# nkwangyh/CubemapSLAM

Hardware: AMD Instinct MI355X
Metric: frames/sec (extract+match+localBA) on Lafida cam0 (higher is better)
Workload: dtype u8 (extract/match), f64 (BA)

## Files before the change

### cubemapslam_amd/api.py

```python
import time
import ctypes as C
import os
import numpy as np

_HERE = os.path.dirname(os.path.abspath(__file__))
LIB_PATH = os.environ.get("CMS_HIP_LIB") or os.path.join(_HERE, "lib", "libcubemapslam_hip.so")


class CmsError(RuntimeError):
    pass


class Camera(C.Structure):
    _fields_ = [("c", C.c_double), ("d", C.c_double), ("e", C.c_double), ("u0", C.c_double), ("v0", C.c_double),
                ("invpol", C.c_double * 12), ("pol", C.c_double * 5), ("Iw", C.c_int), ("Ih", C.c_int),
                ("face", C.c_int), ("fov_deg", C.c_double)]


class OrbParams(C.Structure):
    _fields_ = [("nfeatures", C.c_int), ("scale_factor", C.c_float), ("nlevels", C.c_int),
                ("ini_th_fast", C.c_int), ("min_th_fast", C.c_int)]


class Geometry(C.Structure):
    _fields_ = [("W", C.c_int), ("F", C.c_int), ("nlevels", C.c_int), ("kp_cap", C.c_int), ("max_batch", C.c_int),
                ("level_w", C.c_int * 12), ("level_h", C.c_int * 12), ("level_quota", C.c_int * 12),
                ("level_cells", C.c_int * 12), ("scale", C.c_float * 12), ("inv_scale", C.c_float * 12),
                ("sigma2", C.c_float * 12), ("inv_sigma2", C.c_float * 12), ("pyramid_bytes_per_frame", C.c_size_t),
                ("candidate_entries_per_frame", C.c_size_t), ("fisheye_stride", C.c_int)]


class BaStats(C.Structure):
    _fields_ = [("iterations_done", C.c_int * 2), ("chi2_initial", C.c_double * 2), ("chi2_final", C.c_double * 2),
                ("lambda_final", C.c_double * 2), ("n_outliers_mid", C.c_int), ("n_outliers_final", C.c_int)]


KP_DTYPE = np.dtype([("x", "<f4"), ("y", "<f4"), ("size", "<f4"), ("angle", "<f4"), ("response", "<f4"),
                     ("octave", "<i4")])

_lib = None


def lib():
    global _lib
    if _lib is None:
        if not os.path.exists(LIB_PATH):
            raise CmsError("libcubemapslam_hip.so is missing -- build it with `python -m cubemapslam_amd.build` "
                           "(there is no CPU fallback)")
        L = C.CDLL(LIB_PATH)
        L.cms_last_error.restype = C.c_char_p
        for n in ("cms_ctx_stream", "cms_frames_input", "cms_ba_stream"):
            getattr(L, n).restype = C.c_void_p
            getattr(L, n).argtypes = [C.c_void_p]
        L.cms_ctx_create.argtypes = [C.c_void_p, C.c_int, C.c_void_p, C.c_void_p, C.c_int]
        L.cms_ctx_destroy.argtypes = [C.c_void_p]
        L.cms_ctx_destroy.restype = None
        L.cms_ctx_geometry.argtypes = [C.c_void_p, C.c_void_p]
        L.cms_remap.argtypes = [C.c_void_p, C.c_void_p, C.c_int, C.c_void_p, C.c_int]
        L.cms_set_mask.argtypes = [C.c_void_p, C.c_void_p, C.c_int]
        L.cms_extract.argtypes = [C.c_void_p, C.c_void_p, C.c_int, C.c_void_p, C.c_void_p, C.c_int, C.c_void_p]
        L.cms_remap_extract.argtypes = [C.c_void_p, C.c_void_p, C.c_int, C.c_void_p, C.c_void_p, C.c_int, C.c_void_p]
        L.cms_frames_upload.argtypes = [C.c_void_p, C.c_void_p, C.c_int, C.c_size_t, C.c_int]
        L.cms_frames_upload_async.argtypes = [C.c_void_p, C.c_void_p, C.c_int, C.c_size_t, C.c_int]
        L.cms_frames_upload_wait.argtypes = [C.c_void_p]
        L.cms_frames_upload_device.argtypes = [C.c_void_p, C.c_void_p, C.c_int]
        L.cms_frames_process_device.argtypes = [C.c_void_p, C.c_void_p, C.c_int]
        L.cms_host_alloc.argtypes = [C.c_void_p, C.c_size_t]
        L.cms_host_free.argtypes = [C.c_void_p]
        L.cms_host_free.restype = None
        L.cms_ba_profile_kernel.argtypes = [C.c_void_p, C.c_int]
        L.cms_ba_profile_get.argtypes = [C.c_void_p, C.c_void_p, C.c_void_p]
        L.cms_ba_debug_compose.argtypes = [C.c_int, C.c_void_p, C.c_int, C.c_int, C.c_void_p, C.c_void_p, C.c_int, C.c_void_p, C.c_void_p, C.c_void_p, C.c_void_p]
        L.cms_frames_process.argtypes = [C.c_void_p, C.c_int, C.c_int]
        L.cms_frames_sync.argtypes = [C.c_void_p]
        L.cms_frames_results.argtypes = [C.c_void_p, C.c_void_p, C.c_void_p, C.c_void_p]
        L.cms_frames_fetch.argtypes = [C.c_void_p, C.c_int, C.c_void_p, C.c_void_p, C.c_int, C.c_void_p]
        L.cms_debug_lut.argtypes = [C.c_void_p, C.c_void_p, C.c_void_p]
        L.cms_debug_cubemap.argtypes = [C.c_void_p, C.c_int, C.c_void_p, C.c_int]
        L.cms_debug_level.argtypes = [C.c_void_p, C.c_int, C.c_int, C.c_void_p, C.c_int]
        L.cms_debug_candidates.argtypes = [C.c_void_p, C.c_int, C.c_int, C.c_void_p, C.c_int, C.c_void_p]
        L.cms_debug_distributed.argtypes = [C.c_void_p, C.c_int, C.c_int, C.c_void_p, C.c_int, C.c_void_p]
        L.cms_profile_enable.argtypes = [C.c_void_p, C.c_int]
        L.cms_profile_get.argtypes = [C.c_void_p, C.c_void_p]
        L.cms_hamming_best2.argtypes = [C.c_void_p, C.c_void_p, C.c_int, C.c_void_p, C.c_int] + [C.c_void_p] * 9
        L.cms_hamming_best2_device.argtypes = [C.c_void_p, C.c_void_p, C.c_void_p, C.c_int] + [C.c_void_p] * 10
        L.cms_hamming_matrix.argtypes = [C.c_void_p, C.c_void_p, C.c_int, C.c_void_p, C.c_int, C.c_void_p]
        L.cms_ba_create.argtypes = [C.c_void_p, C.c_int, C.c_int, C.c_void_p, C.c_void_p, C.c_int, C.c_void_p, C.c_int,
                                    C.c_void_p, C.c_void_p, C.c_void_p, C.c_void_p, C.c_void_p, C.c_double, C.c_double,
                                    C.c_double, C.c_double]
        L.cms_ba_reset.argtypes = [C.c_void_p]
        L.cms_ba_optimize.argtypes = [C.c_void_p, C.c_int, C.c_int, C.c_void_p, C.c_void_p]
        L.cms_ba_read.argtypes = [C.c_void_p, C.c_void_p, C.c_void_p, C.c_void_p]
        L.cms_ba_destroy.argtypes = [C.c_void_p]
        L.cms_ba_destroy.restype = None
        L.cms_ba_run.argtypes = [C.c_int, C.c_int, C.c_void_p, C.c_void_p, C.c_int, C.c_void_p, C.c_int, C.c_void_p,
                                 C.c_void_p, C.c_void_p, C.c_void_p, C.c_void_p, C.c_double, C.c_double, C.c_double,
                                 C.c_double, C.c_int, C.c_int, C.c_void_p, C.c_void_p, C.c_void_p]
        L.cms_ba_linearize.argtypes = [C.c_int, C.c_int, C.c_void_p, C.c_void_p, C.c_int, C.c_void_p, C.c_int, C.c_void_p,
                                       C.c_void_p, C.c_void_p, C.c_void_p, C.c_void_p, C.c_double, C.c_double, C.c_double,
                                       C.c_double, C.c_int, C.c_double] + [C.c_void_p] * 7
        L.cms_area_set_keypoints.argtypes = [C.c_void_p, C.c_int, C.c_int, C.c_void_p]
        L.cms_area_grid.argtypes = [C.c_void_p, C.c_int]
        L.cms_features_in_area.argtypes = [C.c_void_p, C.c_int, C.c_int] + [C.c_void_p] * 7 + [C.c_int, C.c_void_p]
        L.cms_features_in_area_device.argtypes = [C.c_void_p, C.c_int, C.c_int] + [C.c_void_p] * 8 + [C.c_int, C.c_int, C.c_void_p]
        L.cms_features_in_area_batch_device.argtypes = [C.c_void_p, C.c_int] + [C.c_void_p] * 9 + [C.c_int, C.c_void_p]
        L.cms_area_set_descriptors.argtypes = [C.c_void_p, C.c_int, C.c_int, C.c_void_p]
        L.cms_search_local_points.argtypes = ([C.c_void_p, C.c_int, C.c_void_p, C.c_int] + [C.c_void_p] * 5 + [C.c_float] * 3 + [C.c_int, C.c_int] +
                                              [C.c_void_p] * 9)
        L.cms_search_by_projection.argtypes = ([C.c_void_p, C.c_int, C.c_void_p, C.c_int] + [C.c_void_p] * 5 + [C.c_float, C.c_int, C.c_int, C.c_int] +
                                               [C.c_void_p] * 3)
        L.cms_project_last_frame_device.argtypes = [C.c_void_p, C.c_int] + [C.c_void_p] * 5 + [C.c_float] + [C.c_void_p] * 5
        L.cms_rotation_filter_device.argtypes = [C.c_void_p, C.c_int] + [C.c_void_p] * 5 + [C.c_int]
        L.cms_is_in_frustum_device.argtypes = [C.c_void_p, C.c_int] + [C.c_void_p] * 6 + [C.c_float, C.c_float] + [C.c_void_p] * 8
        L.cms_search_local_points_device.argtypes = [C.c_void_p, C.c_int] + [C.c_void_p] * 5 + [C.c_float, C.c_int] + [C.c_void_p] * 3
        L.cms_create_new_map_points.argtypes = [C.c_void_p, C.c_int, C.c_void_p, C.c_void_p, C.c_void_p, C.c_int, C.c_int] + [C.c_void_p] * 5
        L.cms_kfstore_create.argtypes = [C.c_void_p, C.c_void_p, C.c_int, C.c_int, C.c_int]
        L.cms_kfstore_destroy.argtypes = [C.c_void_p]
        L.cms_kfstore_destroy.restype = None
        L.cms_kfstore_put.argtypes = [C.c_void_p, C.c_int, C.c_void_p]
        L.cms_kfstore_update.argtypes = [C.c_void_p, C.c_int] + [C.c_void_p] * 5
        L.cms_kfstore_fuse_search.argtypes = [C.c_void_p, C.c_int] + [C.c_void_p] * 8 + [C.c_float, C.c_void_p, C.c_void_p]
        L.cms_kfstore_fuse_search_sets.argtypes = [C.c_void_p, C.c_int] + [C.c_void_p] * 6 + [C.c_int] + [C.c_void_p] * 3 + [C.c_float, C.c_void_p, C.c_void_p]
        L.cms_kfstore_put_from_frame.argtypes = [C.c_void_p, C.c_int, C.c_void_p, C.c_int, C.c_int, C.c_void_p, C.c_void_p, C.c_void_p, C.c_float, C.c_void_p, C.c_int,
                                                 C.c_void_p, C.c_void_p, C.c_void_p]
        L.cms_kfstore_update_poses.argtypes = [C.c_void_p, C.c_int] + [C.c_void_p] * 4
        L.cms_kfstore_debug_fetch.argtypes = [C.c_void_p, C.c_int] + [C.c_void_p] * 12
        L.cms_ba_debug_fetch_plan.argtypes = [C.c_void_p] * 14
        L.cms_kfstore_create_new_map_points.argtypes = [C.c_void_p, C.c_int, C.c_void_p, C.c_void_p, C.c_void_p, C.c_int, C.c_int] + [C.c_void_p] * 5
        L.cms_distinctive_descriptors.argtypes = [C.c_void_p, C.c_int, C.c_void_p, C.c_void_p, C.c_void_p]
        L.cms_update_normal_and_depth.argtypes = [C.c_void_p, C.c_int] + [C.c_void_p] * 8
        L.cms_fuse_search.argtypes = [C.c_void_p, C.c_int, C.c_void_p, C.c_int] + [C.c_void_p] * 6 + [C.c_float, C.c_void_p, C.c_void_p]
        L.cms_pose_create.argtypes = [C.c_void_p, C.c_int, C.c_int, C.c_int]
        L.cms_pose_destroy.argtypes = [C.c_void_p]
        L.cms_pose_destroy.restype = None
        L.cms_pose_stream.argtypes = [C.c_void_p]
        L.cms_pose_stream.restype = C.c_void_p
        _edge = [C.c_void_p] * 5 + [C.c_double] * 4
        L.cms_pose_upload.argtypes = [C.c_void_p, C.c_int] + _edge + [C.c_void_p]
        L.cms_pose_launch.argtypes = [C.c_void_p]
        L.cms_pose_fetch.argtypes = [C.c_void_p, C.c_void_p, C.c_void_p, C.c_void_p, C.c_void_p]
        L.cms_pose_optimize_batch.argtypes = [C.c_void_p, C.c_int] + _edge + [C.c_void_p] * 4
        L.cms_pose_optimize.argtypes = [C.c_int, C.c_int] + [C.c_void_p] * 4 + [C.c_double] * 4 + [C.c_void_p] * 4
        _lib = L
    return _lib


def _p(a):
    if a is None:
        return None
    if isinstance(a, int):
        return C.c_void_p(a)
    return a.ctypes.data_as(C.c_void_p)


def _chk(rc, what):
    if rc < 0:
        raise CmsError("%s failed (%d): %s" % (what, rc, lib().cms_last_error().decode()))
    return rc


def make_camera(d):
    cam = Camera()
    for k in ("c", "d", "e", "u0", "v0", "Iw", "Ih", "face", "fov_deg"):
        setattr(cam, k, d[k])
    for i in range(12):
        cam.invpol[i] = d["invpol"][i] if i < len(d["invpol"]) else 0.0
    for i in range(5):
        cam.pol[i] = d["pol"][i] if i < len(d["pol"]) else 0.0
    return cam


RT_DTYPE = np.dtype([(n, "<u2") for n in ("tx", "ty", "x0", "y0", "nd", "rows", "flags", "pad")])
RT_LDS_MAX = 32768


def remap_lut_host(cam):
    cam = make_camera(cam) if isinstance(cam, dict) else cam
    W = 3 * cam.face
    out = np.zeros((W, (W + 3) // 4 * 4), np.uint32)
    f = lib().cms_remap_lut_host
    f.argtypes = [C.c_void_p, C.c_void_p, C.c_int]
    _chk(f(C.byref(cam), _p(out), out.shape[1]), "cms_remap_lut_host")
    return out[:, :W]


def remap_tiles_host(cam, lut, tile_w, tile_h, lds_budget=RT_LDS_MAX):
    cam = make_camera(cam) if isinstance(cam, dict) else cam
    lut = np.ascontiguousarray(lut, np.uint32)
    W = 3 * cam.face
    cap = ((W + tile_w - 1) // tile_w) * ((W + tile_h - 1) // tile_h)
    out = np.zeros(cap, RT_DTYPE)
    n_live, n_all, lds = C.c_int(), C.c_int(), C.c_int()
    f = lib().cms_remap_tiles_host
    f.argtypes = [C.c_void_p, C.c_void_p] + [C.c_int] * 4 + [C.c_void_p, C.c_int] + [C.c_void_p] * 3
    _chk(f(C.byref(cam), _p(lut), lut.strides[0] // 4, tile_w, tile_h, lds_budget, _p(out), cap, C.byref(n_live), C.byref(n_all), C.byref(lds)),
         "cms_remap_tiles_host")
    return out[:n_all.value].copy(), n_live.value, lds.value


class Context:

    def __init__(self, cam, nfeatures=2000, scale_factor=1.2, nlevels=8, ini_th=20, min_th=7, max_batch=1, device=0):
        self.cam = make_camera(cam) if isinstance(cam, dict) else cam
        self.orb = OrbParams(nfeatures, scale_factor, nlevels, ini_th, min_th)
        self.h = C.c_void_p()
        _chk(lib().cms_ctx_create(C.byref(self.h), device, C.byref(self.cam), C.byref(self.orb), max_batch), "cms_ctx_create")
        self.geom = Geometry()
        _chk(lib().cms_ctx_geometry(self.h, C.byref(self.geom)), "cms_ctx_geometry")
        self.W = self.geom.W
        self.max_batch = max_batch

    def close(self):
        if getattr(self, "h", None) and self.h.value:
            lib().cms_ctx_destroy(self.h)
            self.h = C.c_void_p()

    def __del__(self):
        try:
            self.close()
        except Exception:
            pass

    @property
    def stream(self):
        return lib().cms_ctx_stream(self.h)

    def set_mask(self, mask):
        mask = np.ascontiguousarray(mask, np.uint8)
        _chk(lib().cms_set_mask(self.h, _p(mask), mask.strides[0]), "cms_set_mask")

    def set_distance_bounds_mode(self, scaled):
        f = lib().cms_set_distance_bounds_mode
        f.argtypes = [C.c_void_p, C.c_int]
        _chk(f(self.h, int(scaled)), "cms_set_distance_bounds_mode")

    def set_gaussian_mode(self, column_mode):
        f = lib().cms_set_gaussian_mode
        f.argtypes = [C.c_void_p, C.c_int]
        _chk(f(self.h, int(column_mode)), "cms_set_gaussian_mode")

    def remap(self, fisheye, cubemap=None):
        fisheye = np.ascontiguousarray(fisheye, np.uint8)
        if cubemap is None:
            cubemap = np.zeros((self.W, self.W), np.uint8)
        _chk(lib().cms_remap(self.h, _p(fisheye), fisheye.strides[0], _p(cubemap), cubemap.strides[0]), "cms_remap")
        return cubemap

    def extract(self, cubemap, cap=None):
        cubemap = np.ascontiguousarray(cubemap, np.uint8)
        cap = cap or self.geom.kp_cap
        kps = np.zeros(cap, KP_DTYPE)
        desc = np.zeros((cap, 32), np.uint8)
        n = C.c_int()
        _chk(lib().cms_extract(self.h, _p(cubemap), cubemap.strides[0], _p(kps), _p(desc), cap, C.byref(n)), "cms_extract")
        return kps[:n.value].copy(), desc[:n.value].copy()

    def remap_extract(self, fisheye, cap=None):
        fisheye = np.ascontiguousarray(fisheye, np.uint8)
        cap = cap or self.geom.kp_cap
        kps = np.zeros(cap, KP_DTYPE)
        desc = np.zeros((cap, 32), np.uint8)
        n = C.c_int()
        _chk(lib().cms_remap_extract(self.h, _p(fisheye), fisheye.strides[0], _p(kps), _p(desc), cap, C.byref(n)), "cms_remap_extract")
        return kps[:n.value].copy(), desc[:n.value].copy()

    def remap_extract_rays(self, fisheye, cap=None):
        fisheye = np.ascontiguousarray(fisheye, np.uint8)
# ... 44 lines not shown
    def sync(self):
        _chk(lib().cms_frames_sync(self.h), "cms_frames_sync")

    def fetch(self, b):
        cap = self.geom.kp_cap
        kps = np.zeros(cap, KP_DTYPE)
        desc = np.zeros((cap, 32), np.uint8)
        n = C.c_int()
        _chk(lib().cms_frames_fetch(self.h, b, _p(kps), _p(desc), cap, C.byref(n)), "cms_frames_fetch")
        return kps[:n.value].copy(), desc[:n.value].copy()

    def results_ptrs(self):
        a, b, c = C.c_void_p(), C.c_void_p(), C.c_void_p()
        _chk(lib().cms_frames_results(self.h, C.byref(a), C.byref(b), C.byref(c)), "cms_frames_results")
        return a.value, b.value, c.value

    def input_ptr(self):
        return lib().cms_frames_input(self.h)

    def profile(self, on=True):
        lib().cms_profile_enable(self.h, 1 if on else 0)

    def profile_ms(self):
        ms = np.zeros(7, np.float32)
        _chk(lib().cms_profile_get(self.h, _p(ms)), "cms_profile_get")
        return dict(zip(("remap", "pyramid", "fast", "octree", "cull", "describe", "total"), ms.tolist()))

    def debug_lut(self):
        W = self.W
        out = np.zeros((W, (W + 3) // 4 * 4), np.uint32)
        s = C.c_int()
        _chk(lib().cms_debug_lut(self.h, _p(out), C.byref(s)), "cms_debug_lut")
        return out[:, :W]

    def debug_level(self, b, l):
        w, h = self.geom.level_w[l], self.geom.level_h[l]
        out = np.zeros((h, w), np.uint8)
        _chk(lib().cms_debug_level(self.h, b, l, _p(out), w), "cms_debug_level")
        return out

    def debug_candidates(self, b, l):
        cap = self.geom.level_w[l] * self.geom.level_h[l] // 4 + 4096
        out = np.zeros((cap, 3), np.int32)
        n = C.c_int()
        _chk(lib().cms_debug_candidates(self.h, b, l, _p(out), cap, C.byref(n)), "cms_debug_candidates")
        return out[:n.value].copy()

    def debug_distributed(self, b, l):
        cap = self.geom.level_quota[l] + 8
        out = np.zeros((cap, 3), np.int32)
        n = C.c_int()
        _chk(lib().cms_debug_distributed(self.h, b, l, _p(out), cap, C.byref(n)), "cms_debug_distributed")
        return out[:n.value].copy()

    def hamming_best2(self, qdesc, tdesc, cand_off, cand_idx, tlevel=None, texcl=None):
        qdesc = np.ascontiguousarray(qdesc, np.uint8); tdesc = np.ascontiguousarray(tdesc, np.uint8)
        cand_off = np.ascontiguousarray(cand_off, np.int32); cand_idx = np.ascontiguousarray(cand_idx, np.int32)
        tl = np.ascontiguousarray(tlevel, np.int32) if tlevel is not None else None
        tx = np.ascontiguousarray(texcl, np.uint8) if texcl is not None else None
        nq = len(qdesc)
        outs = [np.zeros(max(nq, 1), np.int32) for _ in range(5)]
        _chk(lib().cms_hamming_best2(self.h, _p(qdesc), nq, _p(tdesc), len(tdesc), _p(cand_off), _p(cand_idx), _p(tl), _p(tx),
                                     *[_p(o) for o in outs]), "cms_hamming_best2")
        keys = ("best_idx", "best_dist", "best_level", "second_dist", "second_level")
        return {k: o[:nq] for k, o in zip(keys, outs)}

    def area_set_keypoints(self, b, kps):
        kps = np.ascontiguousarray(kps, KP_DTYPE)
        _chk(lib().cms_area_set_keypoints(self.h, b, len(kps), _p(kps)), "cms_area_set_keypoints")

    def area_grid(self, B):
        _chk(lib().cms_area_grid(self.h, B), "cms_area_grid")

    def features_in_area(self, b, qx, qy, qr, qmin, qmax, cap=None):
        qx = np.ascontiguousarray(qx, np.float32); qy = np.ascontiguousarray(qy, np.float32); qr = np.ascontiguousarray(qr, np.float32)
        qmin = np.ascontiguousarray(qmin, np.int32); qmax = np.ascontiguousarray(qmax, np.int32)
        nq = len(qx)
        cap = cap or max(1, 64 * nq + 1024)
        off = np.zeros(nq + 1, np.int32); idx = np.zeros(cap, np.int32); tot = C.c_int(0)
        _chk(lib().cms_features_in_area(self.h, b, nq, _p(qx), _p(qy), _p(qr), _p(qmin), _p(qmax), _p(off), _p(idx), cap, C.byref(tot)),
             "cms_features_in_area")
        return off, idx[:tot.value]

    def features_in_area_device(self, b, nq, d_q5, d_cnt, d_off, d_idx, cap, idx_base, d_total):
        _chk(lib().cms_features_in_area_device(self.h, b, nq, *[C.c_void_p(int(a)) for a in d_q5], C.c_void_p(int(d_cnt)), C.c_void_p(int(d_off)),
                                               C.c_void_p(int(d_idx)), cap, idx_base, C.c_void_p(int(d_total))), "cms_features_in_area_device")

    def features_in_area_batch_device(self, nq, d_qframe, d_q5, d_cnt, d_off, d_idx, cap, d_total):
        _chk(lib().cms_features_in_area_batch_device(self.h, nq, C.c_void_p(int(d_qframe)), *[C.c_void_p(int(a)) for a in d_q5], C.c_void_p(int(d_cnt)),
                                                     C.c_void_p(int(d_off)), C.c_void_p(int(d_idx)), cap, C.c_void_p(int(d_total))),
             "cms_features_in_area_batch_device")

    def area_set_descriptors(self, b, desc):
        desc = np.ascontiguousarray(desc, np.uint8)
        _chk(lib().cms_area_set_descriptors(self.h, b, len(desc), _p(desc)), "cms_area_set_descriptors")

    def search_local_points(self, b, pose15, pos, normal, min_dist, max_dist, mp_desc, kp_mp, viewing_cos_limit=0.5, th=1.0, nnratio=0.8,
                            th_high=100):
        pose15 = np.ascontiguousarray(pose15, np.float32).reshape(15)
        pos = np.ascontiguousarray(pos, np.float32).reshape(-1, 3); normal = np.ascontiguousarray(normal, np.float32).reshape(-1, 3)
        n = len(pos)
        min_dist = np.ascontiguousarray(min_dist, np.float32); max_dist = np.ascontiguousarray(max_dist, np.float32)
        mp_desc = np.ascontiguousarray(mp_desc, np.uint8).reshape(n, 32)
        assert kp_mp.dtype == np.int32 and kp_mp.flags.c_contiguous
        vis = np.zeros(n, np.uint8); px = np.zeros(n, np.float32); py = np.zeros(n, np.float32); lvl = np.zeros(n, np.int32)
        vc = np.zeros(n, np.float32); match = np.full(n, -1, np.int32)
        nm = C.c_int(0); rounds = C.c_int(0)
        _chk(lib().cms_search_local_points(self.h, b, _p(pose15), n, _p(pos), _p(normal), _p(min_dist), _p(max_dist), _p(mp_desc),
                                           viewing_cos_limit, th, nnratio, th_high, len(kp_mp), _p(kp_mp), _p(vis), _p(px), _p(py), _p(lvl),
                                           _p(vc), _p(match), C.addressof(nm), C.addressof(rounds)), "cms_search_local_points")
        return dict(in_view=vis, proj_x=px, proj_y=py, level=lvl, view_cos=vc, match=match, n_matches=nm.value, rounds=rounds.value)

    def search_by_projection(self, b, pose12, valid, Xw, octave, angle, mp_desc, kp_mp, th=15.0, check_ori=True, th_high=100):
        a = [np.ascontiguousarray(pose12, np.float32), np.ascontiguousarray(valid, np.uint8), np.ascontiguousarray(Xw, np.float32),
             np.ascontiguousarray(octave, np.int32), np.ascontiguousarray(angle, np.float32), np.ascontiguousarray(mp_desc, np.uint8)]
        n = len(a[1])
        match = np.full(n, -1, np.int32); nm = C.c_int(0)
        assert kp_mp.dtype == np.int32
        _chk(lib().cms_search_by_projection(self.h, b, _p(a[0]), n, *[_p(v) for v in a[1:]], th, int(check_ori), th_high, len(kp_mp), _p(kp_mp), _p(match),
                                            C.addressof(nm)), "cms_search_by_projection")
        return match, nm.value

    def search_for_initialization(self, b2, k1, d1, prev_matched, window=100, nnratio=0.9, check_ori=True):
        k1 = np.ascontiguousarray(k1, KP_DTYPE); d1 = np.ascontiguousarray(d1, np.uint8)
        assert prev_matched.dtype == np.float32 and prev_matched.flags.c_contiguous and prev_matched.shape == (len(k1), 2)
        m12 = np.full(max(len(k1), 1), -1, np.int32); nm = C.c_int(0)
        f = lib().cms_search_for_initialization
        f.argtypes = [C.c_void_p, C.c_int, C.c_int, C.c_void_p, C.c_void_p, C.c_void_p, C.c_int, C.c_float, C.c_int, C.c_void_p, C.c_void_p]
        _chk(f(self.h, b2, len(k1), _p(k1), _p(d1), _p(prev_matched), int(window), float(nnratio), int(check_ori), _p(m12), C.addressof(nm)),
             "cms_search_for_initialization")
        return m12[:len(k1)], nm.value

    def project_last_frame_device(self, n, d_qframe, d_pose12, d_valid, d_Xw, d_oct, th, d_q5):
        v = lambda a: C.c_void_p(int(a)) if a else None
        _chk(lib().cms_project_last_frame_device(self.h, n, v(d_qframe), v(d_pose12), v(d_valid), v(d_Xw), v(d_oct), th, *[v(a) for a in d_q5]),
             "cms_project_last_frame_device")

    def rotation_filter_device(self, B, d_mp_off, d_last_angle, d_kp_mp, d_mp_match, d_n_matches, check_orientation=True):
        v = lambda a: C.c_void_p(int(a)) if a else None
        _chk(lib().cms_rotation_filter_device(self.h, B, v(d_mp_off), v(d_last_angle), v(d_kp_mp), v(d_mp_match), v(d_n_matches), int(check_orientation)),
             "cms_rotation_filter_device")

    def is_in_frustum_device(self, nmp, d_mp_frame, d_pose15, d_pos, d_normal, d_min, d_max, viewing_cos_limit, th, d_outs5, d_q3):
        v = lambda a: C.c_void_p(int(a)) if a else None
        _chk(lib().cms_is_in_frustum_device(self.h, nmp, v(d_mp_frame), v(d_pose15), v(d_pos), v(d_normal), v(d_min), v(d_max),
                                            viewing_cos_limit, th, *[v(a) for a in d_outs5], *[v(a) for a in d_q3]), "cms_is_in_frustum_device")

    def search_local_points_device(self, B, d_mp_off, d_mp_desc, d_cand_off, d_cand_idx, d_pair_dist, nnratio, th_high, d_kp_mp, d_mp_match,
                                   d_rounds=0):
        v = lambda a: C.c_void_p(int(a)) if a else None
        _chk(lib().cms_search_local_points_device(self.h, B, v(d_mp_off), v(d_mp_desc), v(d_cand_off), v(d_cand_idx), v(d_pair_dist), nnratio,
                                                  th_high, v(d_kp_mp), v(d_mp_match), v(d_rounds)), "cms_search_local_points_device")

    def hamming_best2_device(self, qdesc, q_row, nq, tdesc, cand_off, cand_idx, t_level, t_excl, outs):
        _chk(lib().cms_hamming_best2_device(self.h, _p(qdesc), _p(q_row), nq, _p(tdesc), _p(cand_off), _p(cand_idx), _p(t_level),
                                            _p(t_excl), *[_p(o) for o in outs]), "cms_hamming_best2_device")

    def hamming_matrix(self, a, b):
        a = np.ascontiguousarray(a, np.uint8); b = np.ascontiguousarray(b, np.uint8)
        out = np.zeros((len(a), len(b)), np.uint16)
        _chk(lib().cms_hamming_matrix(self.h, _p(a), len(a), _p(b), len(b), _p(out)), "cms_hamming_matrix")
        return out


class PinnedArray:

    def __init__(self, shape):
        n = int(np.prod(shape))
        self.p = C.c_void_p()
        _chk(lib().cms_host_alloc(C.byref(self.p), n), "cms_host_alloc")
        self.array = np.ctypeslib.as_array((C.c_uint8 * n).from_address(self.p.value)).reshape(shape)

    def close(self):
        if self.p:
            self.array = None
            lib().cms_host_free(self.p)
            self.p = None

    def __del__(self):
        try:
            self.close()
        except Exception:
            pass


class Keyframe(C.Structure):
    _fields_ = [("n", C.c_int), ("kps", C.c_void_p), ("desc", C.c_void_p), ("rays", C.c_void_p), ("mp", C.c_void_p),
                ("Rcw", C.c_float * 9), ("tcw", C.c_float * 3), ("Ow", C.c_float * 3),
                ("nnodes", C.c_int), ("node_id", C.c_void_p), ("node_off", C.c_void_p), ("node_feat", C.c_void_p), ("median_depth", C.c_float)]


def make_keyframe(kf):
    n = len(kf["x"])
    kps = np.zeros(n, KP_DTYPE); kps["x"] = kf["x"]; kps["y"] = kf["y"]; kps["octave"] = kf["octave"]; kps["angle"] = kf["angle"]
    keep = [kps, np.ascontiguousarray(kf["desc"], np.uint8), np.ascontiguousarray(kf["rays"], np.float32), np.ascontiguousarray(kf["mp"], np.int32),
            np.ascontiguousarray(kf["node_id"], np.int32), np.ascontiguousarray(kf["node_off"], np.int32), np.ascontiguousarray(kf["node_feat"], np.int32)]
    K = Keyframe()
    K.n = n; K.kps = keep[0].ctypes.data; K.desc = keep[1].ctypes.data; K.rays = keep[2].ctypes.data; K.mp = keep[3].ctypes.data
    K.Rcw[:] = [float(v) for v in np.asarray(kf["R"], np.float32).reshape(9)]
    K.tcw[:] = [float(v) for v in kf["t"]]; K.Ow[:] = [float(v) for v in kf["Ow"]]
    K.nnodes = len(keep[4]); K.node_id = keep[4].ctypes.data; K.node_off = keep[5].ctypes.data; K.node_feat = keep[6].ctypes.data
    K.median_depth = float(kf["median_depth"])
    return K, keep


def search_for_triangulation(ctx, K1, K2, E12=None, check_orientation=False):
    m = np.full(max(K1.n, 1), -1, np.int32)
    n = C.c_int()
    e = None if E12 is None else np.ascontiguousarray(E12, np.float32)
    lib().cms_search_for_triangulation.argtypes = [C.c_void_p, C.c_void_p, C.c_void_p, C.c_void_p, C.c_int, C.c_void_p, C.c_void_p]
    _chk(lib().cms_search_for_triangulation(ctx.h, C.byref(K1), C.byref(K2), _p(e) if e is not None else None, int(check_orientation), _p(m), C.byref(n)),
         "cms_search_for_triangulation")
    return m[:K1.n].copy(), n.value


def create_new_map_points(ctx, jobs, check_orientation=False, cap=None):
    nj = len(jobs)
    cur = (Keyframe * max(nj, 1))(*[j[0] for j in jobs])
    flat = [k for j in jobs for k in j[1]]
    neigh = (Keyframe * max(len(flat), 1))(*flat)
    off = np.concatenate([[0], np.cumsum([len(j[1]) for j in jobs])]).astype(np.int32)
    cap = cap if cap is not None else max([j[0].n for j in jobs] + [1])
    n_new = np.zeros(max(nj, 1), np.int32)
    on = np.zeros((max(nj, 1), cap), np.int32); o1 = np.zeros_like(on); o2 = np.zeros_like(on); ox = np.zeros((max(nj, 1), cap, 3), np.float32)
    _chk(lib().cms_create_new_map_points(ctx.h, nj, C.addressof(cur), _p(off), C.addressof(neigh), int(check_orientation), cap, _p(n_new), _p(on), _p(o1),
                                         _p(o2), _p(ox)), "cms_create_new_map_points")
    return [(on[j, :n_new[j]].copy(), o1[j, :n_new[j]].copy(), o2[j, :n_new[j]].copy(), ox[j, :n_new[j]].copy()) for j in range(nj)]


class BowJob(C.Structure):
    _fields_ = [("slot", C.c_int), ("b", C.c_int), ("n", C.c_int), ("nnodes", C.c_int), ("node_id", C.c_void_p), ("node_off", C.c_void_p),
                ("node_feat", C.c_void_p), ("kf_skip", C.c_void_p)]


def _bow_fv(fv):
    if isinstance(fv, dict):
        fv = (fv["node_id"], fv["node_off"], fv["node_feat"])
    nid, noff, nfeat = (np.ascontiguousarray(a, np.int32) for a in fv)
    if len(noff) == 0:
        noff = np.zeros(1, np.int32)
    return nid, noff, (nfeat if len(nfeat) else np.zeros(1, np.int32))


def search_by_bow(ctx, b, n, fv, K, skip=None, nnratio=0.7, check_orientation=True):
    nid, noff, nfeat = _bow_fv(fv)
    sk = None if skip is None else np.ascontiguousarray(skip, np.uint8)
    kf_idx = np.full(max(n, 1), -1, np.int32)
    nm = C.c_int()
    L = lib()
    L.cms_search_by_bow.argtypes = [C.c_void_p, C.c_int, C.c_int, C.c_int, C.c_void_p, C.c_void_p, C.c_void_p, C.c_void_p, C.c_void_p, C.c_float, C.c_int,
                                    C.c_void_p, C.c_void_p]
    _chk(L.cms_search_by_bow(ctx.h, b, n, len(nid), _p(nid), _p(noff), _p(nfeat), C.byref(K), _p(sk), float(nnratio), int(check_orientation), _p(kf_idx),
                             C.byref(nm)), "cms_search_by_bow")
    return kf_idx[:n].copy(), nm.value


class KeyframeStore:

    def __init__(self, ctx, max_keyframes, max_features=2048, max_nodes=2048):
        self.ctx = ctx
        self.h = C.c_void_p()
        _chk(lib().cms_kfstore_create(C.byref(self.h), ctx.h, max_keyframes, max_features, max_nodes), "cms_kfstore_create")

    def close(self):
        if self.h:
            lib().cms_kfstore_destroy(self.h); self.h = None

    def __del__(self):
        try:
            self.close()
        except Exception:
            pass

    def put(self, slot, K):
        _chk(lib().cms_kfstore_put(self.h, slot, C.byref(K)), "cms_kfstore_put")

    def update(self, slot, R=None, t=None, Ow=None, median_depth=None, mp=None):
        f = lambda a, dt: None if a is None else np.ascontiguousarray(a, dt)
        a = [f(R, np.float32), f(t, np.float32), f(Ow, np.float32), None if median_depth is None else np.array([median_depth], np.float32), f(mp, np.int32)]
        _chk(lib().cms_kfstore_update(self.h, slot, *[_p(v) for v in a]), "cms_kfstore_update")

    def put_from_frame(self, slot, src_ctx, b, n, kf):
        f32 = lambda a: np.ascontiguousarray(a, np.float32)
        i32 = lambda a: None if a is None else np.ascontiguousarray(a, np.int32)
        R, t, Ow = f32(np.asarray(kf["R"]).reshape(9)), f32(kf["t"]), f32(kf["Ow"])
        mp, nid, noff, nfeat = i32(kf.get("mp")), i32(kf["node_id"]), i32(kf["node_off"]), i32(kf["node_feat"])
        L = lib()
        _chk(L.cms_kfstore_put_from_frame(self.h, slot, src_ctx.h, b, n, _p(R), _p(t), _p(Ow), float(kf["median_depth"]), _p(mp), len(nid), _p(nid), _p(noff), _p(nfeat)),
             "cms_kfstore_put_from_frame")

    def put_from_frames(self, src_ctx, items):
        class KfFromFrame(C.Structure):
            _fields_ = [("slot", C.c_int), ("b", C.c_int), ("n", C.c_int), ("Rcw", C.c_void_p), ("tcw", C.c_void_p), ("Ow", C.c_void_p), ("median_depth", C.c_float),
                        ("mp", C.c_void_p), ("nnodes", C.c_int), ("node_id", C.c_void_p), ("node_off", C.c_void_p), ("node_feat", C.c_void_p)]
        arr = (KfFromFrame * len(items))()
        keep = []
        f32 = lambda a: np.ascontiguousarray(a, np.float32)
        i32 = lambda a: None if a is None else np.ascontiguousarray(a, np.int32)
        ptr = lambda a: None if a is None else a.ctypes.data
        for q, (slot, b, n, kf) in zip(arr, items):
            R, t, Ow = f32(np.asarray(kf["R"]).reshape(9)), f32(kf["t"]), f32(kf["Ow"])
            mp, nid, noff, nfeat = i32(kf.get("mp")), i32(kf["node_id"]), i32(kf["node_off"]), i32(kf["node_feat"])
            keep.append((R, t, Ow, mp, nid, noff, nfeat))
            q.slot = slot; q.b = b; q.n = n; q.Rcw = ptr(R); q.tcw = ptr(t); q.Ow = ptr(Ow); q.median_depth = float(kf["median_depth"]); q.mp = ptr(mp)
            q.nnodes = len(nid); q.node_id = ptr(nid); q.node_off = ptr(noff); q.node_feat = ptr(nfeat)
        L = lib()
# ... 405 lines not shown
```

### cubemapslam_amd/csrc/cms_api_frames.hip

```cpp
#include <chrono>
#include <thread>
#include <hip/hip_runtime.h>
#include <math.h>
#include <stdio.h>
#include <stdlib.h>
#include <string.h>
#include <algorithm>
#include <string>
#include <vector>
#include "../../include/cubemapslam_hip.h"
#include "cms_types.h"
#include "orb_pattern.inc"

static bool cms_cu_mask_from_env(uint32_t* words, int* n_words) {
  const char* v = getenv("CMS_CTX_CU_MASK");
  if (!v || !*v) return false;
  int n = 0;
  while (*v && n < 8) {
    char* end = nullptr;
    words[n++] = (uint32_t)strtoul(v, &end, 16);
    if (end == v) return false;
    v = *end == ',' ? end + 1 : end;
    if (*end && *end != ',') return false;
  }
  *n_words = n;
  return n > 0;
}

static thread_local std::string g_cms_err;
static int cms_fail(int code, const char* what, hipError_t e = hipSuccess) {
  char buf[512];
  if (e != hipSuccess) snprintf(buf, sizeof(buf), "%s: %s", what, hipGetErrorString(e));
  else snprintf(buf, sizeof(buf), "%s", what);
  g_cms_err = buf;
  return code;
}
#define HIPCHK(call)                                                        \
  do {                                                                      \
    hipError_t _e = (call);                                                 \
    if (_e != hipSuccess) return cms_fail(CMS_ERR_HIP, #call, _e);          \
  } while (0)

extern "C" const char* cms_last_error(void) { return g_cms_err.c_str(); }
extern "C" int cms_device_count(void) {
  int n = 0;
  if (hipGetDeviceCount(&n) != hipSuccess) return 0;
  return n;
}

struct cms_ctx {
  int device = 0;
  cms_camera cam;
  cms_orb_params orb;
  int max_batch = 0;
  CmsGeom g;
  float scale[CMS_MAX_LEVELS], inv_scale[CMS_MAX_LEVELS], sigma2[CMS_MAX_LEVELS], inv_sigma2[CMS_MAX_LEVELS];
  hipStream_t stream = nullptr;
  int fstride = 0;
  size_t fish_pitch = 0;
  int lut_stride = 0, mstride = 0;
  bool have_mask = false;
  int dirty_frames = 0;
  uint8_t* d_fish = nullptr; uint32_t* d_lut = nullptr; uint8_t* d_pyr = nullptr; uint8_t* d_mask = nullptr;
  cms_remap_tile* d_rtiles = nullptr; int rt_mode = 1, rt_tw = 64, rt_live = 0, rt_all = 0, rt_lds = 0;
  CmsResizeTab* d_tab = nullptr; float* d_pattern = nullptr;
  uint32_t* d_cand = nullptr; uint16_t* d_node = nullptr; int* d_cand_cnt = nullptr; int* d_overflow = nullptr;
  uint32_t* d_qt_out = nullptr; int* d_qt_cnt = nullptr;
  uint32_t* d_cell_cand = nullptr; int* d_cell_cnt = nullptr;
  int* d_cells_all = nullptr; int* d_cells_nz = nullptr; int n_cells_all = 0, n_cells_nz = 0;
  uint16_t* d_area_sorted = nullptr; int* d_area_cell_start = nullptr; int* d_area_nvalid = nullptr; int area_frames = 0;
  int* d_area_bsum = nullptr; int area_bsum_cap = 0;
  int* d_area_tmp = nullptr; size_t area_tmp_cap = 0;
  uint8_t* h_fish_stage = nullptr; int fish_stage_frames = 0;
  hipStream_t copy_stream = nullptr; hipEvent_t ev_upload_done = nullptr, ev_remap_done = nullptr;
  bool upload_pending = false, remap_recorded = false;
  int dist_bounds_scaled = 0;
  hipEvent_t ev_block = nullptr; int last_batch = 0;
  hipEvent_t ev_extracted = nullptr; bool extracted_recorded = false;
  uint8_t* h_stage = nullptr; size_t h_stage_bytes = 0;
  CmsKeyPoint* d_kps = nullptr; uint32_t* d_aux = nullptr; uint8_t* d_desc = nullptr; int* d_kp_cnt = nullptr;
  uint32_t* d_order = nullptr; uint32_t* d_aux_sorted = nullptr; int* d_walk_cnt = nullptr; float* d_rays = nullptr;
  void* d_match = nullptr; size_t match_bytes = 0;
  bool prof = false;
  bool desc_spatial = false;
  hipEvent_t ev[8] = {nullptr, nullptr, nullptr, nullptr, nullptr, nullptr, nullptr, nullptr};
  size_t fast_lds = 0, qt_lds = 0;
};

static inline double cms_horner12(const double* c, double x) {
  double r = 0.0;
  for (int i = 11; i >= 0; --i) r = r * x + c[i];
  return r;
}
static void cms_cubemap_to_fisheye(const cms_camera& cam, double up, double vp, double* uf, double* vf) {
  const int F = cam.face;
  const double half = F / 2.0;
  float i = (float)up, j = (float)vp;
  *uf = -1; *vf = -1;
  const float fi = i / (float)F, fj = j / (float)F;
  int face = CMS_FACE_UNKNOWN;
  if (fi >= 0 && fi < 1 && fj >= 1 && fj < 2) face = CMS_FACE_LEFT;
  else if (fi >= 1 && fi < 2 && fj >= 0 && fj < 1) face = CMS_FACE_UPPER;
  else if (fi >= 1 && fi < 2 && fj >= 1 && fj < 2) face = CMS_FACE_FRONT;
  else if (fi >= 1 && fi < 2 && fj >= 2 && fj < 3) face = CMS_FACE_LOWER;
  else if (fi >= 2 && fi < 3 && fj >= 1 && fj < 2) face = CMS_FACE_RIGHT;
  if (face == CMS_FACE_UNKNOWN) return;
  i = i - (float)((int)(i / (float)F) * F);
  j = j - (float)((int)(j / (float)F) * F);
  const double lx = ((double)i - half) * 1.0 / half, ly = ((double)j - half) * 1.0 / half, lz = 1.0;
  double x, y, z;
  switch (face) {
    case CMS_FACE_FRONT: x = lx; y = ly; z = lz; break;
    case CMS_FACE_LEFT: x = -lz; y = ly; z = lx; break;
    case CMS_FACE_RIGHT: x = lz; y = ly; z = -lx; break;
    case CMS_FACE_LOWER: x = lx; y = lz; z = -ly; break;
    default: x = lx; y = -lz; z = ly; break;
  }
  double norm = sqrt(x * x + y * y);
  if (norm == 0.0) norm = 1e-14;
  const double theta = atan(-z / norm);
  const double rho = cms_horner12(cam.invpol, theta);
  const double uu = x / norm * rho, vv = y / norm * rho;
  *uf = uu * cam.c + vv * cam.d + cam.u0;
  *vf = uu * cam.e + vv + cam.v0;
  if (*uf < 0 || *uf >= cam.Iw || *vf < 0 || *vf >= cam.Ih) { *uf = -1; *vf = -1; }
}
static void cms_build_lut(const cms_camera& cam, int lut_stride, std::vector<uint32_t>& lut) {
  const int W = 3 * cam.face;
  lut.assign((size_t)W * lut_stride, 0u);
  for (int y = 0; y < W; ++y)
    for (int x = 0; x < W; ++x) {
      double u, v;
      cms_cubemap_to_fisheye(cam, (double)x, (double)y, &u, &v);
      if (u < 0 || v < 0 || u >= cam.Iw || v >= cam.Ih) continue;
      const float mu = (float)u, mv = (float)v;
      const int sx = (int)lrint((double)(mu * 32.f)), sy = (int)lrint((double)(mv * 32.f));
      const uint32_t X = (uint32_t)(sx >> 5), Y = (uint32_t)(sy >> 5), ax = (uint32_t)(sx & 31), ay = (uint32_t)(sy & 31);
      lut[(size_t)y * lut_stride + x] = X | (Y << 11) | (ax << 22) | (ay << 27);
    }
}

extern "C" int cms_remap_lut_host(const cms_camera* cam, uint32_t* lut, int lut_stride) {
  if (!cam || !lut || cam->face < 1 || lut_stride < 3 * cam->face) return cms_fail(CMS_ERR_ARG, "cms_remap_lut_host: bad argument");
  std::vector<uint32_t> v;
  cms_build_lut(*cam, lut_stride, v);
  memcpy(lut, v.data(), v.size() * 4);
  return CMS_OK;
}
extern "C" int cms_remap_tiles_host(const cms_camera* cam, const uint32_t* lut, int lut_stride, int tile_w, int tile_h, int lds_budget,
                                    cms_remap_tile* out, int cap, int* n_live, int* n_all, int* lds_bytes) {
  if (!cam || !lut || !out || !n_live || !n_all || !lds_bytes || cam->face < 1 || lut_stride < 3 * cam->face || !cms_rt_shape_ok(tile_w, tile_h) || lds_budget < 0)
    return cms_fail(CMS_ERR_ARG, "cms_remap_tiles_host: bad argument");
  std::vector<cms_remap_tile> v;
  cms_rt_build(cam->face, lut, lut_stride, tile_w, tile_h, lds_budget, v, n_live, lds_bytes);
  *n_all = (int)v.size();
  if ((int)v.size() > cap) return cms_fail(CMS_ERR_OVERFLOW, "cms_remap_tiles_host: caller capacity too small");
  memcpy(out, v.data(), v.size() * sizeof(cms_remap_tile));
  return CMS_OK;
}

static inline short cms_sat_short(float v) {
  const long iv = lrint((double)v);
  return (short)(iv < -32768 ? -32768 : iv > 32767 ? 32767 : iv);
}
static void cms_resize_table(int sn, int dn, bool clamp_frac, CmsResizeTab* out) {
  const double inv_scale = (double)dn / sn, scale = 1. / inv_scale;
  for (int d = 0; d < dn; ++d) {
    float f = (float)((d + 0.5) * scale - 0.5);
    int s = (int)floorf(f);
    f -= s;
    if (clamp_frac) {
      if (s < 0) { f = 0; s = 0; }
      if (s >= sn - 1) { f = 0; s = sn - 1; }
    }
    out[d].s = (short)s;
    out[d].a0 = cms_sat_short((1.f - f) * 2048);
    out[d].a1 = cms_sat_short(f * 2048);
    out[d].pad = 0;
  }
}

static size_t align_up(size_t v, size_t a) { return (v + a - 1) / a * a; }

static void cms_ctx_free(cms_ctx* c) {
  if (!c) return;
  hipSetDevice(c->device);
  void* ptrs[] = {c->d_fish, c->d_lut, c->d_pyr, c->d_mask, c->d_tab, c->d_pattern, c->d_cand, c->d_node, c->d_cand_cnt,
                  c->d_overflow, c->d_qt_out, c->d_qt_cnt, c->d_kps, c->d_aux, c->d_order, c->d_aux_sorted, c->d_desc, c->d_kp_cnt, c->d_match, c->d_cell_cand,
                  c->d_cell_cnt, c->d_cells_all, c->d_cells_nz, c->d_area_sorted, c->d_area_cell_start, c->d_area_nvalid, c->d_area_bsum, c->d_area_tmp, c->d_walk_cnt, c->d_rays, c->d_rtiles};
  for (void* p : ptrs) if (p) hipFree(p);
  if (c->h_fish_stage) (void)hipHostFree(c->h_fish_stage);
  if (c->h_stage) (void)hipHostFree(c->h_stage);
  for (int i = 0; i < 8; ++i) if (c->ev[i]) hipEventDestroy(c->ev[i]);
  if (c->ev_extracted) hipEventDestroy(c->ev_extracted);
  if (c->ev_block) hipEventDestroy(c->ev_block);
  if (c->ev_upload_done) hipEventDestroy(c->ev_upload_done);
  if (c->ev_remap_done) hipEventDestroy(c->ev_remap_done);
  if (c->copy_stream) hipStreamDestroy(c->copy_stream);
  if (c->stream) hipStreamDestroy(c->stream);
  delete c;
}

extern "C" int cms_ctx_create(cms_ctx** out, int device, const cms_camera* cam, const cms_orb_params* orb, int max_batch) {
  if (!out || !cam || !orb || max_batch < 1) return cms_fail(CMS_ERR_ARG, "cms_ctx_create: bad argument");
  *out = nullptr;
  if (orb->nlevels < 1 || orb->nlevels > CMS_MAX_LEVELS) return cms_fail(CMS_ERR_UNSUPPORTED, "nlevels must be 1..12");
  if (cam->face < 32 || 3 * cam->face > 4095) return cms_fail(CMS_ERR_UNSUPPORTED, "face size must satisfy 32 <= F and 3F <= 4095");
  if (cam->Iw < 2 || cam->Ih < 2 || cam->Iw > 2047 || cam->Ih > 2047) return cms_fail(CMS_ERR_UNSUPPORTED, "fisheye size must be <= 2047");
  int ndev = 0;
  if (hipGetDeviceCount(&ndev) != hipSuccess || ndev == 0) return cms_fail(CMS_ERR_NO_DEVICE, "no HIP device: the product path has no CPU fallback");
  if (device < 0 || device >= ndev) return cms_fail(CMS_ERR_ARG, "device index out of range");
  HIPCHK(hipSetDevice(device));
  cms_ctx* c = new cms_ctx;
  c->device = device; c->cam = *cam; c->orb = *orb; c->max_batch = max_batch;
  CmsGeom& g = c->g;
  memset(&g, 0, sizeof(g));
  const int L = orb->nlevels, F = cam->face, W = 3 * F;
  g.nlevels = L; g.W = W; g.F = F; g.ini_th = orb->ini_th_fast; g.min_th = orb->min_th_fast;
  const double scaleFactor = orb->scale_factor;
  c->scale[0] = 1.0f; c->sigma2[0] = 1.0f;
  for (int i = 1; i < L; ++i) { c->scale[i] = (float)(c->scale[i - 1] * scaleFactor); c->sigma2[i] = c->scale[i] * c->scale[i]; }
  for (int i = 0; i < L; ++i) { c->inv_scale[i] = 1.0f / c->scale[i]; c->inv_sigma2[i] = 1.0f / c->sigma2[i]; }
  {
    const float factor = (float)(1.0f / scaleFactor);
    float nDesired = orb->nfeatures * (1 - factor) / (1 - (float)pow((double)factor, (double)L));
    int sum = 0;
    for (int l = 0; l < L - 1; ++l) { g.lv[l].quota = (int)lrint((double)nDesired); sum += g.lv[l].quota; nDesired *= factor; }
    g.lv[L - 1].quota = orb->nfeatures - sum > 0 ? orb->nfeatures - sum : 0;
  }
  size_t off = 0, cand_off = 0, tab_off = 0;
  int cell0 = 0, kp_off = 0, maxq = 0, wCellMax = 0, hCellMax = 0;
  for (int l = 0; l < L; ++l) {
    CmsLevel& lv = g.lv[l];
    lv.w = (int)lrint((double)((float)W * c->inv_scale[l]));
    lv.h = lv.w;
    if (lv.w < 2 * CMS_MINB + 30) { delete c; return cms_fail(CMS_ERR_UNSUPPORTED, "pyramid level too small for the FAST cell grid"); }
    lv.stride = (int)align_up((size_t)lv.w + 8, 128);
    lv.off = off;
    off += align_up((size_t)lv.stride * (lv.h + 1), 256);
    const float width = (float)(lv.w - 2 * CMS_MINB), height = (float)(lv.h - 2 * CMS_MINB);
    lv.nCols = (int)(width / 30.f); lv.nRows = (int)(height / 30.f);
    lv.wCell = (int)ceilf(width / lv.nCols); lv.hCell = (int)ceilf(height / lv.nRows);
    lv.cell0 = cell0; cell0 += lv.nCols * lv.nRows;
    lv.cand_cap = (lv.w * lv.h) / 4 + 4096;
    lv.cand_off = cand_off; cand_off += align_up((size_t)lv.cand_cap, 64);
    lv.kp_off = kp_off; kp_off += lv.quota + 3;
    lv.scale = c->scale[l];
    lv.patch_size = (float)(int)(31 * c->scale[l]);
    lv.tab_off = tab_off; tab_off += (size_t)lv.w + lv.h;
    if (lv.quota > maxq) maxq = lv.quota;
    if (lv.wCell > wCellMax) wCellMax = lv.wCell;
    if (lv.hCell > hCellMax) hCellMax = lv.hCell;
    if (lv.nCols > 255 || lv.nRows > 255) { delete c; return cms_fail(CMS_ERR_UNSUPPORTED, "more than 255 FAST cells per row"); }
  }
  g.total_cells = cell0; g.kp_cap = kp_off; g.pyr_bytes = off; g.cand_total = cand_off;
  g.qt_maxn = 8;
  while (g.qt_maxn < maxq + 3) g.qt_maxn <<= 1;
  if (g.qt_maxn > 2048) { delete c; return cms_fail(CMS_ERR_UNSUPPORTED, "per-level feature quota above 2045 is not supported"); }
  g.tile_h = hCellMax + 6;
  g.tile_stride = (int)align_up((size_t)wCellMax + 6 + 3, 4) + 4;
  g.sc_h = hCellMax + 2;
  g.sc_stride = (int)align_up((size_t)wCellMax + 2, 4);
  g.list_cap = wCellMax * hCellMax;
  g.cell_cap = (int)align_up((size_t)((wCellMax + 1) / 2) * ((hCellMax + 1) / 2), 8);
  g.dbg_stop = getenv("CMS_DBG_FAST_STOP") ? atoi(getenv("CMS_DBG_FAST_STOP")) : 0;
  c->desc_spatial = getenv("CMS_DESC_SPATIAL_ORDER") != nullptr && g.kp_cap <= CMS_ORDER_MAX && max_batch <= 65535;
  g.gauss_column_mode = 0;
  if (wCellMax > 60 || hCellMax > 60) { delete c; return cms_fail(CMS_ERR_UNSUPPORTED, "FAST cell larger than 60 pixels"); }
  if (orb->scale_factor < 1.01f || orb->scale_factor > 1.9f) { delete c; return cms_fail(CMS_ERR_UNSUPPORTED, "scaleFactor must be in [1.01, 1.9]"); }
  g.fast_cell_lds = (int)align_up((size_t)g.tile_h * g.tile_stride + (size_t)g.sc_h * g.sc_stride + 2 * (size_t)g.list_cap + 16, 16);
  c->fast_lds = CMS_FAST_WPB * (size_t)g.fast_cell_lds;
  c->qt_lds = 64 * (size_t)g.qt_maxn + 4 * 512 + 64;

  c->fstride = (int)align_up((size_t)cam->Iw, 64);
  c->fish_pitch = (size_t)c->fstride * cam->Ih;
  c->lut_stride = (int)align_up((size_t)W, 4);
  c->mstride = (int)align_up((size_t)W, 64);
  const size_t B = (size_t)max_batch;
#define ALLOC(ptr, bytes) do { hipError_t _e = hipMalloc((void**)&(ptr), (bytes)); if (_e != hipSuccess) { cms_ctx_free(c); return cms_fail(CMS_ERR_HIP, "hipMalloc " #ptr, _e); } } while (0)
  hipError_t e;
  {
    const char* pr = getenv("CMS_FRAME_STREAM_PRIORITY");
    int lo = 0, hi = 0;
    uint32_t cu_mask[8]; int cu_words = 0;
    if (cms_cu_mask_from_env(cu_mask, &cu_words))
      e = hipExtStreamCreateWithCUMask(&c->stream, (uint32_t)cu_words, cu_mask);
    else
    if (pr && hipDeviceGetStreamPriorityRange(&lo, &hi) == hipSuccess && lo != hi)
      e = hipStreamCreateWithPriority(&c->stream, hipStreamNonBlocking, pr[0] == 'h' ? hi : lo);
    else
      e = hipStreamCreateWithFlags(&c->stream, hipStreamNonBlocking);
  }
  if (e != hipSuccess) { cms_ctx_free(c); return cms_fail(CMS_ERR_HIP, "hipStreamCreate", e); }
  for (int i = 0; i < 8; ++i) hipEventCreate(&c->ev[i]);
  ALLOC(c->d_fish, B * c->fish_pitch + 256);
  ALLOC(c->d_lut, (size_t)W * c->lut_stride * 4);
  ALLOC(c->d_pyr, B * g.pyr_bytes + 256);
  ALLOC(c->d_mask, (size_t)W * c->mstride);
  ALLOC(c->d_tab, tab_off * sizeof(CmsResizeTab));
  ALLOC(c->d_pattern, 1024 * sizeof(float));
  ALLOC(c->d_cand, B * g.cand_total * 4);
  ALLOC(c->d_node, B * g.cand_total * 2);
  ALLOC(c->d_cand_cnt, B * L * sizeof(int));
  ALLOC(c->d_overflow, sizeof(int));
  ALLOC(c->d_cell_cand, B * g.total_cells * g.cell_cap * 4);
  ALLOC(c->d_cell_cnt, B * g.total_cells * sizeof(int));
  ALLOC(c->d_qt_out, B * g.kp_cap * 4);
  ALLOC(c->d_qt_cnt, B * L * sizeof(int));
  ALLOC(c->d_kps, B * g.kp_cap * sizeof(CmsKeyPoint));
  ALLOC(c->d_aux, B * g.kp_cap * 4);
  ALLOC(c->d_order, B * g.kp_cap * 4);
  ALLOC(c->d_walk_cnt, 16);
  ALLOC(c->d_rays, B * g.kp_cap * 12);
  ALLOC(c->d_aux_sorted, B * g.kp_cap * 4);
  ALLOC(c->d_desc, B * g.kp_cap * 32);
  ALLOC(c->d_kp_cnt, B * sizeof(int));
#undef ALLOC
  hipMemset(c->d_pyr, 0, B * g.pyr_bytes + 256);
  hipMemset(c->d_fish, 0, B * c->fish_pitch + 256);
  hipMemset(c->d_mask, 255, (size_t)W * c->mstride);
  hipMemset(c->d_overflow, 0, sizeof(int));
  hipMemset(c->d_kp_cnt, 0, B * sizeof(int));
  {
    std::vector<uint32_t> lut;
    cms_build_lut(*cam, c->lut_stride, lut);
    hipMemcpy(c->d_lut, lut.data(), lut.size() * 4, hipMemcpyHostToDevice);
    {
      const char* m = getenv("CMS_REMAP_TILES"); const char* tw = getenv("CMS_REMAP_TILE_W");
      c->rt_mode = m && *m ? atoi(m) : 1;
      c->rt_tw = tw && *tw ? atoi(tw) : 64;
      if (c->rt_mode < 0 || c->rt_mode > 2 || !cms_rt_shape_ok(c->rt_tw, CMS_RT_PIXELS / std::max(c->rt_tw, 1))) {
        cms_ctx_free(c); return cms_fail(CMS_ERR_ARG, "CMS_REMAP_TILES must be 0, 1 or 2 and CMS_REMAP_TILE_W 32, 64 or 128");
      }
      std::vector<cms_remap_tile> tiles;
      cms_rt_build(F, lut.data(), c->lut_stride, c->rt_tw, CMS_RT_PIXELS / c->rt_tw, c->rt_mode == 1 ? CMS_RT_LDS_MAX : 0, tiles, &c->rt_live, &c->rt_lds);
      c->rt_all = (int)tiles.size();
      if (hipMalloc((void**)&c->d_rtiles, tiles.size() * sizeof(cms_remap_tile)) != hipSuccess) { cms_ctx_free(c); return cms_fail(CMS_ERR_HIP, "hipMalloc tile table"); }
      hipMemcpy(c->d_rtiles, tiles.data(), tiles.size() * sizeof(cms_remap_tile), hipMemcpyHostToDevice);
    }
    std::vector<CmsResizeTab> tab(tab_off);
    for (int l = 1; l < L; ++l) {
      cms_resize_table(g.lv[l - 1].w, g.lv[l].w, true, &tab[g.lv[l].tab_off]);
      cms_resize_table(g.lv[l - 1].h, g.lv[l].h, false, &tab[g.lv[l].tab_off + g.lv[l].w]);
    }
    g.lv[0].zlo = F; g.lv[0].zhi = F;
    for (int l = 1; l < L; ++l) {
      const CmsResizeTab* tx = &tab[g.lv[l].tab_off];
      const int sw = g.lv[l - 1].w, dw = g.lv[l].w;
      int lo = 0, hi = 0;
      while (lo < dw && std::min((int)tx[lo].s + 1, sw - 1) < g.lv[l - 1].zlo) ++lo;
      while (hi < dw && (int)tx[dw - 1 - hi].s >= sw - g.lv[l - 1].zhi) ++hi;
      g.lv[l].zlo = lo; g.lv[l].zhi = hi;
    }
    hipMemcpy(c->d_tab, tab.data(), tab.size() * sizeof(CmsResizeTab), hipMemcpyHostToDevice);
    std::vector<int> all, nz;
    for (int l = 0; l < L; ++l) {
      if (g.lv[l].nRows > 255 || g.lv[l].nCols > 255) { cms_ctx_free(c); return cms_fail(CMS_ERR_UNSUPPORTED, "cms_ctx_create: more than 255 FAST cells per row"); }
      const CmsLevel& lv = g.lv[l];
      const int maxBX = lv.w - CMS_MINB, maxBY = lv.h - CMS_MINB;
      for (int ci = 0; ci < lv.nRows; ++ci)
        for (int cj = 0; cj < lv.nCols; ++cj) {
          const int iniY = CMS_MINB + ci * lv.hCell, iniX = CMS_MINB + cj * lv.wCell;
          if (iniY >= maxBY - 3 || iniX >= maxBX - 6) continue;
          const int maxY = std::min(iniY + lv.hCell + 6, maxBY), maxX = std::min(iniX + lv.wCell + 6, maxBX);
          if (maxX - iniX - 6 <= 0 || maxY - iniY - 6 <= 0) continue;
          const int id = l | (ci << 4) | (cj << 12);
          all.push_back(id);
          const bool zero = (maxX <= lv.zlo || iniX >= lv.w - lv.zhi) && (maxY <= lv.zlo || iniY >= lv.h - lv.zhi);
          if (!zero) nz.push_back(id);
        }
    }
    auto xcd_stripe = [](std::vector<int>& v) {
      if (getenv("CMS_FAST_NO_XCD_STRIPE")) return;
      const size_t n = v.size(), per = (n + 7) / 8;
      std::vector<int> out;
      out.reserve(n);
      for (size_t j = 0; j < per; ++j)
        for (size_t x = 0; x < 8; ++x) if (x * per + j < n) out.push_back(v[x * per + j]);
      v.swap(out);
    };
    xcd_stripe(all); xcd_stripe(nz);
    c->n_cells_all = (int)all.size(); c->n_cells_nz = (int)nz.size();
    if (hipMalloc((void**)&c->d_cells_all, std::max<size_t>(all.size(), 1) * 4) != hipSuccess ||
        hipMalloc((void**)&c->d_cells_nz, std::max<size_t>(nz.size(), 1) * 4) != hipSuccess) {
      cms_ctx_free(c); return cms_fail(CMS_ERR_HIP, "hipMalloc cell lists");
    }
    hipMemcpy(c->d_cells_all, all.data(), all.size() * 4, hipMemcpyHostToDevice);
    hipMemcpy(c->d_cells_nz, nz.data(), nz.size() * 4, hipMemcpyHostToDevice);
    float patf[1024];
    for (int i = 0; i < 1024; ++i) patf[i] = (float)kOrbPattern[i];
    hipMemcpy(c->d_pattern, patf, sizeof(patf), hipMemcpyHostToDevice);
  }
  e = hipFuncSetAttribute((const void*)k_quadtree, hipFuncAttributeMaxDynamicSharedMemorySize, (int)c->qt_lds);
  if (e != hipSuccess) { cms_ctx_free(c); return cms_fail(CMS_ERR_HIP, "hipFuncSetAttribute(k_quadtree)", e); }
  e = hipDeviceSynchronize();
  if (e != hipSuccess) { cms_ctx_free(c); return cms_fail(CMS_ERR_HIP, "ctx init", e); }
  *out = c;
  return CMS_OK;
}

extern "C" void cms_ctx_destroy(cms_ctx* ctx) { cms_ctx_free(ctx); }
extern "C" void* cms_ctx_stream(cms_ctx* ctx) { return ctx ? (void*)ctx->stream : nullptr; }

extern "C" int cms_ctx_geometry(const cms_ctx* c, cms_geometry* o) {
  if (!c || !o) return cms_fail(CMS_ERR_ARG, "cms_ctx_geometry: null");
  memset(o, 0, sizeof(*o));
  o->W = c->g.W; o->F = c->g.F; o->nlevels = c->g.nlevels; o->kp_cap = c->g.kp_cap; o->max_batch = c->max_batch;
  for (int l = 0; l < c->g.nlevels; ++l) {
    o->level_w[l] = c->g.lv[l].w; o->level_h[l] = c->g.lv[l].h; o->level_quota[l] = c->g.lv[l].quota;
    o->level_cells[l] = c->g.lv[l].nCols * c->g.lv[l].nRows;
    o->scale[l] = c->scale[l]; o->inv_scale[l] = c->inv_scale[l]; o->sigma2[l] = c->sigma2[l]; o->inv_sigma2[l] = c->inv_sigma2[l];
  }
  o->pyramid_bytes_per_frame = c->g.pyr_bytes; o->candidate_entries_per_frame = c->g.cand_total;
  o->fisheye_stride = c->fstride;
  return CMS_OK;
}

extern "C" void* cms_frames_input(cms_ctx* c) { return c ? (void*)c->d_fish : nullptr; }

static int cms_frames_upload_impl(cms_ctx* c, const uint8_t* fisheye, int fstride, size_t frame_pitch, int B, bool wait) {
  if (!c || !fisheye || B < 1 || B > c->max_batch || fstride < c->cam.Iw) return cms_fail(CMS_ERR_ARG, "cms_frames_upload: bad argument");
  HIPCHK(hipSetDevice(c->device));
  const size_t per_frame = c->fish_pitch;
  if (!c->h_fish_stage || c->fish_stage_frames < B) {
    if (c->h_fish_stage) (void)hipHostFree(c->h_fish_stage);
    c->h_fish_stage = nullptr; c->fish_stage_frames = 0;
    if (hipHostMalloc((void**)&c->h_fish_stage, per_frame * (size_t)B) == hipSuccess) c->fish_stage_frames = B;
  }
  if (c->h_fish_stage) {
    for (int b = 0; b < B; ++b)
      for (int r = 0; r < c->cam.Ih; ++r)
        memcpy(c->h_fish_stage + (size_t)b * per_frame + (size_t)r * c->fstride, fisheye + (size_t)b * frame_pitch + (size_t)r * fstride, (size_t)c->cam.Iw);
    HIPCHK(hipMemcpyAsync(c->d_fish, c->h_fish_stage, per_frame * (size_t)B, hipMemcpyHostToDevice, c->stream));
  } else {
    for (int b = 0; b < B; ++b)
      HIPCHK(hipMemcpy2DAsync(c->d_fish + (size_t)b * c->fish_pitch, c->fstride, fisheye + (size_t)b * frame_pitch, fstride,
                              c->cam.Iw, c->cam.Ih, hipMemcpyHostToDevice, c->stream));
  }
  if (wait || !c->h_fish_stage) HIPCHK(hipStreamSynchronize(c->stream));
  return CMS_OK;
}
extern "C" int cms_frames_upload(cms_ctx* c, const uint8_t* fisheye, int fstride, size_t frame_pitch, int B) {
  return cms_frames_upload_impl(c, fisheye, fstride, frame_pitch, B, true);
}

extern "C" int cms_frames_upload_async(cms_ctx* c, const uint8_t* fisheye, int fstride, size_t frame_pitch, int B) {
  if (!c || !fisheye || B < 1 || B > c->max_batch || fstride < c->cam.Iw) return cms_fail(CMS_ERR_ARG, "cms_frames_upload_async: bad argument");
  HIPCHK(hipSetDevice(c->device));
  if (!c->copy_stream) {
    HIPCHK(hipStreamCreateWithFlags(&c->copy_stream, hipStreamNonBlocking));
    HIPCHK(hipEventCreateWithFlags(&c->ev_upload_done, hipEventDisableTiming));
    HIPCHK(hipEventCreateWithFlags(&c->ev_remap_done, hipEventDisableTiming));
    HIPCHK(hipEventRecord(c->ev_remap_done, c->stream));
    c->remap_recorded = true;
  }
  if (c->remap_recorded) HIPCHK(hipStreamWaitEvent(c->copy_stream, c->ev_remap_done, 0));
  if (fstride == c->fstride && (frame_pitch == c->fish_pitch || B == 1)) {
    HIPCHK(hipMemcpyAsync(c->d_fish, fisheye, c->fish_pitch * (size_t)B, hipMemcpyHostToDevice, c->copy_stream));
  } else {
    for (int b = 0; b < B; ++b)
      HIPCHK(hipMemcpy2DAsync(c->d_fish + (size_t)b * c->fish_pitch, c->fstride, fisheye + (size_t)b * frame_pitch, fstride,
                              c->cam.Iw, c->cam.Ih, hipMemcpyHostToDevice, c->copy_stream));
  }
  HIPCHK(hipEventRecord(c->ev_upload_done, c->copy_stream));
  c->upload_pending = true;
  return CMS_OK;
}
extern "C" int cms_frames_upload_device(cms_ctx* c, const void* d_src, int B) {
  if (!c || !d_src || B < 1 || B > c->max_batch) return cms_fail(CMS_ERR_ARG, "cms_frames_upload_device: bad argument");
  HIPCHK(hipSetDevice(c->device));
  HIPCHK(hipMemcpyAsync(c->d_fish, d_src, c->fish_pitch * (size_t)B, hipMemcpyDeviceToDevice, c->stream));
  return CMS_OK;
}
extern "C" int cms_stream_copy_device(cms_ctx* c, void* d_dst, const void* d_src, size_t bytes) {
  if (!c || (bytes > 0 && (!d_dst || !d_src))) return cms_fail(CMS_ERR_ARG, "cms_stream_copy_device: bad argument");
  if (bytes == 0) return CMS_OK;
  HIPCHK(hipSetDevice(c->device));
  HIPCHK(hipMemcpyAsync(d_dst, d_src, bytes, hipMemcpyDeviceToDevice, c->stream));
  return CMS_OK;
}
// ... 422 lines not shown
```

### cubemapslam_amd/csrc/cms_api_track.hip

```cpp
#include <mutex>
#include <cmath>
#include <vector>

extern "C" int cms_area_set_descriptors(cms_ctx* c, int b, int n, const uint8_t* desc) {
  if (!c || b < 0 || b >= c->max_batch || n < 0 || n > c->g.kp_cap || (n > 0 && !desc)) return cms_fail(CMS_ERR_ARG, "cms_area_set_descriptors: bad argument");
  HIPCHK(hipSetDevice(c->device));
  if (n > 0) HIPCHK(hipMemcpyAsync(c->d_desc + (size_t)b * c->g.kp_cap * 32, desc, (size_t)n * 32, hipMemcpyHostToDevice, c->stream));
  HIPCHK(hipStreamSynchronize(c->stream));
  return CMS_OK;
}

extern "C" int cms_set_distance_bounds_mode(cms_ctx* c, int scaled) {
  if (!c || scaled < 0 || scaled > 1) return cms_fail(CMS_ERR_ARG, "cms_set_distance_bounds_mode: mode must be 0 or 1");
  c->dist_bounds_scaled = scaled;
  return CMS_OK;
}

extern "C" int cms_is_in_frustum_device(cms_ctx* c, int nmp, const void* d_mp_frame, const void* d_pose15, const void* d_pos, const void* d_normal,
                                        const void* d_min_dist, const void* d_max_dist, float viewing_cos_limit, float th, void* d_in_view,
                                        void* d_proj_x, void* d_proj_y, void* d_level, void* d_view_cos, void* d_qr, void* d_qmin, void* d_qmax) {
  if (!c || nmp < 0 || (nmp > 0 && (!d_pose15 || !d_pos || !d_normal || !d_min_dist || !d_max_dist || !d_in_view || !d_proj_x || !d_proj_y ||
                                    !d_level || !d_view_cos)) || (d_qr && (!d_qmin || !d_qmax)))
    return cms_fail(CMS_ERR_ARG, "cms_is_in_frustum_device: bad argument");
  if (nmp == 0) return CMS_OK;
  if (c->g.nlevels > 16) return cms_fail(CMS_ERR_UNSUPPORTED, "cms_is_in_frustum_device: more than 16 pyramid levels");
  HIPCHK(hipSetDevice(c->device));
  CmsFrustumArgs a;
  a.pose15 = (const float*)d_pose15; a.mp_frame = (const int*)d_mp_frame; a.n = nmp;
  a.P = (const float*)d_pos; a.normal = (const float*)d_normal; a.min_dist = (const float*)d_min_dist; a.max_dist = (const float*)d_max_dist;
  a.viewing_cos_limit = viewing_cos_limit; a.th = th; a.bounds_scaled = c->dist_bounds_scaled;
  a.log_scale = std::log(c->g.nlevels > 1 ? c->scale[1] : 1.2f);
  a.nlevels = c->g.nlevels; a.F = c->g.F;
  for (int l = 0; l < 16; ++l) a.sf[l] = l < c->g.nlevels ? c->scale[l] : 0.0f;
  a.in_view = (uint8_t*)d_in_view; a.proj_x = (float*)d_proj_x; a.proj_y = (float*)d_proj_y; a.level = (int*)d_level; a.view_cos = (float*)d_view_cos;
  a.qr = (float*)d_qr; a.qmin = (int*)d_qmin; a.qmax = (int*)d_qmax;
  hipLaunchKernelGGL(k_in_frustum, dim3((nmp + 255) / 256), dim3(256), 0, c->stream, a);
  HIPCHK(hipGetLastError());
  return CMS_OK;
}

extern "C" int cms_search_local_points_device(cms_ctx* c, int B, const void* d_mp_off, const void* d_mp_desc, const void* d_cand_off,
                                              const void* d_cand_idx, void* d_pair_dist, float nnratio, int th_high, void* d_kp_mp,
                                              void* d_mp_match, void* d_rounds) {
  if (!c || B < 1 || B > c->area_frames || !d_mp_off || !d_mp_desc || !d_cand_off || !d_cand_idx || !d_pair_dist || !d_kp_mp || !d_mp_match)
    return cms_fail(CMS_ERR_ARG, "cms_search_local_points_device: bad argument (cms_area_grid first)");
  if (c->g.kp_cap > CMS_TRACK_KPMAX) return cms_fail(CMS_ERR_UNSUPPORTED, "cms_search_local_points_device: more than 4096 key points per frame");
  HIPCHK(hipSetDevice(c->device));
  CmsSearchLocalArgs a;
  a.mp_off = (const int*)d_mp_off; a.mp_desc = (const uint4*)d_mp_desc; a.cand_off = (const int*)d_cand_off; a.cand_idx = (const int*)d_cand_idx;
  a.t_desc = (const uint4*)c->d_desc; a.kp = (const CmsKeyPoint*)c->d_kps; a.kp_cap = c->g.kp_cap;
  a.pair_dist = (uint16_t*)d_pair_dist; a.kp_mp = (int*)d_kp_mp; a.mp_match = (int*)d_mp_match; a.rounds = (int*)d_rounds;
  a.nnratio = nnratio; a.th_high = th_high; a.frame0 = 0; a.total = nullptr; a.cap = 0;
  hipLaunchKernelGGL(k_search_local, dim3(B), dim3(1024), 0, c->stream, a);
  HIPCHK(hipGetLastError());
  return CMS_OK;
}

extern "C" int cms_search_local_points(cms_ctx* c, int b, const float* pose15, int nmp, const float* pos, const float* normal,
                                       const float* min_dist, const float* max_dist, const uint8_t* mp_desc, float viewing_cos_limit, float th,
                                       float nnratio, int th_high, int nkp, int* kp_mp, uint8_t* in_view, float* proj_x, float* proj_y,
                                       int* level, float* view_cos, int* mp_match, int* n_matches, int* rounds) {
  if (!c || !pose15 || nmp < 0 || nkp < 0 || nkp > (c ? c->g.kp_cap : 0) || (nmp > 0 && (!pos || !normal || !min_dist || !max_dist || !mp_desc || !mp_match)) ||
      (nkp > 0 && !kp_mp))
    return cms_fail(CMS_ERR_ARG, "cms_search_local_points: bad argument");
  if (b < 0 || b >= c->area_frames) return cms_fail(CMS_ERR_ARG, "cms_search_local_points: no grid for this frame (cms_area_grid first)");
  if (c->g.kp_cap > CMS_TRACK_KPMAX) return cms_fail(CMS_ERR_UNSUPPORTED, "cms_search_local_points: more than 4096 key points per frame");
  if (n_matches) *n_matches = 0;
  if (rounds) *rounds = 0;
  if (nmp == 0) return CMS_OK;
  HIPCHK(hipSetDevice(c->device));
  hipStream_t s = c->stream;
  const size_t n4 = (size_t)nmp * 4, kp4 = (size_t)c->g.kp_cap * 4;
  auto al = [](size_t v) { return (v + 255) & ~(size_t)255; };
  size_t o = 0;
  auto take = [&](size_t bytes) { const size_t at = o; o += al(bytes); return at; };
  const size_t o_pose = take(64), o_pos = take(3 * n4), o_nrm = take(3 * n4), o_min = take(n4), o_max = take(n4), o_desc = take((size_t)nmp * 32),
               o_qf = take(n4), o_mpoff = take(16), o_kpmp = take(kp4);
  const size_t in_bytes = o;
  const size_t o_vis = take(nmp), o_px = take(n4), o_py = take(n4), o_lvl = take(n4), o_vc = take(n4), o_match = take(n4), o_tot = take(16), o_rounds = take(16);
  const size_t out_begin = o_kpmp, out_bytes = o - o_kpmp;
  const size_t o_qr = take(n4), o_qmin = take(n4), o_qmax = take(n4), o_cnt = take(n4), o_off = take(n4 + 4);
  const size_t fixed = o;
  int cap = 64 * nmp + 1024;
  for (int attempt = 0; attempt < 2; ++attempt) {
    const size_t o_idx = fixed, o_pd = fixed + al((size_t)cap * 4);
    int rc = cms_scratch(c, o_pd + al((size_t)cap * 2));
    if (rc) return rc;
    rc = cms_hstage(c, std::max(in_bytes, out_begin + out_bytes));
    if (rc) return rc;
    uint8_t* p = (uint8_t*)c->d_match;
    uint8_t* h = c->h_stage;
    memcpy(h + o_pose, pose15, 60);
    memcpy(h + o_pos, pos, 3 * n4); memcpy(h + o_nrm, normal, 3 * n4); memcpy(h + o_min, min_dist, n4); memcpy(h + o_max, max_dist, n4);
    memcpy(h + o_desc, mp_desc, (size_t)nmp * 32);
    { int* qf = reinterpret_cast<int*>(h + o_qf); for (int i = 0; i < nmp; ++i) qf[i] = b; }
    { int* mo = reinterpret_cast<int*>(h + o_mpoff); mo[0] = 0; mo[1] = nmp; }
    { int* km = reinterpret_cast<int*>(h + o_kpmp); for (int k = 0; k < c->g.kp_cap; ++k) km[k] = k < nkp ? kp_mp[k] : -1; }
    HIPCHK(hipMemcpyAsync(p, h, in_bytes, hipMemcpyHostToDevice, s));
    rc = cms_is_in_frustum_device(c, nmp, nullptr, p + o_pose, p + o_pos, p + o_nrm, p + o_min, p + o_max, viewing_cos_limit, th, p + o_vis,
                                  p + o_px, p + o_py, p + o_lvl, p + o_vc, p + o_qr, p + o_qmin, p + o_qmax);
    if (rc) return rc;
    rc = cms_features_in_area_batch_device(c, nmp, p + o_qf, p + o_px, p + o_py, p + o_qr, p + o_qmin, p + o_qmax, p + o_cnt, p + o_off, p + o_idx,
                                           cap, p + o_tot);
    if (rc) return rc;
    CmsSearchLocalArgs a;
    a.mp_off = (const int*)(p + o_mpoff); a.mp_desc = (const uint4*)(p + o_desc); a.cand_off = (const int*)(p + o_off); a.cand_idx = (const int*)(p + o_idx);
    a.t_desc = (const uint4*)c->d_desc; a.kp = (const CmsKeyPoint*)c->d_kps; a.kp_cap = c->g.kp_cap;
    a.pair_dist = (uint16_t*)(p + o_pd);
    a.kp_mp = (int*)(p + o_kpmp) - (size_t)b * c->g.kp_cap;
    a.mp_match = (int*)(p + o_match); a.rounds = (int*)(p + o_rounds);
    a.nnratio = nnratio; a.th_high = th_high; a.frame0 = b; a.total = (const int*)(p + o_tot); a.cap = cap;
    hipLaunchKernelGGL(k_search_local, dim3(1), dim3(1024), 0, s, a);
    HIPCHK(hipGetLastError());
    HIPCHK(hipMemcpyAsync(h + out_begin, p + out_begin, out_bytes, hipMemcpyDeviceToHost, s));
    HIPCHK(hipStreamSynchronize(s));
    const int tot = *reinterpret_cast<const int*>(h + o_tot);
    if (tot > cap) { cap = tot + 64; continue; }
    const int* match = reinterpret_cast<const int*>(h + o_match);
    if (nkp > 0) memcpy(kp_mp, h + o_kpmp, (size_t)nkp * 4);
    if (in_view) memcpy(in_view, h + o_vis, nmp);
    if (proj_x) memcpy(proj_x, h + o_px, n4);
    if (proj_y) memcpy(proj_y, h + o_py, n4);
    if (level) memcpy(level, h + o_lvl, n4);
    if (view_cos) memcpy(view_cos, h + o_vc, n4);
    int nm = 0;
    for (int i = 0; i < nmp; ++i) {
      const int m = match[i];
      mp_match[i] = m >= 0 ? m - b * c->g.kp_cap : -1;
      nm += m >= 0;
    }
    if (n_matches) *n_matches = nm;
    if (rounds) *rounds = *reinterpret_cast<const int*>(h + o_rounds);
    return CMS_OK;
  }
  return cms_fail(CMS_ERR_OVERFLOW, "cms_search_local_points: candidate lists kept growing");
}

extern "C" int cms_project_last_frame_device(cms_ctx* c, int n, const void* d_qframe, const void* d_pose12, const void* d_valid, const void* d_Xw,
                                             const void* d_oct, float th, void* d_qx, void* d_qy, void* d_qr, void* d_qmin, void* d_qmax) {
  if (!c || n < 0 || (n > 0 && (!d_pose12 || !d_valid || !d_Xw || !d_oct || !d_qx || !d_qy || !d_qr || !d_qmin || !d_qmax)))
    return cms_fail(CMS_ERR_ARG, "cms_project_last_frame_device: bad argument");
  if (n == 0) return CMS_OK;
  HIPCHK(hipSetDevice(c->device));
  CmsProjectLastArgs a;
  a.pose12 = (const float*)d_pose12; a.q_frame = (const int*)d_qframe; a.n = n; a.valid = (const uint8_t*)d_valid; a.Xw = (const float*)d_Xw;
  a.oct = (const int*)d_oct; a.th = th; a.F = c->g.F;
  {
    const float fov = (float)c->cam.fov_deg;
    const float pif = 3.1415926535897932384626f;
    a.cos_fov = std::cos(fov / 2 * (pif / 180));
  }
  for (int l = 0; l < 16; ++l) a.sf[l] = l < c->g.nlevels ? c->scale[l] : 0.0f;
  a.qx = (float*)d_qx; a.qy = (float*)d_qy; a.qr = (float*)d_qr; a.qmin = (int*)d_qmin; a.qmax = (int*)d_qmax;
  hipLaunchKernelGGL(k_project_last, dim3((n + 255) / 256), dim3(256), 0, c->stream, a);
  HIPCHK(hipGetLastError());
  return CMS_OK;
}
extern "C" int cms_rotation_filter_device(cms_ctx* c, int B, const void* d_mp_off, const void* d_last_angle, void* d_kp_mp, void* d_mp_match,
                                          void* d_n_matches, int check_orientation) {
  if (!c || B < 1 || !d_mp_off || !d_last_angle || !d_kp_mp || !d_mp_match) return cms_fail(CMS_ERR_ARG, "cms_rotation_filter_device: bad argument");
  HIPCHK(hipSetDevice(c->device));
  CmsRotFilterArgs a;
  a.mp_off = (const int*)d_mp_off; a.last_angle = (const float*)d_last_angle; a.kp = (const CmsKeyPoint*)c->d_kps; a.kp_mp = (int*)d_kp_mp;
  a.mp_match = (int*)d_mp_match; a.n_matches = (int*)d_n_matches; a.check_orientation = check_orientation; a.total = nullptr; a.cap = 0;
  hipLaunchKernelGGL(k_rot_filter, dim3(B), dim3(1024), 0, c->stream, a);
  HIPCHK(hipGetLastError());
  return CMS_OK;
}

extern "C" int cms_search_by_projection(cms_ctx* c, int b, const float* pose12, int nlast, const uint8_t* valid, const float* Xw, const int* octave,
                                        const float* angle, const uint8_t* mp_desc, float th, int check_orientation, int th_high, int nkp, int* kp_mp,
                                        int* match, int* n_matches) {
  if (!c || !pose12 || nlast < 0 || nkp < 0 || nkp > (c ? c->g.kp_cap : 0) || (nlast > 0 && (!valid || !Xw || !octave || !angle || !mp_desc || !match)) ||
      (nkp > 0 && !kp_mp))
    return cms_fail(CMS_ERR_ARG, "cms_search_by_projection: bad argument");
  if (b < 0 || b >= c->area_frames) return cms_fail(CMS_ERR_ARG, "cms_search_by_projection: no grid for this frame (cms_area_grid first)");
  if (c->g.kp_cap > CMS_TRACK_KPMAX) return cms_fail(CMS_ERR_UNSUPPORTED, "cms_search_by_projection: more than 4096 key points per frame");
  if (n_matches) *n_matches = 0;
  if (nlast == 0) return CMS_OK;
  for (int i = 0; i < nlast; ++i)
    if (valid[i] && (octave[i] < 0 || octave[i] >= c->g.nlevels)) return cms_fail(CMS_ERR_ARG, "cms_search_by_projection: octave out of range");
  HIPCHK(hipSetDevice(c->device));
  hipStream_t s = c->stream;
  const size_t n4 = (size_t)nlast * 4, kp4 = (size_t)c->g.kp_cap * 4;
  auto al = [](size_t v) { return (v + 255) & ~(size_t)255; };
  size_t o = 0;
  auto take = [&](size_t bytes) { const size_t at = o; o += al(bytes); return at; };
  const size_t o_pose = take(64), o_valid = take(nlast), o_xw = take(3 * n4), o_oct = take(n4), o_ang = take(n4), o_desc = take((size_t)nlast * 32),
               o_qf = take(n4), o_mpoff = take(16), o_kpmp = take(kp4);
  const size_t in_bytes = o;
  const size_t o_match = take(n4), o_nm = take(16), o_tot = take(16);
  const size_t out_begin = o_kpmp, out_bytes = o - o_kpmp;
  const size_t o_qx = take(n4), o_qy = take(n4), o_qr = take(n4), o_qmin = take(n4), o_qmax = take(n4), o_cnt = take(n4), o_off = take(n4 + 4);
  const size_t fixed = o;
  int cap = 64 * nlast + 1024;
  for (int attempt = 0; attempt < 2; ++attempt) {
    const size_t o_idx = fixed, o_pd = fixed + al((size_t)cap * 4);
    int rc = cms_scratch(c, o_pd + al((size_t)cap * 2));
    if (rc) return rc;
    rc = cms_hstage(c, std::max(in_bytes, out_begin + out_bytes));
    if (rc) return rc;
    uint8_t* p = (uint8_t*)c->d_match;
    uint8_t* h = c->h_stage;
    memcpy(h + o_pose, pose12, 48);
    memcpy(h + o_valid, valid, nlast); memcpy(h + o_xw, Xw, 3 * n4); memcpy(h + o_oct, octave, n4); memcpy(h + o_ang, angle, n4);
    memcpy(h + o_desc, mp_desc, (size_t)nlast * 32);
    { int* qf = reinterpret_cast<int*>(h + o_qf); for (int i = 0; i < nlast; ++i) qf[i] = b; }
    { int* mo = reinterpret_cast<int*>(h + o_mpoff); mo[0] = 0; mo[1] = nlast; }
    { int* km = reinterpret_cast<int*>(h + o_kpmp); for (int k = 0; k < c->g.kp_cap; ++k) km[k] = k < nkp ? kp_mp[k] : -1; }
    HIPCHK(hipMemcpyAsync(p, h, in_bytes, hipMemcpyHostToDevice, s));
    rc = cms_project_last_frame_device(c, nlast, nullptr, p + o_pose, p + o_valid, p + o_xw, p + o_oct, th, p + o_qx, p + o_qy, p + o_qr, p + o_qmin, p + o_qmax);
    if (rc) return rc;
    rc = cms_features_in_area_batch_device(c, nlast, p + o_qf, p + o_qx, p + o_qy, p + o_qr, p + o_qmin, p + o_qmax, p + o_cnt, p + o_off, p + o_idx, cap, p + o_tot);
    if (rc) return rc;
    CmsSearchLocalArgs a;
    a.mp_off = (const int*)(p + o_mpoff); a.mp_desc = (const uint4*)(p + o_desc); a.cand_off = (const int*)(p + o_off); a.cand_idx = (const int*)(p + o_idx);
    a.t_desc = (const uint4*)c->d_desc; a.kp = (const CmsKeyPoint*)c->d_kps; a.kp_cap = c->g.kp_cap;
    a.pair_dist = (uint16_t*)(p + o_pd); a.kp_mp = (int*)(p + o_kpmp) - (size_t)b * c->g.kp_cap; a.mp_match = (int*)(p + o_match); a.rounds = nullptr;
    a.nnratio = -1.0f; a.th_high = th_high; a.frame0 = b; a.total = (const int*)(p + o_tot); a.cap = cap;
    hipLaunchKernelGGL(k_search_local, dim3(1), dim3(1024), 0, s, a);
    CmsRotFilterArgs r;
    r.mp_off = (const int*)(p + o_mpoff); r.last_angle = (const float*)(p + o_ang); r.kp = (const CmsKeyPoint*)c->d_kps; r.kp_mp = a.kp_mp;
    r.mp_match = (int*)(p + o_match); r.n_matches = (int*)(p + o_nm); r.check_orientation = check_orientation; r.total = a.total; r.cap = cap;
    hipLaunchKernelGGL(k_rot_filter, dim3(1), dim3(1024), 0, s, r);
    HIPCHK(hipGetLastError());
    HIPCHK(hipMemcpyAsync(h + out_begin, p + out_begin, out_bytes, hipMemcpyDeviceToHost, s));
    HIPCHK(hipStreamSynchronize(s));
    const int tot = *reinterpret_cast<const int*>(h + o_tot);
    if (tot > cap) { cap = tot + 64; continue; }
    const int* m = reinterpret_cast<const int*>(h + o_match);
    if (nkp > 0) memcpy(kp_mp, h + o_kpmp, (size_t)nkp * 4);
    for (int i = 0; i < nlast; ++i) match[i] = m[i] >= 0 ? m[i] - b * c->g.kp_cap : -1;
    if (n_matches) *n_matches = *reinterpret_cast<const int*>(h + o_nm);
    return CMS_OK;
  }
  return cms_fail(CMS_ERR_OVERFLOW, "cms_search_by_projection: candidate lists kept growing");
}

extern "C" int cms_search_for_initialization(cms_ctx* c, int b2, int n1, const cms_keypoint* kps1, const uint8_t* desc1, float* prev_matched,
                                             int window_size, float nnratio, int check_orientation, int* matches12, int* n_matches) {
  if (!c || n1 < 0 || (n1 > 0 && (!kps1 || !desc1 || !prev_matched || !matches12)) || window_size < 0)
    return cms_fail(CMS_ERR_ARG, "cms_search_for_initialization: bad argument");
  if (b2 < 0 || b2 >= c->area_frames) return cms_fail(CMS_ERR_ARG, "cms_search_for_initialization: no grid for this frame (cms_area_grid first)");
  if (n_matches) *n_matches = 0;
  if (n1 == 0) return CMS_OK;
  HIPCHK(hipSetDevice(c->device));
  {
    static std::mutex mu;
    static bool done[64] = {false};
    std::lock_guard<std::mutex> lk(mu);
    if (c->device >= 0 && c->device < 64 && !done[c->device]) {
      HIPCHK(hipFuncSetAttribute((const void*)k_init_greedy, hipFuncAttributeMaxDynamicSharedMemorySize, 160 * 1024 - 1024));
      done[c->device] = true;
    }
  }
  const size_t lds = (size_t)c->g.kp_cap * 8;
  if (lds > 160 * 1024 - 1024) return cms_fail(CMS_ERR_UNSUPPORTED, "cms_search_for_initialization: too many key points per frame for the LDS tables");
  hipStream_t s = c->stream;
  std::vector<int> qi;
  for (int i = 0; i < n1; ++i) if (kps1[i].octave <= 0) qi.push_back(i);
  const int nq = (int)qi.size();
  for (int i = 0; i < n1; ++i) matches12[i] = -1;
  if (nq == 0) return CMS_OK;
  const size_t q4 = (size_t)nq * 4, n4 = (size_t)n1 * 4;
  auto al = [](size_t v) { return (v + 255) & ~(size_t)255; };
  size_t o = 0;
  auto take = [&](size_t bytes) { const size_t at = o; o += al(bytes); return at; };
  const size_t o_qi = take(q4), o_qx = take(q4), o_qy = take(q4), o_qr = take(q4), o_qmin = take(q4), o_qmax = take(q4), o_qf = take(q4),
               o_desc = take((size_t)n1 * 32), o_ang = take(n4), o_prev = take(2 * n4);
  const size_t in_bytes = o;
  const size_t o_m12 = take(n4), o_nm = take(16), o_tot = take(16);
  const size_t out_begin = o_prev, out_bytes = o - o_prev;
  const size_t o_bin = take(n1), o_cnt = take(q4), o_off = take(q4 + 4);
  const size_t fixed = o;
  int cap = 128 * nq + 4096;
  for (int attempt = 0; attempt < 2; ++attempt) {
    const size_t o_idx = fixed, o_pd = fixed + al((size_t)cap * 4);
    int rc = cms_scratch(c, o_pd + al((size_t)cap * 2));
    if (rc) return rc;
    rc = cms_hstage(c, std::max(in_bytes, out_begin + out_bytes));
    if (rc) return rc;
    uint8_t* p = (uint8_t*)c->d_match;
    uint8_t* h = c->h_stage;
    {
      int* hq = reinterpret_cast<int*>(h + o_qi); float* hx = reinterpret_cast<float*>(h + o_qx); float* hy = reinterpret_cast<float*>(h + o_qy);
      float* hr = reinterpret_cast<float*>(h + o_qr); int* hmin = reinterpret_cast<int*>(h + o_qmin); int* hmax = reinterpret_cast<int*>(h + o_qmax);
      int* hf = reinterpret_cast<int*>(h + o_qf);
      for (int q = 0; q < nq; ++q) {
        hq[q] = qi[q]; hx[q] = prev_matched[2 * qi[q]]; hy[q] = prev_matched[2 * qi[q] + 1]; hr[q] = (float)window_size; hmin[q] = 0; hmax[q] = 0; hf[q] = b2;
      }
      float* ha = reinterpret_cast<float*>(h + o_ang);
      for (int i = 0; i < n1; ++i) ha[i] = kps1[i].angle;
      memcpy(h + o_desc, desc1, (size_t)n1 * 32);
      memcpy(h + o_prev, prev_matched, 2 * n4);
    }
    HIPCHK(hipMemcpyAsync(p, h, in_bytes, hipMemcpyHostToDevice, s));
    rc = cms_features_in_area_batch_device(c, nq, p + o_qf, p + o_qx, p + o_qy, p + o_qr, p + o_qmin, p + o_qmax, p + o_cnt, p + o_off, p + o_idx, cap, p + o_tot);
    if (rc) return rc;
    CmsInitArgs a;
    a.nq = nq; a.q_i1 = (const int*)(p + o_qi); a.cand_off = (const int*)(p + o_off); a.cand_idx = (const int*)(p + o_idx);
    a.desc1 = (const uint4*)(p + o_desc); a.t_desc = (const uint4*)c->d_desc; a.kp2 = (const CmsKeyPoint*)c->d_kps; a.row0 = b2 * c->g.kp_cap; a.kp_cap = c->g.kp_cap;
    a.angle1 = (const float*)(p + o_ang); a.pair_dist = (uint16_t*)(p + o_pd);
    a.n1 = n1; a.matches12 = (int*)(p + o_m12); a.prev_matched = (float*)(p + o_prev); a.n_matches = (int*)(p + o_nm); a.bin_of = (int8_t*)(p + o_bin);
    a.nnratio = nnratio; a.check_orientation = check_orientation; a.total = (const int*)(p + o_tot); a.cap = cap;
    hipLaunchKernelGGL(k_init_dist, dim3(nq), dim3(64), 0, s, a);
    hipLaunchKernelGGL(k_init_greedy, dim3(1), dim3(64), lds, s, a);
    HIPCHK(hipGetLastError());
    HIPCHK(hipMemcpyAsync(h + out_begin, p + out_begin, out_bytes, hipMemcpyDeviceToHost, s));
    HIPCHK(hipStreamSynchronize(s));
    const int tot = *reinterpret_cast<const int*>(h + o_tot);
    if (tot > cap) { cap = tot + 64; continue; }
    memcpy(matches12, h + o_m12, n4);
    memcpy(prev_matched, h + o_prev, 2 * n4);
    if (n_matches) *n_matches = *reinterpret_cast<const int*>(h + o_nm);
    return CMS_OK;
  }
  return cms_fail(CMS_ERR_OVERFLOW, "cms_search_for_initialization: candidate lists kept growing");
}
```

### cubemapslam_amd/csrc/cms_area_kernels.hip

```cpp
#include <hip/hip_runtime.h>
#include <stdint.h>
#include "cms_types.h"
#include "cms_area_table.h"

#define CMS_AREA_CELLS (5 * CMS_AREA_G * CMS_AREA_G)
#define CMS_AREA_MAXKP 16383

extern "C" __global__ void __launch_bounds__(1024)
k_area_grid(const CmsKeyPoint* __restrict__ kps, const int* __restrict__ kp_cnt, int kp_cap, int F, float inv,
            uint16_t* __restrict__ sorted_idx, int* __restrict__ cell_start, int* __restrict__ n_valid_out) {
  extern __shared__ uint32_t area_lds[];
  uint32_t* keys = area_lds;
  uint32_t* sorted = area_lds + (kp_cap + 1);
  __shared__ int s_nvalid;
  const int b = blockIdx.x, tid = threadIdx.x, T = blockDim.x;
  const int n = min(kp_cnt[b], min(kp_cap, CMS_AREA_MAXKP));
  const CmsKeyPoint* kp = kps + (size_t)b * kp_cap;
  if (tid == 0) s_nvalid = 0;
  __syncthreads();
  for (int i = tid; i < n; i += T) {
    const float x = kp[i].x, y = kp[i].y;
    const double fi = (double)(x / (float)F), fj = (double)(y / (float)F);
    int f = -1;
    if (fi >= 0 && fi < 1 && fj >= 1 && fj < 2) f = 1;
    else if (fi >= 1 && fi < 2 && fj >= 0 && fj < 1) f = 3;
    else if (fi >= 1 && fi < 2 && fj >= 1 && fj < 2) f = 0;
    else if (fi >= 1 && fi < 2 && fj >= 2 && fj < 3) f = 4;
    else if (fi >= 2 && fi < 3 && fj >= 1 && fj < 2) f = 2;
    uint32_t key = 0xFFFFC000u | (uint32_t)i;
    if (f >= 0) {
      const int px = (int)(x * inv) % CMS_AREA_G, py = (int)(y * inv) % CMS_AREA_G;
      key = ((uint32_t)((f * CMS_AREA_G + px) * CMS_AREA_G + py) << 14) | (uint32_t)i;
      atomicAdd(&s_nvalid, 1);
    }
    keys[i] = key;
  }
  __syncthreads();
  for (int i = tid; i < n; i += T) {
    const uint32_t k = keys[i];
    int r = 0;
    for (int q = 0; q < n; ++q) r += keys[q] < k ? 1 : 0;
    sorted[r] = k;
  }
  __syncthreads();
  const int nv = s_nvalid;
  uint16_t* si = sorted_idx + (size_t)b * kp_cap;
  int* cs = cell_start + (size_t)b * (CMS_AREA_CELLS + 1);
  for (int s = tid; s < nv; s += T) {
    const int c = (int)(sorted[s] >> 14), prev = s ? (int)(sorted[s - 1] >> 14) : -1;
    si[s] = (uint16_t)(sorted[s] & 0x3FFFu);
    for (int cc = prev + 1; cc <= c; ++cc) cs[cc] = s;
  }
  const int last = nv ? (int)(sorted[nv - 1] >> 14) : -1;
  for (int cc = last + 1 + tid; cc <= CMS_AREA_CELLS; cc += T) cs[cc] = nv;
  if (tid == 0) n_valid_out[b] = nv;
}

struct CmsAreaArgs {
  const CmsKeyPoint* kp;
  const uint16_t* sorted_idx;
  const int* cell_start;
  const float* qx; const float* qy; const float* qr; const int* qmin; const int* qmax;
  const int* q_frame;
  int kp_cap;
  int nq, F; float inv;
  int* cnt;
  const int* off;
  int* idx; int cap; int idx_base;
  int* tmp;
};
#define CMS_AREA_TMP 8

#define CMS_AREA_QL 8
extern "C" __global__ void __launch_bounds__(256) k_area_query(CmsAreaArgs a, int pass) {
  const int gl = threadIdx.x & (CMS_AREA_QL - 1);
  const int q = (blockIdx.x * blockDim.x + threadIdx.x) / CMS_AREA_QL;
  const int qq = q < a.nq ? q : 0;
  const float x = a.qx[qq], y = a.qy[qq], r = a.qr[qq];
  const bool live = q < a.nq && !(r < 0.0f);
  const int minLevel = a.qmin[qq], maxLevel = a.qmax[qq];
  const bool check = (minLevel > 0) || (maxLevel >= 0);
  CmsAreaRectI rc[3];
  const int base = (pass && live) ? a.off[qq] : 0;
  bool copied = false;
  if (pass && a.tmp && live) {
    const int c = a.cnt[qq];
    if (c <= CMS_AREA_TMP) {
      if (gl < c && base + gl < a.cap) a.idx[base + gl] = a.tmp[(size_t)qq * CMS_AREA_TMP + gl];
      copied = true;
    }
  }
  const int nr = (live && !copied) ? cms_area_rects(x, y, r, a.F, a.inv, rc) : 0;
  int n = 0;
  int* tmpq = (!pass && a.tmp) ? a.tmp + (size_t)qq * CMS_AREA_TMP : nullptr;
  const int fr = a.q_frame ? a.q_frame[qq] : 0;
  const CmsKeyPoint* kp = a.kp + (size_t)fr * a.kp_cap;
  const uint16_t* sorted_idx = a.sorted_idx + (size_t)fr * a.kp_cap;
  const int* cell_start = a.cell_start + (size_t)fr * (CMS_AREA_CELLS + 1);
  const int idx_base = a.idx_base + (a.q_frame ? fr * a.kp_cap : 0);
  for (int k = 0; k < 3; ++k) {
    const bool has = k < nr;
    const int x0 = has ? max(0, rc[k].x0) : 0, x1 = has ? min(CMS_AREA_G - 1, rc[k].x1) : -1;
    const int y0 = has ? max(0, rc[k].y0) : 0, y1 = has ? min(CMS_AREA_G - 1, rc[k].y1) : -1;
    const int face = has ? rc[k].face : 0;
    const int ncol = (x1 >= x0 && y1 >= y0) ? x1 - x0 + 1 : 0;
    int maxcol = ncol;
    for (int o = 32; o > 0; o >>= 1) maxcol = max(maxcol, __shfl_xor(maxcol, o));
    for (int cb = 0; cb < maxcol; cb += CMS_AREA_QL) {
      const int ix = x0 + cb + gl;
      const bool col = cb + gl < ncol;
      int s0 = 0, s1 = 0;
      if (col) {
        const int c0 = (face * CMS_AREA_G + ix) * CMS_AREA_G + y0;
        s0 = cell_start[c0]; s1 = cell_start[c0 + (y1 - y0) + 1];
      }
      int h0 = 0, h1 = 0, h2 = 0, h3 = 0;
      int nh = 0;
      for (int s = s0; s < s1; ++s) {
        const int j = sorted_idx[s];
        const CmsKeyPoint p = kp[j];
        if (check) {
          if (p.octave < minLevel) continue;
          if (maxLevel >= 0 && p.octave > maxLevel) continue;
        }
        if (fabsf(p.x - x) < r && fabsf(p.y - y) < r) {
          if (nh == 0) h0 = j; else if (nh == 1) h1 = j; else if (nh == 2) h2 = j; else if (nh == 3) h3 = j;
          ++nh;
        }
      }
      int incl = nh;
#pragma unroll
      for (int o = 1; o < CMS_AREA_QL; o <<= 1) { const int t = __shfl_up(incl, o, CMS_AREA_QL); if (gl >= o) incl += t; }
      const int tot = __shfl(incl, CMS_AREA_QL - 1, CMS_AREA_QL);
      if (tmpq && nh > 0) {
        int w = n + incl - nh;
        if (w < CMS_AREA_TMP) {
          if (nh <= 4) {
            tmpq[w] = idx_base + h0;
            if (nh > 1 && w + 1 < CMS_AREA_TMP) tmpq[w + 1] = idx_base + h1;
            if (nh > 2 && w + 2 < CMS_AREA_TMP) tmpq[w + 2] = idx_base + h2;
            if (nh > 3 && w + 3 < CMS_AREA_TMP) tmpq[w + 3] = idx_base + h3;
          } else {
            for (int s = s0; s < s1 && w < CMS_AREA_TMP; ++s) {
              const int j = sorted_idx[s];
              const CmsKeyPoint p = kp[j];
              if (check && (p.octave < minLevel || (maxLevel >= 0 && p.octave > maxLevel))) continue;
              if (fabsf(p.x - x) < r && fabsf(p.y - y) < r) { tmpq[w] = idx_base + j; ++w; }
            }
          }
        }
      }
      if (pass && nh > 0) {
        int w = base + n + incl - nh;
        if (nh <= 4) {
          if (w < a.cap) a.idx[w] = idx_base + h0;
          if (nh > 1 && w + 1 < a.cap) a.idx[w + 1] = idx_base + h1;
          if (nh > 2 && w + 2 < a.cap) a.idx[w + 2] = idx_base + h2;
          if (nh > 3 && w + 3 < a.cap) a.idx[w + 3] = idx_base + h3;
        } else {
          for (int s = s0; s < s1; ++s) {
            const int j = sorted_idx[s];
            const CmsKeyPoint p = kp[j];
            if (check && (p.octave < minLevel || (maxLevel >= 0 && p.octave > maxLevel))) continue;
            if (fabsf(p.x - x) < r && fabsf(p.y - y) < r) { if (w < a.cap) a.idx[w] = idx_base + j; ++w; }
          }
        }
      }
      n += tot;
    }
  }
  if (!pass && q < a.nq && gl == 0) a.cnt[q] = n;
}

extern "C" __global__ void __launch_bounds__(1024) k_area_blocksum(const int* __restrict__ cnt, int nq, int* __restrict__ bsum) {
  __shared__ int part[16];
  const int i = blockIdx.x * 1024 + threadIdx.x, lane = threadIdx.x & 63, wv = threadIdx.x >> 6;
  int v = i < nq ? cnt[i] : 0;
  for (int o = 32; o > 0; o >>= 1) v += __shfl_xor(v, o);
  if (lane == 0) part[wv] = v;
  __syncthreads();
  if (threadIdx.x == 0) { int t = 0; for (int w = 0; w < 16; ++w) t += part[w]; bsum[blockIdx.x] = t; }
}
extern "C" __global__ void __launch_bounds__(1024) k_area_scan(const int* __restrict__ cnt, int nq, const int* __restrict__ bsum,
                                                                int* __restrict__ off, int* __restrict__ total) {
  __shared__ int part[16];
  __shared__ int s_before;
  const int tid = threadIdx.x, lane = tid & 63, wv = tid >> 6;
  int before = 0;
  for (int b = tid; b < (int)blockIdx.x; b += 1024) before += bsum[b];
  for (int o = 32; o > 0; o >>= 1) before += __shfl_xor(before, o);
  if (lane == 0) part[wv] = before;
  __syncthreads();
  if (tid == 0) { int t = 0; for (int w = 0; w < 16; ++w) t += part[w]; s_before = t; }
  __syncthreads();
  const int i = blockIdx.x * 1024 + tid;
  const int v = i < nq ? cnt[i] : 0;
  int incl = v;
#pragma unroll
  for (int o = 1; o < 64; o <<= 1) { const int t = __shfl_up(incl, o); if (lane >= o) incl += t; }
  __syncthreads();
  if (lane == 63) part[wv] = incl;
  __syncthreads();
  int wbase = 0;
  for (int w = 0; w < wv; ++w) wbase += part[w];
  const int mine = s_before + wbase + incl;
  if (i < nq) off[i + 1] = mine;
  if (i == 0) off[0] = 0;
  if (i == nq - 1 && total) *total = mine;
}
```

### cubemapslam_amd/csrc/cms_area_table.h

```cpp
#ifndef CMS_AREA_TABLE_H
#define CMS_AREA_TABLE_H
#include <stdint.h>

#define CMS_AREA_G 50
#ifdef CMS_AREA_HOST_EMU
#include <math.h>
#define AREA_TAB static const
#define AREA_FN inline
#else
#define AREA_TAB static const __device__
#define AREA_FN __device__ __forceinline__
#endif

enum { AV_A, AV_B, AV_C, AV_D,
       AV_BO, AV_DO,
       AV_AU, AV_CU,
       AV_AN, AV_CN,
       AV_COUNT };
#define AE_Z 0
#define AE_G1 1
#define AE_GG 2
#define AE_V(v) (3 + (v))
#define AE_M(v) (3 + AV_COUNT + (v))

struct CmsAreaRect { int8_t face, x0, x1, y0, y1; };
struct CmsAreaCase { int8_t n; CmsAreaRect r[3]; };

#define AF 0
#define AL 1
#define AR 2
#define AU 3
#define AW 4
#define vA AE_V(AV_A)
#define vB AE_V(AV_B)
#define vC AE_V(AV_C)
#define vD AE_V(AV_D)
#define vBO AE_V(AV_BO)
#define vDO AE_V(AV_DO)
#define vAU AE_V(AV_AU)
#define vCU AE_V(AV_CU)
#define vAN AE_V(AV_AN)
#define vCN AE_V(AV_CN)
#define mA AE_M(AV_A)
#define mB AE_M(AV_B)
#define mC AE_M(AV_C)
#define mD AE_M(AV_D)
#define mBO AE_M(AV_BO)
#define mDO AE_M(AV_DO)
#define mAU AE_M(AV_AU)
#define mCU AE_M(AV_CU)
#define mAN AE_M(AV_AN)
#define mCN AE_M(AV_CN)
#define Z_ AE_Z
#define G1 AE_G1
#define GG AE_GG
#define NONE {0, 0, 0, 0, 0}

AREA_TAB CmsAreaCase kAreaXin[5][2] = {
   {{2, {{AF, vA, vB, vC, G1}, {AW, vA, vB, Z_, vDO}, NONE}}, {2, {{AU, vA, vB, vCU, G1}, {AF, vA, vB, Z_, vD}, NONE}}},
   {{2, {{AL, vA, vB, vC, G1}, {AW, Z_, vDO, mB, mA}, NONE}}, {2, {{AU, Z_, vCN, vA, vB}, {AL, vA, vB, Z_, vD}, NONE}}},
   {{2, {{AR, vA, vB, vC, G1}, {AW, mDO, G1, vA, vB}, NONE}}, {2, {{AU, vCU, G1, mB, mA}, {AR, vA, vB, Z_, vD}, NONE}}},
   {{2, {{AU, vA, vB, vC, G1}, {AF, vA, vB, Z_, vDO}, NONE}}, {1, {{AW, vA, vB, Z_, vD}, NONE, NONE}}},
   {{1, {{AW, vA, vB, vC, G1}, NONE, NONE}},                   {2, {{AF, vA, vB, vCU, G1}, {AW, vA, vB, Z_, vD}, NONE}}},
};
AREA_TAB CmsAreaCase kAreaYin[5][2] = {
   {{2, {{AF, vA, G1, vC, vD}, {AR, Z_, vBO, vC, vD}, NONE}}, {2, {{AL, vAU, G1, vC, vD}, {AF, Z_, vB, vC, vD}, NONE}}},
   {{2, {{AF, Z_, vBO, vC, vD}, {AL, vA, G1, vC, vD}, NONE}}, {1, {{AL, Z_, vB, vC, vD}, NONE, NONE}}},
   {{1, {{AR, vA, G1, vC, vD}, NONE, NONE}},                   {2, {{AF, vAU, G1, vC, vD}, {AR, Z_, vB, vC, vD}, NONE}}},
   {{2, {{AU, vA, G1, vC, vD}, {AR, mD, mC, Z_, vBO}, NONE}}, {2, {{AL, vC, vD, Z_, vAN}, {AU, Z_, vB, vC, vD}, NONE}}},
   {{2, {{AW, vA, G1, vC, vD}, {AR, vC, vD, mBO, GG}, NONE}}, {2, {{AL, mD, mC, vAU, G1}, {AW, Z_, vB, vC, vD}, NONE}}},
};
AREA_TAB CmsAreaCase kAreaCorner[5][4] = {
   {{3, {{AF, vA, G1, vC, G1}, {AR, Z_, vBO, vC, G1}, {AW, vA, G1, Z_, vDO}}},
               {3, {{AF, Z_, vB, vC, G1}, {AL, vAU, G1, vC, G1}, {AW, Z_, vB, Z_, vDO}}},
               {3, {{AF, vA, G1, Z_, vD}, {AR, Z_, vBO, Z_, vD}, {AU, vA, G1, mCU, G1}}},
               {3, {{AF, Z_, vB, Z_, vD}, {AL, mAU, G1, Z_, vD}, {AU, Z_, vB, mCU, G1}}}},
   {{3, {{AL, vA, G1, vC, G1}, {AF, Z_, vBO, vC, G1}, {AW, Z_, vDO, Z_, mA}}},
               {2, {{AL, Z_, vB, vC, G1}, {AW, Z_, vDO, mB, G1}, NONE}},
               {3, {{AL, vA, G1, Z_, vD}, {AF, Z_, vBO, Z_, vD}, {AU, Z_, vCN, vA, G1}}},
               {2, {{AL, Z_, vB, Z_, vD}, {AU, Z_, vCN, Z_, vD}, NONE}}},
   {{2, {{AR, vA, G1, vC, G1}, {AW, mDO, G1, vA, G1}, NONE}},
               {3, {{AR, Z_, vB, vC, G1}, {AF, mAN, G1, vC, G1}, {AW, mDO, G1, Z_, vB}}},
               {2, {{AR, vA, G1, Z_, vD}, {AU, mCN, G1, Z_, mA}, NONE}},
               {3, {{AR, Z_, vB, Z_, vD}, {AF, mAN, G1, Z_, vD}, {AU, mCN, G1, mB, G1}}}},
   {{3, {{AU, vA, G1, vC, G1}, {AR, Z_, mC, Z_, vBO}, {AF, vA, G1, Z_, vDO}}},
               {3, {{AU, Z_, vB, vC, G1}, {AL, vC, G1, Z_, vAN}, {AF, Z_, vB, Z_, vDO}}},
               {2, {{AU, vA, G1, Z_, vD}, {AR, mD, G1, Z_, vD}, NONE}},
               {2, {{AU, Z_, vB, Z_, vD}, {AL, Z_, vD, Z_, vAN}, NONE}}},
   {{2, {{AW, vA, G1, vC, G1}, {AR, vA, G1, mBO, G1}, NONE}},
               {2, {{AW, Z_, vB, vC, G1}, {AL, Z_, mC, mAU, G1}, NONE}},
               {3, {{AW, vA, G1, Z_, vD}, {AR, Z_, vD, mBO, GG}, {AF, vA, G1, mCN, G1}}},
               {3, {{AW, Z_, vB, Z_, vD}, {AL, mAN, G1, mAN, GG}, {AF, Z_, vB, mCN, G1}}}},
};
#undef AF
#undef AL
#undef AR
#undef AU
#undef AW
#undef NONE

struct CmsAreaRectI { int face, x0, x1, y0, y1; };

AREA_FN int cms_area_rects(float x, float y, float r, int F, float inv, CmsAreaRectI out[3]) {
  int face = -1;
  {
    const float i = x / (float)F, j = y / (float)F;
    if (i >= 0 && i < 1 && j >= 1 && j < 2) face = 1;
    else if (i >= 1 && i < 2 && j >= 0 && j < 1) face = 3;
    else if (i >= 1 && i < 2 && j >= 1 && j < 2) face = 0;
    else if (i >= 1 && i < 2 && j >= 2 && j < 3) face = 4;
    else if (i >= 2 && i < 3 && j >= 1 && j < 2) face = 2;
  }
  if (face < 0) return 0;
  const int cornerX = (int)x / F * F, cornerY = (int)y / F * F;
  const float xin = x - (float)cornerX, yin = y - (float)cornerY;
  const float xs = xin - r, xe = xin + r, ys = yin - r, ye = yin + r;
  const bool xu = xs < 0, xo = xe > (float)(F - 1), yu = ys < 0, yo = ye > (float)(F - 1);
  const bool xinf = !xo && !xu, yinf = !yo && !yu;
  const float Ff = (float)F;
  int v[AV_COUNT];
  v[AV_A] = (int)floorf(xs * inv); v[AV_B] = (int)floorf(xe * inv); v[AV_C] = (int)floorf(ys * inv); v[AV_D] = (int)floorf(ye * inv);
  v[AV_BO] = (int)floorf((xe - Ff) * inv); v[AV_DO] = (int)floorf((ye - Ff) * inv);
  v[AV_AU] = (int)floorf((xs + Ff) * inv); v[AV_CU] = (int)floorf((ys + Ff) * inv);
  v[AV_AN] = (int)floorf((-xs) * inv); v[AV_CN] = (int)floorf((-ys) * inv);
  const CmsAreaCase* cs;
  CmsAreaCase inside;
  if (xinf && yinf) {
    inside.n = 1;
    inside.r[0].face = (int8_t)face; inside.r[0].x0 = vA; inside.r[0].x1 = vB; inside.r[0].y0 = vC; inside.r[0].y1 = vD;
    cs = &inside;
  } else if (xinf) {
    cs = &kAreaXin[face][yo ? 0 : 1];
  } else if (yinf) {
    cs = &kAreaYin[face][xo ? 0 : 1];
  } else {
    int k;
    if (xo && yo) k = 0; else if (xu && yo) k = 1; else if (xo && yu) k = 2; else k = 3;
    cs = &kAreaCorner[face][k];
  }
  auto ev = [&](int e) -> int {
    if (e == AE_Z) return 0;
    if (e == AE_G1) return CMS_AREA_G - 1;
    if (e == AE_GG) return CMS_AREA_G;
    if (e < 3 + AV_COUNT) return v[e - 3];
    return CMS_AREA_G - v[e - 3 - AV_COUNT] - 1;
  };
  for (int k = 0; k < cs->n; ++k) {
    out[k].face = cs->r[k].face; out[k].x0 = ev(cs->r[k].x0); out[k].x1 = ev(cs->r[k].x1); out[k].y0 = ev(cs->r[k].y0); out[k].y1 = ev(cs->r[k].y1);
  }
  return cs->n;
}
#undef vA
#undef vB
#undef vC
#undef vD
#undef vBO
#undef vDO
#undef vAU
#undef vCU
#undef vAN
#undef vCN
#undef mA
#undef mB
#undef mC
#undef mD
#undef mBO
#undef mDO
#undef mAU
#undef mCU
#undef mAN
#undef mCN
#undef Z_
#undef G1
#undef GG
#endif
```

### cubemapslam_amd/csrc/cms_track_kernels.hip

```cpp
#include <hip/hip_runtime.h>
#include <stdint.h>

struct CmsFrustumArgs {
  const float* pose15;
  const int* mp_frame;
  int n;
  const float* P; const float* normal; const float* min_dist; const float* max_dist;
  float viewing_cos_limit, log_scale, th;
  int nlevels, F;
  int bounds_scaled;
  float sf[16];
  uint8_t* in_view; float* proj_x; float* proj_y; int* level; float* view_cos;
  float* qr; int* qmin; int* qmax;
};

__device__ __forceinline__ void track_distance_bounds(int scaled, float min_in, float max_in, float& minDistance, float& maxDistance, float& raw_max) {
  if (scaled) {
    maxDistance = max_in; minDistance = min_in;
    float r = (float)((double)max_in / (double)1.2f);
    const float lo = __uint_as_float(__float_as_uint(r) - 1u), hi = __uint_as_float(__float_as_uint(r) + 1u);
    if (r > 0.0f && __fmul_rn(1.2f, lo) == max_in) r = lo;
    else if (__fmul_rn(1.2f, r) != max_in && __fmul_rn(1.2f, hi) == max_in) r = hi;
    raw_max = r;
  } else {
    raw_max = max_in; maxDistance = __fmul_rn(1.2f, max_in); minDistance = __fmul_rn(0.8f, min_in);
  }
}

__host__ __device__ __forceinline__ int track_rays_to_cubemap(int F, float x, float y, float z, float& up, float& vp) {
  const double f = F / 2.0;
  float lx, ly, lz, ox, oy;
  int face;
  if (z > 0 && x / z <= 1 && x / z >= -1 && y / z <= 1 && y / z >= -1) { face = 0; lx = x; ly = y; lz = z; ox = (float)F; oy = (float)F; }
  else if (x > 0 && y / x <= 1 && y / x >= -1 && z / x <= 1 && z / x >= -1) { face = 2; lx = -z; ly = y; lz = x; ox = (float)(2 * F); oy = (float)F; }
  else if (x < 0 && y / (-x) <= 1 && y / (-x) >= -1 && z / (-x) <= 1 && z / (-x) >= -1) { face = 1; lx = z; ly = y; lz = -x; ox = 0.0f; oy = (float)F; }
  else if (y > 0 && x / y <= 1 && x / y >= -1 && z / y <= 1 && z / y >= -1) { face = 4; lx = x; ly = -z; lz = y; ox = (float)F; oy = (float)(2 * F); }
  else if (y < 0 && x / (-y) <= 1 && x / (-y) >= -1 && z / (-y) <= 1 && z / (-y) >= -1) { face = 3; lx = x; ly = z; lz = -y; ox = (float)F; oy = 0.0f; }
  else { up = -1.0f; vp = -1.0f; return -1; }
  up = (float)((double)lx * f / (double)lz + f);
  vp = (float)((double)ly * f / (double)lz + f);
  if (up < 0 || up >= F || vp < 0 || vp >= F) return -1;
  if (ox != 0.0f) up += ox;
  if (oy != 0.0f) vp += oy;
  return face;
}

extern "C" __global__ void __launch_bounds__(256) k_in_frustum(CmsFrustumArgs a) {
  const int i = blockIdx.x * blockDim.x + threadIdx.x;
  if (i >= a.n) return;
  const float* ps = a.pose15 + 15 * (size_t)(a.mp_frame ? a.mp_frame[i] : 0);
  uint8_t vis = 0; float u = -1.0f, v = -1.0f, vc = 0.0f; int lvl = -1;
  const float px = a.P[3 * (size_t)i], py = a.P[3 * (size_t)i + 1], pz = a.P[3 * (size_t)i + 2];
  float Pc[3];
#pragma unroll
  for (int r = 0; r < 3; ++r) {
    float t = __fmul_rn(ps[3 * r], px);
    t = __fadd_rn(t, __fmul_rn(ps[3 * r + 1], py));
    t = __fadd_rn(t, __fmul_rn(ps[3 * r + 2], pz));
    Pc[r] = (float)((double)t * 1.0 + (double)ps[9 + r] * 1.0);
  }
  const float mnMax = (float)(3 * a.F);
  do {
    const int face = track_rays_to_cubemap(a.F, Pc[0], Pc[1], Pc[2], u, v);
    if (face < 0) break;
    if (u < 0.0f || u > mnMax || v < 0.0f || v > mnMax) break;
    float maxd, maxDistance, minDistance;
    track_distance_bounds(a.bounds_scaled, a.min_dist[i], a.max_dist[i], minDistance, maxDistance, maxd);
    const float PO[3] = {__fsub_rn(px, ps[12]), __fsub_rn(py, ps[13]), __fsub_rn(pz, ps[14])};
    double s = 0;
#pragma unroll
    for (int k = 0; k < 3; ++k) s = __dadd_rn(s, __dmul_rn((double)PO[k], (double)PO[k]));
    const float dist = (float)sqrt(s);
    if (dist < minDistance || dist > maxDistance) break;
    double d = 0;
#pragma unroll
    for (int k = 0; k < 3; ++k) d = __dadd_rn(d, __dmul_rn((double)PO[k], (double)a.normal[3 * (size_t)i + k]));
    vc = (float)(d / (double)dist);
    if (vc < a.viewing_cos_limit) break;
    const float ratio = maxd / dist;
    const float lg = (float)log((double)ratio);
    int ns = (int)ceilf(lg / a.log_scale);
    if (ns < 0) ns = 0; else if (ns >= a.nlevels) ns = a.nlevels - 1;
    lvl = ns; vis = 1;
  } while (false);
  if (!vis) { u = -1.0f; v = -1.0f; vc = 0.0f; }
  a.in_view[i] = vis; a.proj_x[i] = u; a.proj_y[i] = v; a.level[i] = lvl; a.view_cos[i] = vc;
  if (a.qr) {
    float r = (double)vc > 0.998 ? 2.5f : 4.0f;
    if (a.th != 1.0f) r = __fmul_rn(r, a.th);
    a.qr[i] = vis ? __fmul_rn(r, a.sf[lvl]) : -1.0f;
    a.qmin[i] = lvl - 1; a.qmax[i] = lvl;
  }
}

struct CmsSearchLocalArgs {
  const int* mp_off;
  const uint4* mp_desc;
  const int* cand_off; const int* cand_idx;
  const uint4* t_desc; const CmsKeyPoint* kp; int kp_cap;
  uint16_t* pair_dist;
  int* kp_mp;
  int* mp_match;
  int* rounds;
  float nnratio; int th_high;
  int frame0;
  const int* total; int cap;
};

__device__ __forceinline__ int track_hamming256(const uint4& a0, const uint4& a1, const uint4& b0, const uint4& b1) {
  return __popc(a0.x ^ b0.x) + __popc(a0.y ^ b0.y) + __popc(a0.z ^ b0.z) + __popc(a0.w ^ b0.w) +
         __popc(a1.x ^ b1.x) + __popc(a1.y ^ b1.y) + __popc(a1.z ^ b1.z) + __popc(a1.w ^ b1.w);
}

#define CMS_TRACK_KPMAX 4096
extern "C" __global__ void __launch_bounds__(1024) k_search_local(CmsSearchLocalArgs a) {
  __shared__ int min_open[CMS_TRACK_KPMAX];
  const int f = blockIdx.x, tid = threadIdx.x, nt = blockDim.x;
  if (a.total && *a.total > a.cap) return;
  const int m0 = a.mp_off[f], m1 = a.mp_off[f + 1];
  const int row0 = (f + a.frame0) * a.kp_cap;
  {
    const int sub = tid & 3;
    for (int i = m0 + (tid >> 2); i < m1; i += nt >> 2) {
      const int c0 = a.cand_off[i], c1 = a.cand_off[i + 1];
      if (c0 == c1) continue;
      const uint4 q0 = a.mp_desc[2 * (size_t)i], q1 = a.mp_desc[2 * (size_t)i + 1];
      for (int c = c0 + sub; c < c1; c += 4) {
        const size_t row = (size_t)a.cand_idx[c];
        a.pair_dist[c] = (uint16_t)track_hamming256(q0, q1, a.t_desc[2 * row], a.t_desc[2 * row + 1]);
      }
    }
  }
  for (int i = m0 + tid; i < m1; i += nt) a.mp_match[i] = a.cand_off[i] == a.cand_off[i + 1] ? -1 : -2;
  __syncthreads();
  int round = 0;
  for (;;) {
    for (int k = tid; k < a.kp_cap; k += nt) min_open[k] = 0x7FFFFFFF;
    __syncthreads();
    for (int i = m0 + tid; i < m1; i += nt) {
      if (a.mp_match[i] != -2) continue;
      for (int c = a.cand_off[i]; c < a.cand_off[i + 1]; ++c) {
        const int row = a.cand_idx[c];
        if (a.kp_mp[row] < 0) atomicMin(&min_open[row - row0], i);
      }
    }
    __syncthreads();
    int open = 0;
    for (int i = m0 + tid; i < m1; i += nt) {
      if (a.mp_match[i] != -2) continue;
      bool ok = true;
      for (int c = a.cand_off[i]; c < a.cand_off[i + 1] && ok; ++c) {
        const int row = a.cand_idx[c];
        ok = a.kp_mp[row] >= 0 || min_open[row - row0] == i;
      }
      if (ok) a.mp_match[i] = -3; else ++open;
    }
    __syncthreads();
    for (int i = m0 + tid; i < m1; i += nt) {
      if (a.mp_match[i] != -3) continue;
      int bestDist = 256, bestLevel = -1, bestDist2 = 256, bestLevel2 = -1, bestRow = -1;
      for (int c = a.cand_off[i]; c < a.cand_off[i + 1]; ++c) {
        const int row = a.cand_idx[c];
        if (a.kp_mp[row] >= 0) continue;
        const int dist = a.pair_dist[c];
        if (dist < bestDist) { bestDist2 = bestDist; bestDist = dist; bestLevel2 = bestLevel; bestLevel = a.kp[row].octave; bestRow = row; }
        else if (dist < bestDist2) { bestLevel2 = a.kp[row].octave; bestDist2 = dist; }
      }
      int m = -1;
      const bool ratio_ok = a.nnratio < 0.0f || !(bestLevel == bestLevel2 && (float)bestDist > __fmul_rn(a.nnratio, (float)bestDist2));
      if (bestDist <= a.th_high && ratio_ok) m = bestRow;
      if (m >= 0) a.kp_mp[m] = i;
      a.mp_match[i] = m;
    }
    ++round;
    if (__syncthreads_count(open > 0) == 0) break;
  }
  if (a.rounds && tid == 0) a.rounds[f] = round;
}


struct CmsProjectLastArgs {
  const float* pose12;
  const int* q_frame;
  int n; const uint8_t* valid; const float* Xw; const int* oct;
  float th, cos_fov; int F; float sf[16];
  float* qx; float* qy; float* qr; int* qmin; int* qmax;
};
extern "C" __global__ void __launch_bounds__(256) k_project_last(CmsProjectLastArgs a) {
  const int i = blockIdx.x * blockDim.x + threadIdx.x;
  if (i >= a.n) return;
  float u = -1.0f, v = -1.0f, r = -1.0f;
  const int o = a.oct[i];
  if (a.valid[i]) {
    const float* ps = a.pose12 + 12 * (size_t)(a.q_frame ? a.q_frame[i] : 0);
    const float p0 = a.Xw[3 * (size_t)i], p1 = a.Xw[3 * (size_t)i + 1], p2 = a.Xw[3 * (size_t)i + 2];
    float xc[3];
#pragma unroll
    for (int k = 0; k < 3; ++k) {
      float t = __fmul_rn(ps[3 * k], p0);
      t = __fadd_rn(t, __fmul_rn(ps[3 * k + 1], p1));
      t = __fadd_rn(t, __fmul_rn(ps[3 * k + 2], p2));
      xc[k] = (float)((double)t * 1.0 + (double)ps[9 + k] * 1.0);
    }
    if (!(xc[2] < a.cos_fov) && track_rays_to_cubemap(a.F, xc[0], xc[1], xc[2], u, v) >= 0) r = __fmul_rn(a.th, a.sf[o & 15]);
  }
  a.qx[i] = u; a.qy[i] = v; a.qr[i] = r; a.qmin[i] = o - 1; a.qmax[i] = o + 1;
}

__device__ __forceinline__ int track_rot_bin(float angle_ref, float angle_cur) {
  float rot = __fsub_rn(angle_ref, angle_cur);
  if (rot < 0.0f) rot = __fadd_rn(rot, 360.0f);
  int bin = (int)roundf(__fmul_rn(rot, 1.0f / 12));
  return bin == 30 ? 0 : bin;
}
__device__ __forceinline__ void track_three_maxima(const int* hist, int* keep) {
  int max1 = 0, max2 = 0, max3 = 0, i1 = -1, i2 = -1, i3 = -1;
  for (int b = 0; b < 30; ++b) {
    const int s = hist[b];
    if (s > max1) { max3 = max2; max2 = max1; max1 = s; i3 = i2; i2 = i1; i1 = b; }
    else if (s > max2) { max3 = max2; max2 = s; i3 = i2; i2 = b; }
    else if (s > max3) { max3 = s; i3 = b; }
  }
  if ((float)max2 < __fmul_rn(0.1f, (float)max1)) { i2 = -1; i3 = -1; } else if ((float)max3 < __fmul_rn(0.1f, (float)max1)) i3 = -1;
  keep[0] = i1; keep[1] = i2; keep[2] = i3;
}

struct CmsRotFilterArgs {
  const int* mp_off; const float* last_angle; const CmsKeyPoint* kp; int* kp_mp; int* mp_match; int* n_matches; int check_orientation;
  const int* total; int cap;
};
extern "C" __global__ void __launch_bounds__(1024) k_rot_filter(CmsRotFilterArgs a) {
  __shared__ int hist[32];
  __shared__ int keep[3];
  __shared__ int s_n;
  const int f = blockIdx.x, tid = threadIdx.x, nt = blockDim.x;
  if (a.total && *a.total > a.cap) return;
  const int m0 = a.mp_off[f], m1 = a.mp_off[f + 1];
  if (tid < 32) hist[tid] = 0;
  if (tid == 0) s_n = 0;
  __syncthreads();
  auto bin_of = [&](int i, int row) { return track_rot_bin(a.last_angle[i], a.kp[row].angle); };
  for (int i = m0 + tid; i < m1; i += nt) {
    const int row = a.mp_match[i];
    if (row >= 0 && a.check_orientation) atomicAdd(&hist[bin_of(i, row)], 1);
  }
  __syncthreads();
  if (tid == 0) track_three_maxima(hist, keep);
  __syncthreads();
  int mine = 0;
  for (int i = m0 + tid; i < m1; i += nt) {
    const int row = a.mp_match[i];
    if (row < 0) continue;
    if (a.check_orientation) {
      const int b = bin_of(i, row);
      if (b != keep[0] && b != keep[1] && b != keep[2]) { a.kp_mp[row] = -1; a.mp_match[i] = -1; continue; }
    }
    ++mine;
  }
  atomicAdd(&s_n, mine);
  __syncthreads();
  if (tid == 0 && a.n_matches) a.n_matches[f] = s_n;
}

struct CmsInitArgs {
  int nq; const int* q_i1;
  const int* cand_off; const int* cand_idx;
  const uint4* desc1; const uint4* t_desc; const CmsKeyPoint* kp2; int row0, kp_cap;
  const float* angle1; uint16_t* pair_dist;
  int n1; int* matches12; float* prev_matched; int* n_matches; int8_t* bin_of;
  float nnratio; int check_orientation;
  const int* total; int cap;
};
extern "C" __global__ void __launch_bounds__(64) k_init_dist(CmsInitArgs a) {
  if (*a.total > a.cap) return;
  const int q = blockIdx.x, i1 = a.q_i1[q];
  const uint4 q0 = a.desc1[2 * (size_t)i1], q1 = a.desc1[2 * (size_t)i1 + 1];
  for (int c = a.cand_off[q] + threadIdx.x; c < a.cand_off[q + 1]; c += 64) {
    const size_t row = (size_t)a.cand_idx[c];
    a.pair_dist[c] = (uint16_t)track_hamming256(q0, q1, a.t_desc[2 * row], a.t_desc[2 * row + 1]);
  }
}
extern "C" __global__ void __launch_bounds__(64) k_init_greedy(CmsInitArgs a) {
  extern __shared__ int init_lds[];
  __shared__ int hist[32];
  int* md = init_lds;
  int* m21 = init_lds + a.kp_cap;
  const int lane = threadIdx.x;
  for (int k = lane; k < a.kp_cap; k += 64) { md[k] = 0x7FFFFFFF; m21[k] = -1; }
  if (lane < 32) hist[lane] = 0;
  for (int i = lane; i < a.n1; i += 64) { a.matches12[i] = -1; a.bin_of[i] = -1; }
  __syncthreads();
  if (*a.total > a.cap) return;
  int nmatches = 0;
  for (int q = 0; q < a.nq; ++q) {
    const int i1 = a.q_i1[q], c0 = a.cand_off[q], c1 = a.cand_off[q + 1];
    if (c0 == c1) continue;
    unsigned k1 = 0xFFFFFFFFu, k2 = 0xFFFFFFFFu;
    for (int c = c0 + lane; c < c1; c += 64) {
      const int i2 = a.cand_idx[c] - a.row0;
      const unsigned dist = a.pair_dist[c];
      if (md[i2] <= (int)dist) continue;
      const unsigned key = (dist << 16) | (unsigned)(c - c0);
      if (key < k1) { k2 = k1; k1 = key; } else if (key < k2) k2 = key;
    }
    for (int o = 32; o > 0; o >>= 1) {
      const unsigned o1 = __shfl_xor(k1, o), o2 = __shfl_xor(k2, o);
      const unsigned lo = min(k1, o1), hi = max(k1, o1);
      k2 = min(hi, min(k2, o2)); k1 = lo;
    }
    if (k1 == 0xFFFFFFFFu) continue;
    const int bestDist = (int)(k1 >> 16);
    const int bestDist2 = k2 == 0xFFFFFFFFu ? 0x7FFFFFFF : (int)(k2 >> 16);
    if (bestDist <= 50 && (float)bestDist < __fmul_rn((float)bestDist2, a.nnratio)) {
      const int row = a.cand_idx[c0 + (int)(k1 & 0xFFFFu)], i2 = row - a.row0;
      const int old = m21[i2];
      __syncthreads();
      if (lane == 0) {
        if (old >= 0) a.matches12[old] = -1;
        a.matches12[i1] = i2; m21[i2] = i1; md[i2] = bestDist;
        if (a.check_orientation) {
          float rot = __fsub_rn(a.angle1[i1], a.kp2[row].angle);
          if (rot < 0.0f) rot = __fadd_rn(rot, 360.0f);
          int bin = (int)roundf(__fmul_rn(rot, 1.0f / 12));
          if (bin == 30) bin = 0;
          ++hist[bin];
          a.bin_of[i1] = (int8_t)bin;
        }
      }
      nmatches += old >= 0 ? 0 : 1;
      __syncthreads();
// ... 29 lines not shown
```

### cubemapslam_amd/host/batch_driver.cpp

```cpp
#include <atomic>
#include <chrono>
#include <condition_variable>
#include <cstring>
#include <deque>
#include <functional>
#include <future>
#include <memory>
#include <mutex>
#include <stdexcept>
#include <string>
#include <thread>
#include <pthread.h>
#include <vector>

#include "cubemapslam_hip.h"

#define CBD_MAX_GROUPS 8

extern "C" {
typedef struct cbd_frame_set {
  const void* d_frames;
  int nq; const void* d_mm_frame; const void* d_mm_pose; const void* d_mm_valid; const void* d_mm_xw; const void* d_mm_oct; void* d_mm_q[5];
  void* d_cnt; void* d_off; void* d_idx; int cand_cap; void* d_tot;
  const void* d_mm_mpoff; const void* d_mm_desc; void* d_mm_pd; void* d_mm_match; const void* d_mm_ang; void* d_mm_n;
// ... 42 lines not shown
    cv_.notify_one();
    th_.join();
  }
  template <class F> auto submit(F f) -> std::future<decltype(f())> {
    auto task = std::make_shared<std::packaged_task<decltype(f())()>>(std::move(f));
    auto fut = task->get_future();
    { std::lock_guard<std::mutex> lk(mu_); q_.push_back([task]() { (*task)(); }); }
    cv_.notify_one();
    return fut;
  }
 private:
  void run() {
    for (;;) {
      std::function<void()> job;
      {
        std::unique_lock<std::mutex> lk(mu_);
        cv_.wait(lk, [this]() { return stop_ || !q_.empty(); });
        if (q_.empty()) return;
        job = std::move(q_.front()); q_.pop_front();
      }
      job();
    }
  }
  std::mutex mu_; std::condition_variable cv_; std::deque<std::function<void()>> q_; bool stop_ = false;
  std::thread th_;
};

double now_ms() { return std::chrono::duration<double, std::milli>(std::chrono::steady_clock::now().time_since_epoch()).count(); }
struct Fail : std::runtime_error { using std::runtime_error::runtime_error; };
void chk(int rc, const char* what) { if (rc < 0) throw Fail(std::string(what) + ": " + cms_last_error()); }

typedef std::vector<cms_ba*> Windows;
struct BaJobResult { std::future<void> finish; double ms = 0; long n_new = 0; };
}

struct cbd {
  cbd_plan p;
  std::vector<std::unique_ptr<Worker>> mapping, ba, builder, finisher;
  std::mutex stats_mu; cbd_stats st;
  std::mutex store_mu[CBD_MAX_GROUPS];
  std::mutex wb_mu; int wb_pending[CBD_MAX_GROUPS];
  std::deque<std::pair<int, std::vector<std::future<Windows>>>> queue;
  std::vector<std::future<BaJobResult>> inflight;
  std::vector<std::future<void>> reads;
  std::vector<double> poses7; std::vector<uint8_t> pose_out; std::vector<int> pose_inl; std::vector<cms_pose_stats> pose_st;
  std::vector<std::vector<double>> rd_poses, rd_pts; std::vector<std::vector<uint8_t>> rd_flags;
  std::string err;
};

namespace {
Windows build_group(cbd* d, int set, int g) {
  const cbd_group& G = d->p.groups[g];
  const double t0 = now_ms();
  Windows w((size_t)G.nwin, nullptr);
  chk(cms_ba_create_many(w.data(), G.nwin, d->p.device, G.windows[set], d->p.create_threads), "cms_ba_create_many");
  for (cms_ba* b : w) chk(cms_ba_set_stream(b, G.ba_stream), "cms_ba_set_stream");
  std::lock_guard<std::mutex> lk(d->stats_mu);
  d->st.create_ms_sum += now_ms() - t0; d->st.create_windows += G.nwin;
  return w;
}
void submit_windows(cbd* d, int set) {
  std::vector<std::future<Windows>> futs;
  for (int g = 0; g < d->p.ngroups; ++g) futs.push_back(d->builder[(size_t)g]->submit([d, set, g]() { return build_group(d, set, g); }));
  d->queue.emplace_back(set, std::move(futs));
}
void apply_write_backs(cbd* d, int g) {
  const cbd_group& G = d->p.groups[g];
  for (;;) {
    { std::lock_guard<std::mutex> lk(d->wb_mu); if (d->wb_pending[g] <= 0) return; --d->wb_pending[g]; }
    const double t0 = now_ms();
    chk(cms_kfstore_update_poses(G.store, G.n_upd, G.upd_slots, G.upd_R, G.upd_t, G.upd_Ow), "cms_kfstore_update_poses");
    std::lock_guard<std::mutex> lk(d->stats_mu);
    d->st.upd_ms_sum += now_ms() - t0; ++d->st.upd_calls;
  }
}
long mapping_job(cbd* d, int g) {
  const cbd_group& G = d->p.groups[g];
  long n_new = 0;
  {
    std::lock_guard<std::mutex> lock(d->store_mu[g]);
    if (d->p.mapping_full) apply_write_backs(d, g);
    const double t0 = now_ms();
    chk(cms_kfstore_create_new_map_points(G.store, G.njobs, G.cur_slot, G.neigh_off, G.neigh_slot, 0, G.cap, G.n_new, G.o_neigh, G.o_idx1, G.o_idx2, G.o_x3d),
        "cms_kfstore_create_new_map_points");
    for (int j = 0; j < G.njobs; ++j) n_new += G.n_new[j];
    std::lock_guard<std::mutex> lk(d->stats_mu);
    d->st.tri_ms_sum += now_ms() - t0; ++d->st.tri_calls;
  }
  if (d->p.mapping_full) {
    const double t0 = now_ms();
    {
      std::lock_guard<std::mutex> lock(d->store_mu[g]);
      chk(cms_kfstore_fuse_search_sets(G.store, G.nsets, G.set_off, G.pos, G.normal, G.min_d, G.max_d, G.desc, G.nfjobs, G.job_slot, G.job_set, G.skip, G.th,
                                       G.best_idx, G.best_dist), "cms_kfstore_fuse_search_sets");
    }
    std::lock_guard<std::mutex> lk(d->stats_mu);
    d->st.fuse_ms_sum += now_ms() - t0; ++d->st.fuse_calls;
  }
  return n_new;
}
void finish_job(cbd* d, int g, Windows w) {
  const int n = (int)w.size();
  std::vector<double*> pp((size_t)n), pq((size_t)n); std::vector<uint8_t*> pf((size_t)n);
  const cbd_group& G = d->p.groups[g];
  size_t op = 0, oq = 0, of = 0;
  for (int i = 0; i < n; ++i) {
    const cms_ba_window& W0 = G.windows[0][i]; const cms_ba_window& W1 = G.windows[1][i];
    const size_t K = (size_t)std::max(W0.K, W1.K), P = (size_t)std::max(W0.P, W1.P), E = (size_t)std::max(W0.E, W1.E);
    pp[(size_t)i] = d->rd_poses[(size_t)g].data() + op; pq[(size_t)i] = d->rd_pts[(size_t)g].data() + oq; pf[(size_t)i] = d->rd_flags[(size_t)g].data() + of;
    op += 7 * K; oq += 3 * P; of += E;
  }
  chk(cms_ba_read_many(w.data(), n, pp.data(), pq.data(), pf.data()), "cms_ba_read_many");
  if (d->p.mapping_full) { std::lock_guard<std::mutex> lk(d->wb_mu); ++d->wb_pending[g]; }
  for (cms_ba* b : w) cms_ba_destroy(b);
}
BaJobResult ba_job(cbd* d, int g, std::shared_ptr<std::future<Windows>> wf, std::shared_ptr<std::future<long>> tri) {
  BaJobResult r;
  const double t0 = now_ms();
  Windows w = wf->get();
  const double t1 = now_ms();
  chk(cms_ba_profile_kernel(w[0], 3), "cms_ba_profile_kernel");
  r.n_new = tri->get();
  const double t2 = now_ms();
  std::vector<cms_ba_stats> stats(w.size());
  chk(cms_ba_optimize_many(w.data(), (int)w.size(), 5, 10, nullptr, stats.data()), "cms_ba_optimize_many");
  const double t3 = now_ms();
  double ms = 0; long nl = 0;
  chk(cms_ba_profile_get(w[0], &ms, &nl), "cms_ba_profile_get");
  r.finish = d->finisher[(size_t)g]->submit([d, g, w]() { finish_job(d, g, w); });
  r.ms = now_ms() - t0;
  std::lock_guard<std::mutex> lk(d->stats_mu);
  d->st.schur_ms += ms; d->st.schur_launches += nl;
  d->st.wait_windows_ms += t1 - t0; d->st.wait_tri_ms += t2 - t1; d->st.optimize_ms += t3 - t2;
  d->st.ba_ms_sum += r.ms; ++d->st.ba_jobs;
  return r;
}
void collect(cbd* d, std::vector<std::future<BaJobResult>>& ths) {
  std::vector<BaJobResult> res;
  for (auto& f : ths) res.push_back(f.get());
  if (res.empty()) return;
  for (auto& f : d->reads) f.get();
  d->reads.clear();
  long n_new = 0;
  for (auto& r : res) { d->reads.push_back(std::move(r.finish)); n_new += r.n_new; }
  std::lock_guard<std::mutex> lk(d->stats_mu);
  d->st.new_map_points_last_step = n_new;
}
void tracking(cbd* d, const cbd_frame_set& S) {
  cms_ctx* c = d->p.ctx; const int B = d->p.B;
  chk(cms_area_grid(c, B), "cms_area_grid");
  chk(cms_stream_copy_device(c, S.d_kpmp, S.d_kpmp0, S.kpmp_bytes), "cms_stream_copy_device");
  chk(cms_project_last_frame_device(c, S.nq, S.d_mm_frame, S.d_mm_pose, S.d_mm_valid, S.d_mm_xw, S.d_mm_oct, 15.0f, S.d_mm_q[0], S.d_mm_q[1], S.d_mm_q[2],
                                    S.d_mm_q[3], S.d_mm_q[4]), "cms_project_last_frame_device");
  chk(cms_features_in_area_batch_device(c, S.nq, S.d_mm_frame, S.d_mm_q[0], S.d_mm_q[1], S.d_mm_q[2], S.d_mm_q[3], S.d_mm_q[4], S.d_cnt, S.d_off, S.d_idx,
                                        S.cand_cap, S.d_tot), "cms_features_in_area_batch_device");
  chk(cms_search_local_points_device(c, B, S.d_mm_mpoff, S.d_mm_desc, S.d_off, S.d_idx, S.d_mm_pd, -1.0f, 100, S.d_kpmp, S.d_mm_match, nullptr),
      "cms_search_local_points_device");
  chk(cms_rotation_filter_device(c, B, S.d_mm_mpoff, S.d_mm_ang, S.d_kpmp, S.d_mm_match, S.d_mm_n, 1), "cms_rotation_filter_device");
  chk(cms_is_in_frustum_device(c, S.n_mp, S.d_lm_frame, S.d_lm_pose, S.d_lm_in[0], S.d_lm_in[1], S.d_lm_in[2], S.d_lm_in[3], 0.5f, 1.0f, S.d_lm_vis, S.d_lm_f[0],
                               S.d_lm_f[1], S.d_lm_i[0], S.d_lm_f[2], S.d_lm_f[3], S.d_lm_i[1], S.d_lm_i[2]), "cms_is_in_frustum_device");
  chk(cms_features_in_area_batch_device(c, S.n_mp, S.d_lm_frame, S.d_lm_f[0], S.d_lm_f[1], S.d_lm_f[3], S.d_lm_i[1], S.d_lm_i[2], S.d_lm_i[3], S.d_lm_off,
                                        S.d_lm_idx, S.lm_cap, S.d_lm_tot), "cms_features_in_area_batch_device");
  chk(cms_search_local_points_device(c, B, S.d_lm_mpoff, S.d_lm_desc, S.d_lm_off, S.d_lm_idx, S.d_lm_pd, 0.8f, 100, S.d_kpmp, S.d_lm_i[4], nullptr),
      "cms_search_local_points_device");
}
void one_step(cbd* d, int i) {
  const cbd_plan& p = d->p;
  const cbd_frame_set& S = p.sets[i & 1];
  chk(cms_pose_launch(p.po), "cms_pose_launch");
  chk(cms_frames_process_device(p.ctx, S.d_frames, p.B), "cms_frames_process_device");
  auto cur = std::move(d->queue.front()); d->queue.pop_front();
  submit_windows(d, d->queue.empty() ? (cur.first ^ 1) : (d->queue.back().first ^ 1));
  std::vector<std::future<BaJobResult>> ths;
  for (int g = 0; g < p.ngroups; ++g) {
    auto tri = std::make_shared<std::future<long>>(d->mapping[(size_t)g]->submit([d, g]() { return mapping_job(d, g); }));
    auto wf = std::make_shared<std::future<Windows>>(std::move(cur.second[(size_t)g]));
    ths.push_back(d->ba[(size_t)g]->submit([d, g, wf, tri]() { return ba_job(d, g, wf, tri); }));
  }
  tracking(d, S);
  if (p.mapping_full) {
    const double t0 = now_ms();
    for (int g = 0; g < p.ngroups; ++g) chk(cms_kfstore_put_from_frames(p.groups[g].store, p.ctx, S.put_n[g], S.put_items[g]), "cms_kfstore_put_from_frames");
    std::lock_guard<std::mutex> lk(d->stats_mu);
    d->st.put_ms_sum += now_ms() - t0; ++d->st.put_calls;
  }
  chk(cms_frames_sync(p.ctx), "cms_frames_sync");
  chk(cms_pose_fetch(p.po, d->poses7.data(), d->pose_out.data(), d->pose_inl.data(), d->pose_st.data()), "cms_pose_fetch");
  if (p.step_done) p.step_done(p.user, i, d->poses7.data(), p.B);
  float ms7[7];
  if (cms_profile_get(p.ctx, ms7) == CMS_OK) for (int k = 0; k < 7; ++k) d->st.stage_ms[k] += ms7[k];
  std::vector<std::future<BaJobResult>> prev = std::move(d->inflight);
  d->inflight = std::move(ths);
  collect(d, prev);
  ++d->st.steps;
}
}

extern "C" {
static thread_local std::string g_cbd_err;
const char* cbd_last_error() { return g_cbd_err.c_str(); }
#define CBD_TRY(...) try { __VA_ARGS__ } catch (const std::exception& e) { g_cbd_err = e.what(); return -1; }

cbd* cbd_create(const cbd_plan* plan, int max_pose_edges) {
  if (!plan || plan->ngroups < 1 || plan->ngroups > CBD_MAX_GROUPS || plan->B < 1) { g_cbd_err = "cbd_create: bad plan"; return nullptr; }
  cbd* d = new cbd;
  d->p = *plan;
  std::memset(&d->st, 0, sizeof(d->st));
  for (int g = 0; g < plan->ngroups; ++g) {
    const std::string gs = std::to_string(g);
    d->mapping.emplace_back(new Worker("cbd-map" + gs)); d->ba.emplace_back(new Worker("cbd-ba" + gs)); d->builder.emplace_back(new Worker("cbd-build" + gs));
    d->finisher.emplace_back(new Worker("cbd-finish" + gs));
    d->wb_pending[g] = 0;
    size_t np = 0, nq = 0, nf = 0;
    for (int i = 0; i < plan->groups[g].nwin; ++i) {
      const cms_ba_window& W0 = plan->groups[g].windows[0][i]; const cms_ba_window& W1 = plan->groups[g].windows[1][i];
      np += 7 * (size_t)std::max(W0.K, W1.K); nq += 3 * (size_t)std::max(W0.P, W1.P); nf += (size_t)std::max(W0.E, W1.E);
    }
    d->rd_poses.emplace_back(np); d->rd_pts.emplace_back(nq); d->rd_flags.emplace_back(nf);
  }
  d->poses7.assign(7 * (size_t)plan->B, 0.0); d->pose_out.assign((size_t)std::max(max_pose_edges, 1), 0); d->pose_inl.assign((size_t)plan->B, 0);
  d->pose_st.resize((size_t)plan->B);
  return d;
}
int cbd_begin(cbd* d) { CBD_TRY(for (int a = 0; a < std::max(1, d->p.ahead); ++a) submit_windows(d, a & 1); return 0;) }
int cbd_steps(cbd* d, int first, int n) { CBD_TRY(for (int i = 0; i < n; ++i) one_step(d, first + i); return 0;) }
int cbd_collect_inflight(cbd* d) { CBD_TRY(std::vector<std::future<BaJobResult>> prev = std::move(d->inflight); d->inflight.clear(); collect(d, prev); return 0;) }
int cbd_finish(cbd* d) {
  CBD_TRY(
    for (auto& f : d->reads) f.get();
    d->reads.clear();
    if (d->p.mapping_full)
      for (int g = 0; g < d->p.ngroups; ++g) { std::lock_guard<std::mutex> lock(d->store_mu[g]); apply_write_backs(d, g); }
    return 0;)
}
int cbd_drain(cbd* d) {
  CBD_TRY(
    while (!d->queue.empty()) {
      for (auto& f : d->queue.front().second) { Windows w = f.get(); for (cms_ba* b : w) cms_ba_destroy(b); }
      d->queue.pop_front();
    }
    return 0;)
}
void cbd_sizes(int* out4) { out4[0] = (int)sizeof(cbd_frame_set); out4[1] = (int)sizeof(cbd_group); out4[2] = (int)sizeof(cbd_plan); out4[3] = (int)sizeof(cbd_stats); }
void cbd_stats_get(cbd* d, cbd_stats* out, int reset) {
  std::lock_guard<std::mutex> lk(d->stats_mu);
  if (out) *out = d->st;
  if (reset) std::memset(&d->st, 0, sizeof(d->st));
}
void cbd_destroy(cbd* d) {
  if (!d) return;
  try { cbd_collect_inflight(d); cbd_finish(d); cbd_drain(d); } catch (...) {}
  delete d;
}
}
```

### include/cubemapslam_hip.h

```cpp
#ifndef CUBEMAPSLAM_HIP_H
#define CUBEMAPSLAM_HIP_H
#include <stddef.h>
#include <stdint.h>
#ifdef __cplusplus
extern "C" {
#endif

#define CMS_OK 0
#define CMS_ERR_ARG (-1)
#define CMS_ERR_HIP (-2)
#define CMS_ERR_UNSUPPORTED (-3)
#define CMS_ERR_OVERFLOW (-4)
#define CMS_ERR_NO_DEVICE (-5)

enum { CMS_FACE_UNKNOWN = -1, CMS_FACE_FRONT = 0, CMS_FACE_LEFT = 1, CMS_FACE_RIGHT = 2, CMS_FACE_UPPER = 3, CMS_FACE_LOWER = 4 };

typedef struct {
  double c, d, e, u0, v0;
  double invpol[12];
  double pol[5];
  int Iw, Ih;
  int face;
  double fov_deg;
} cms_camera;

typedef struct { int nfeatures; float scale_factor; int nlevels; int ini_th_fast; int min_th_fast; } cms_orb_params;

typedef struct { float x, y, size, angle, response; int octave; } cms_keypoint;

typedef struct {
  int W, F, nlevels, kp_cap, max_batch;
  int level_w[12], level_h[12], level_quota[12], level_cells[12];
  float scale[12], inv_scale[12], sigma2[12], inv_sigma2[12];
  size_t pyramid_bytes_per_frame, candidate_entries_per_frame;
  int fisheye_stride;
} cms_geometry;

typedef struct cms_ctx cms_ctx;

const char* cms_last_error(void);
int cms_device_count(void);

int cms_ctx_create(cms_ctx** out, int device, const cms_camera* cam, const cms_orb_params* orb, int max_batch);
void cms_ctx_destroy(cms_ctx* ctx);
int cms_ctx_geometry(const cms_ctx* ctx, cms_geometry* out);
void* cms_ctx_stream(cms_ctx* ctx);

int cms_remap(cms_ctx* ctx, const uint8_t* fisheye, int fstride, uint8_t* cubemap, int cstride);
int cms_set_mask(cms_ctx* ctx, const uint8_t* mask, int mstride);
int cms_set_gaussian_mode(cms_ctx* ctx, int column_mode);
int cms_extract(cms_ctx* ctx, const uint8_t* cubemap, int cstride, cms_keypoint* kps, uint8_t* desc, int cap, int* n);
int cms_remap_extract(cms_ctx* ctx, const uint8_t* fisheye, int fstride, cms_keypoint* kps, uint8_t* desc, int cap, int* n);
int cms_remap_extract_rays(cms_ctx* ctx, const uint8_t* fisheye, int fstride, cms_keypoint* kps, uint8_t* desc, float* rays, int cap, int* n);
int cms_frames_rays(cms_ctx* ctx, void** d_rays);
int cms_frames_fetch_rays(cms_ctx* ctx, int b, float* rays, int cap, int* n);

void* cms_frames_input(cms_ctx* ctx);
int cms_frames_upload(cms_ctx* ctx, const uint8_t* fisheye, int fstride, size_t frame_pitch, int B);
int cms_frames_upload_async(cms_ctx* ctx, const uint8_t* fisheye, int fstride, size_t frame_pitch, int B);
int cms_frames_upload_wait(cms_ctx* ctx);
int cms_stream_wait_extracted(cms_ctx* ctx, void* hip_stream);
int cms_frames_upload_device(cms_ctx* ctx, const void* d_src, int B);
int cms_stream_copy_device(cms_ctx* ctx, void* d_dst, const void* d_src, size_t bytes);
int cms_host_alloc(void** out, size_t bytes);
void cms_host_free(void* p);
int cms_frames_process(cms_ctx* ctx, int B, int from_fisheye);
int cms_frames_process_device(cms_ctx* ctx, const void* d_src, int B);
int cms_frames_sync(cms_ctx* ctx);
int cms_frames_results(cms_ctx* ctx, void** d_kps, void** d_desc, void** d_counts);
int cms_frames_fetch(cms_ctx* ctx, int b, cms_keypoint* kps, uint8_t* desc, int cap, int* n);

typedef struct { uint16_t tx, ty, x0, y0, nd, rows, flags, pad; } cms_remap_tile;
int cms_remap_lut_host(const cms_camera* cam, uint32_t* lut, int lut_stride);
int cms_remap_tiles_host(const cms_camera* cam, const uint32_t* lut, int lut_stride, int tile_w, int tile_h, int lds_budget,
                         cms_remap_tile* out, int cap, int* n_live, int* n_all, int* lds_bytes);

int cms_debug_lut(cms_ctx* ctx, uint32_t* out, int* stride);
int cms_debug_cubemap(cms_ctx* ctx, int b, uint8_t* dst, int dstride);
int cms_debug_level(cms_ctx* ctx, int b, int level, uint8_t* dst, int dstride);
int cms_debug_candidates(cms_ctx* ctx, int b, int level, int* xys, int cap, int* n);
int cms_debug_distributed(cms_ctx* ctx, int b, int level, int* xys, int cap, int* n);

int cms_profile_enable(cms_ctx* ctx, int on);
int cms_profile_get(cms_ctx* ctx, float* ms7);

int cms_hamming_best2(cms_ctx* ctx, const uint8_t* qdesc, int nq, const uint8_t* tdesc, int nt, const int* cand_off,
                      const int* cand_idx, const int* t_level, const uint8_t* t_excluded, int* best_idx, int* best_dist,
                      int* best_level, int* second_dist, int* second_level);
int cms_hamming_best2_device(cms_ctx* ctx, const void* qdesc, const void* q_row, int nq, const void* tdesc, const void* cand_off,
                             const void* cand_idx, const void* t_level, const void* t_excluded, void* best_idx,
                             void* best_dist, void* best_level, void* second_dist, void* second_level);
int cms_hamming_matrix(cms_ctx* ctx, const uint8_t* a, int na, const uint8_t* b, int nb, uint16_t* out);

typedef struct cms_ba cms_ba;
typedef struct {
  int iterations_done[2];
  double chi2_initial[2], chi2_final[2], lambda_final[2];
  int n_outliers_mid, n_outliers_final;
} cms_ba_stats;
int cms_ba_create(cms_ba** out, int device, int K, const double* poses, const uint8_t* fixed, int P, const double* points,
                  int E, const int* e_pose, const int* e_point, const double* e_obs, const double* e_invsig2,
                  const int8_t* e_face, double fx, double fy, double cx, double cy);
typedef struct cms_ba_window {
  int K; const double* poses; const uint8_t* fixed; int P; const double* points; int E; const int* e_pose; const int* e_point;
  const double* e_obs; const double* e_invsig2; const int8_t* e_face; double fx, fy, cx, cy;
  int flags;
} cms_ba_window;
#define CMS_BA_INPUTS_PINNED 1
#define CMS_BA_PLAN_ON_DEVICE 2
int cms_ba_create_many(cms_ba** out, int n, int device, const cms_ba_window* windows, int threads);
int cms_ba_read_many(cms_ba** bas, int n, double** poses, double** points, uint8_t** outlier_flags);
int cms_ba_reset(cms_ba* ba);
int cms_ba_optimize(cms_ba* ba, int its_robust, int its_final, const volatile uint8_t* stop, cms_ba_stats* stats);
int cms_ba_optimize_many(cms_ba** bas, int n, int its_robust, int its_final, const volatile uint8_t* stop, cms_ba_stats* stats);
int cms_ba_read(cms_ba* ba, double* poses, double* points, uint8_t* outlier_flags);
void* cms_ba_stream(cms_ba* ba);
int cms_ba_set_stream(cms_ba* ba, void* hip_stream);
int cms_ba_debug_clocks(cms_ba* ba, long long* out16);
int cms_ba_profile_kernel(cms_ba* ba, int kernel_id);
int cms_ba_profile_get(cms_ba* ba, double* total_ms, long* launches);
int cms_ba_debug_compose(int K, const uint8_t* fixed, int P, int E, const int* e_pose, const int* e_point, int lookahead,
                         int* pinv, int* chunk_pt0, int* n_chunks, uint8_t* rank);
int cms_ba_debug_plan(int K, const uint8_t* fixed, int P, int E, const int* e_pose, const int* e_point, int* pinv, int* perm, uint32_t* info,
                      int* chunk_pt0, int* rm_chunk, uint32_t* run_lane, int* counts, uint32_t* run_mf, uint32_t* run_fl);
int cms_ba_debug_fetch_plan(cms_ba* ba, int* pinv, int* perm, uint32_t* info, int* pt_off, int* e_pose, int* e_point, int8_t* e_face, int* chunk_e0,
                            int* rm_chunk, uint32_t* rm_cost, uint32_t* run_mf, uint32_t* run_fl, int* counts);
int cms_ba_debug_plan_fast(int K, const uint8_t* fixed, int P, int E, const int* e_pose, const int* e_point, int* pinv, int* perm, uint32_t* info,
                           int* chunk_pt0, int* rm_chunk, int* counts, uint32_t* run_mf, uint32_t* run_fl);
int cms_ba_debug_run_fg(int K, const uint8_t* fixed, int P, int E, const int* e_pose, const int* e_point, int fast, uint32_t* run_fg, int* rm_cut, int* counts);
int cms_ba_debug_match(int which, int n, const int* slots, int np, int* choice_out);
void cms_ba_destroy(cms_ba* ba);
int cms_ba_pool_trim(int device, size_t* released);
int cms_ba_set_deterministic(int on);
int cms_ba_get_deterministic(void);
int cms_ba_run(int device, int K, double* poses, const uint8_t* fixed, int P, double* points, int E, const int* e_pose,
               const int* e_point, const double* e_obs, const double* e_invsig2, const int8_t* e_face, double fx, double fy,
               double cx, double cy, int its_robust, int its_final, const volatile uint8_t* stop, uint8_t* outlier_flags,
               cms_ba_stats* stats);
int cms_ba_linearize(int device, int K, const double* poses, const uint8_t* fixed, int P, const double* points, int E,
                     const int* e_pose, const int* e_point, const double* e_obs, const double* e_invsig2,
                     const int8_t* e_face, double fx, double fy, double cx, double cy, int robust, double huber_delta,
                     double* err, double* Hpp, double* bp, double* Hll, double* bl, double* Hpl, double* robust_chi2_sum);

int cms_area_set_keypoints(cms_ctx* ctx, int b, int n, const cms_keypoint* kps);
int cms_area_grid(cms_ctx* ctx, int B);
int cms_features_in_area(cms_ctx* ctx, int b, int nq, const float* qx, const float* qy, const float* qr, const int* min_level,
                         const int* max_level, int* cand_off, int* cand_idx, int cap, int* total);
int cms_features_in_area_device(cms_ctx* ctx, int b, int nq, const void* d_qx, const void* d_qy, const void* d_qr, const void* d_min_level,
                                const void* d_max_level, void* d_cnt_scratch, void* d_cand_off, void* d_cand_idx, int cap, int idx_base,
                                void* d_total);
int cms_features_in_area_batch_device(cms_ctx* ctx, int nq, const void* d_qframe, const void* d_qx, const void* d_qy, const void* d_qr,
                                      const void* d_min_level, const void* d_max_level, void* d_cnt_scratch, void* d_cand_off,
                                      void* d_cand_idx, int cap, void* d_total);

int cms_area_set_descriptors(cms_ctx* ctx, int b, int n, const uint8_t* desc);
int cms_set_distance_bounds_mode(cms_ctx* ctx, int scaled);
int cms_search_by_projection(cms_ctx* ctx, int b, const float* pose12, int nlast, const uint8_t* valid, const float* Xw, const int* octave,
                             const float* angle, const uint8_t* mp_desc, float th, int check_orientation, int th_high, int nkp, int* kp_mp,
                             int* match, int* n_matches);
int cms_search_for_initialization(cms_ctx* ctx, int b2, int n1, const cms_keypoint* kps1, const uint8_t* desc1, float* prev_matched,
                                  int window_size, float nnratio, int check_orientation, int* matches12, int* n_matches);
int cms_project_last_frame_device(cms_ctx* ctx, int n, const void* d_qframe, const void* d_pose12, const void* d_valid, const void* d_Xw,
                                  const void* d_oct, float th, void* d_qx, void* d_qy, void* d_qr, void* d_qmin, void* d_qmax);
int cms_rotation_filter_device(cms_ctx* ctx, int B, const void* d_mp_off, const void* d_last_angle, void* d_kp_mp, void* d_mp_match,
                               void* d_n_matches, int check_orientation);
int cms_search_local_points(cms_ctx* ctx, int b, const float* pose15, int nmp, const float* pos, const float* normal,
                            const float* min_dist, const float* max_dist, const uint8_t* mp_desc, float viewing_cos_limit, float th,
                            float nnratio, int th_high, int nkp, int* kp_mp, uint8_t* in_view, float* proj_x, float* proj_y, int* level,
                            float* view_cos, int* mp_match, int* n_matches, int* rounds);
int cms_is_in_frustum_device(cms_ctx* ctx, int nmp, const void* d_mp_frame, const void* d_pose15, const void* d_pos, const void* d_normal,
                             const void* d_min_dist, const void* d_max_dist, float viewing_cos_limit, float th, void* d_in_view,
                             void* d_proj_x, void* d_proj_y, void* d_level, void* d_view_cos, void* d_qr, void* d_qmin, void* d_qmax);
int cms_search_local_points_device(cms_ctx* ctx, int B, const void* d_mp_off, const void* d_mp_desc, const void* d_cand_off,
                                   const void* d_cand_idx, void* d_pair_dist, float nnratio, int th_high, void* d_kp_mp, void* d_mp_match,
                                   void* d_rounds);

typedef struct {
  int n; const cms_keypoint* kps; const uint8_t* desc; const float* rays; const int* mp;
  float Rcw[9], tcw[3], Ow[3];
  int nnodes; const int* node_id; const int* node_off; const int* node_feat;
  float median_depth;
} cms_keyframe;
int cms_create_new_map_points(cms_ctx* ctx, int njobs, const cms_keyframe* cur, const int* neigh_off, const cms_keyframe* neigh,
                              int check_orientation, int cap_per_job, int* n_new, int* out_neigh, int* out_idx1, int* out_idx2,
                              float* out_x3d);
int cms_search_for_triangulation(cms_ctx* ctx, const cms_keyframe* kf1, const cms_keyframe* kf2, const float* E12, int check_orientation,
                                 int* matches12, int* n_matches);
typedef struct cms_kfstore cms_kfstore;
int cms_kfstore_create(cms_kfstore** out, cms_ctx* ctx, int max_keyframes, int max_features, int max_nodes);
void cms_kfstore_destroy(cms_kfstore* st);
int cms_kfstore_put(cms_kfstore* st, int slot, const cms_keyframe* kf);
int cms_kfstore_update(cms_kfstore* st, int slot, const float* Rcw, const float* tcw, const float* Ow, const float* median_depth, const int* mp);
int cms_kfstore_put_from_frame(cms_kfstore* st, int slot, cms_ctx* src, int b, int n, const float* Rcw, const float* tcw, const float* Ow, float median_depth,
                               const int* mp, int nnodes, const int* node_id, const int* node_off, const int* node_feat);
typedef struct {
  int slot, b, n;
  const float* Rcw; const float* tcw; const float* Ow; float median_depth;
  const int* mp; int nnodes; const int* node_id; const int* node_off; const int* node_feat;
} cms_kf_from_frame;
int cms_kfstore_put_from_frames(cms_kfstore* st, cms_ctx* src, int n_items, const cms_kf_from_frame* items);
int cms_kfstore_update_poses(cms_kfstore* st, int n, const int* slots, const float* Rcw, const float* tcw, const float* Ow);
int cms_kfstore_debug_fetch(cms_kfstore* st, int slot, cms_keypoint* kps, uint8_t* desc, float* rays, int* mp, int* feat_node, uint16_t* sorted,
                            int* node_id, int* node_off, int* node_feat, int* cell_start, uint32_t* header, int* misc);
int cms_kfstore_fuse_search(cms_kfstore* st, int njobs, const int* job_slot, const int* mp_off, const uint8_t* skip, const float* pos,
                            const float* normal, const float* min_dist, const float* max_dist, const uint8_t* mp_desc, float th, int* best_idx,
                            int* best_dist);
int cms_kfstore_fuse_search_sets(cms_kfstore* st, int nsets, const int* set_off, const float* pos, const float* normal, const float* min_dist,
                                 const float* max_dist, const uint8_t* mp_desc, int njobs, const int* job_slot, const int* job_set, const uint8_t* skip,
                                 float th, int* best_idx, int* best_dist);
int cms_kfstore_create_new_map_points(cms_kfstore* st, int njobs, const int* cur_slot, const int* neigh_off, const int* neigh_slot,
                                      int check_orientation, int cap_per_job, int* n_new, int* out_neigh, int* out_idx1, int* out_idx2,
                                      float* out_x3d);
int cms_distinctive_descriptors(cms_ctx* ctx, int npts, const int* obs_off, const uint8_t* desc, int* best_idx);
int cms_update_normal_and_depth(cms_ctx* ctx, int npts, const int* obs_off, const float* pos, const float* obs_Ow, const float* ref_Ow,
                                const int* ref_level, float* normal, float* min_dist, float* max_dist);
int cms_fuse_search(cms_ctx* ctx, int b, const float* pose15, int nmp, const uint8_t* skip, const float* pos, const float* normal,
                    const float* min_dist, const float* max_dist, const uint8_t* mp_desc, float th, int* best_idx, int* best_dist);

int cms_search_by_bow(cms_ctx* ctx, int b, int n, int nnodes, const int* node_id, const int* node_off, const int* node_feat,
                      const cms_keyframe* kf, const uint8_t* kf_skip, float nnratio, int check_orientation,
                      int* kf_idx , int* n_matches);
typedef struct {
  int slot;
  int b, n;
  int nnodes; const int* node_id; const int* node_off; const int* node_feat;
  const uint8_t* kf_skip;
} cms_bow_job;
int cms_kfstore_search_by_bow(cms_kfstore* st, cms_ctx* src, int njobs, const cms_bow_job* jobs, float nnratio,
                              int check_orientation, int* kf_idx , int* n_matches );

typedef struct cms_pose cms_pose;
typedef struct { int rounds, n_bad; int iterations_done[4]; } cms_pose_stats;
int cms_pose_create(cms_pose** out, int device, int max_frames, int max_edges);
void cms_pose_destroy(cms_pose* p);
void* cms_pose_stream(cms_pose* p);
int cms_pose_optimize_batch(cms_pose* p, int nf, const int* edge_off, const double* Xw, const double* obs_uv, const double* inv_sigma2,
                            const int8_t* face, double fx, double fy, double cx, double cy, double* poses7, uint8_t* outlier,
                            int* n_inliers, cms_pose_stats* stats);
int cms_pose_upload(cms_pose* p, int nf, const int* edge_off, const double* Xw, const double* obs_uv, const double* inv_sigma2,
                    const int8_t* face, double fx, double fy, double cx, double cy, const double* poses7);
int cms_pose_launch(cms_pose* p);
int cms_pose_fetch(cms_pose* p, double* poses7, uint8_t* outlier, int* n_inliers, cms_pose_stats* stats);
int cms_pose_optimize(int device, int n, const double* Xw, const double* obs_uv, const double* inv_sigma2, const int8_t* face,
                      double fx, double fy, double cx, double cy, double* pose7, uint8_t* outlier, int* n_inliers, cms_pose_stats* stats);

#ifdef __cplusplus
}
#endif
#endif
```

Measured before the change: 24220.

## Fuse area query with Hamming distance into single window-search kernel for tracking

Replaces the two-pass features-in-area batch query plus separate search kernel with a fused k_track_windows kernel. It walks grid cells once, writes up to eight candidates per query into fixed slots together with their precomputed Hamming distances, and spills larger sets to an atomically allocated overflow buffer. A slot-aware greedy matching kernel then reads from both the slots and the overflow, and resets a double-buffered counter for the next call. The aim is to cut kernel launches, the count/scan/fill passes and the separate descriptor-distance work in the tracking path. The cost is extra slot buffers and atomics, and the old path stays available through CMS_TRACK_FUSED=0.

```diff
diff --git a/cubemapslam_amd/api.py b/cubemapslam_amd/api.py
--- a/cubemapslam_amd/api.py
+++ b/cubemapslam_amd/api.py
@@ -113,6 +113,8 @@
         L.cms_rotation_filter_device.argtypes = [C.c_void_p, C.c_int] + [C.c_void_p] * 5 + [C.c_int]
         L.cms_is_in_frustum_device.argtypes = [C.c_void_p, C.c_int] + [C.c_void_p] * 6 + [C.c_float, C.c_float] + [C.c_void_p] * 8
         L.cms_search_local_points_device.argtypes = [C.c_void_p, C.c_int] + [C.c_void_p] * 5 + [C.c_float, C.c_int] + [C.c_void_p] * 3
+        L.cms_search_windows_device.argtypes = ([C.c_void_p, C.c_int, C.c_int] + [C.c_void_p] * 8 + [C.c_float, C.c_int] + [C.c_void_p] * 7 +
+                                                [C.c_int, C.c_void_p])
         L.cms_create_new_map_points.argtypes = [C.c_void_p, C.c_int, C.c_void_p, C.c_void_p, C.c_void_p, C.c_int, C.c_int] + [C.c_void_p] * 5
         L.cms_kfstore_create.argtypes = [C.c_void_p, C.c_void_p, C.c_int, C.c_int, C.c_int]
         L.cms_kfstore_destroy.argtypes = [C.c_void_p]
@@ -463,6 +465,13 @@
         _chk(lib().cms_search_local_points_device(self.h, B, v(d_mp_off), v(d_mp_desc), v(d_cand_off), v(d_cand_idx), v(d_pair_dist), nnratio,
                                                   th_high, v(d_kp_mp), v(d_mp_match), v(d_rounds)), "cms_search_local_points_device")
 
+    def search_windows_device(self, B, nq, d_qframe, d_q5, d_mp_off, d_mp_desc, nnratio, th_high, d_kp_mp, d_mp_match, d_rounds, d_cnt, d_ovf_start,
+                              d_ovf_idx, d_ovf_pd, ovf_cap, d_ovf_total):
+        v = lambda a: C.c_void_p(int(a)) if a else None
+        _chk(lib().cms_search_windows_device(self.h, B, nq, v(d_qframe), *[v(a) for a in d_q5], v(d_mp_off), v(d_mp_desc), nnratio, th_high, v(d_kp_mp),
+                                             v(d_mp_match), v(d_rounds), v(d_cnt), v(d_ovf_start), v(d_ovf_idx), v(d_ovf_pd), ovf_cap, v(d_ovf_total)),
+             "cms_search_windows_device")
+
     def hamming_best2_device(self, qdesc, q_row, nq, tdesc, cand_off, cand_idx, t_level, t_excl, outs):
         _chk(lib().cms_hamming_best2_device(self.h, _p(qdesc), _p(q_row), nq, _p(tdesc), _p(cand_off), _p(cand_idx), _p(t_level),
                                             _p(t_excl), *[_p(o) for o in outs]), "cms_hamming_best2_device")
diff --git a/cubemapslam_amd/csrc/cms_api_frames.hip b/cubemapslam_amd/csrc/cms_api_frames.hip
--- a/cubemapslam_amd/csrc/cms_api_frames.hip
+++ b/cubemapslam_amd/csrc/cms_api_frames.hip
@@ -71,6 +71,8 @@
   uint16_t* d_area_sorted = nullptr; int* d_area_cell_start = nullptr; int* d_area_nvalid = nullptr; int area_frames = 0;
   int* d_area_bsum = nullptr; int area_bsum_cap = 0;
   int* d_area_tmp = nullptr; size_t area_tmp_cap = 0;
+  uint16_t* d_track_slot_pd = nullptr; size_t track_slot_cap = 0; int* d_track_ctr = nullptr; int track_par = 0;
+  bool track_fused = true;
   uint8_t* h_fish_stage = nullptr; int fish_stage_frames = 0;
   hipStream_t copy_stream = nullptr; hipEvent_t ev_upload_done = nullptr, ev_remap_done = nullptr;
   bool upload_pending = false, remap_recorded = false;
@@ -187,7 +189,7 @@
   hipSetDevice(c->device);
   void* ptrs[] = {c->d_fish, c->d_lut, c->d_pyr, c->d_mask, c->d_tab, c->d_pattern, c->d_cand, c->d_node, c->d_cand_cnt,
                   c->d_overflow, c->d_qt_out, c->d_qt_cnt, c->d_kps, c->d_aux, c->d_order, c->d_aux_sorted, c->d_desc, c->d_kp_cnt, c->d_match, c->d_cell_cand,
-                  c->d_cell_cnt, c->d_cells_all, c->d_cells_nz, c->d_area_sorted, c->d_area_cell_start, c->d_area_nvalid, c->d_area_bsum, c->d_area_tmp, c->d_walk_cnt, c->d_rays, c->d_rtiles};
+                  c->d_cell_cnt, c->d_cells_all, c->d_cells_nz, c->d_area_sorted, c->d_area_cell_start, c->d_area_nvalid, c->d_area_bsum, c->d_area_tmp, c->d_track_slot_pd, c->d_track_ctr, c->d_walk_cnt, c->d_rays, c->d_rtiles};
   for (void* p : ptrs) if (p) hipFree(p);
   if (c->h_fish_stage) (void)hipHostFree(c->h_fish_stage);
   if (c->h_stage) (void)hipHostFree(c->h_stage);
@@ -326,6 +328,8 @@
     cms_build_lut(*cam, c->lut_stride, lut);
     hipMemcpy(c->d_lut, lut.data(), lut.size() * 4, hipMemcpyHostToDevice);
     {
+      const char* tf = getenv("CMS_TRACK_FUSED");
+      c->track_fused = !(tf && *tf && atoi(tf) == 0);
       const char* m = getenv("CMS_REMAP_TILES"); const char* tw = getenv("CMS_REMAP_TILE_W");
       c->rt_mode = m && *m ? atoi(m) : 1;
       c->rt_tw = tw && *tw ? atoi(tw) : 64;
diff --git a/cubemapslam_amd/csrc/cms_api_track.hip b/cubemapslam_amd/csrc/cms_api_track.hip
--- a/cubemapslam_amd/csrc/cms_api_track.hip
+++ b/cubemapslam_amd/csrc/cms_api_track.hip
@@ -54,6 +54,78 @@
   hipLaunchKernelGGL(k_search_local, dim3(B), dim3(1024), 0, c->stream, a);
   HIPCHK(hipGetLastError());
   return CMS_OK;
+}
+
+static int cms_track_slots_reserve(cms_ctx* c, int nq) {
+  int rc = cms_area_tmp_reserve(c, nq);
+  if (rc) return rc;
+  if (!c->d_track_ctr) {
+    HIPCHK(hipMalloc((void**)&c->d_track_ctr, 2 * sizeof(int)));
+    HIPCHK(hipMemsetAsync(c->d_track_ctr, 0, 2 * sizeof(int), c->stream));
+    c->track_par = 0;
+  }
+  if ((size_t)nq <= c->track_slot_cap) return CMS_OK;
+  if (c->d_track_slot_pd) hipFree(c->d_track_slot_pd);
+  c->d_track_slot_pd = nullptr; c->track_slot_cap = 0;
+  HIPCHK(hipMalloc((void**)&c->d_track_slot_pd, c->area_tmp_cap * CMS_AREA_TMP * sizeof(uint16_t)));
+  c->track_slot_cap = c->area_tmp_cap;
+  return CMS_OK;
+}
+
+static int cms_search_windows_launch(cms_ctx* c, int B, int frame0, int nq, const void* d_qframe, const void* d_qx, const void* d_qy, const void* d_qr,
+                                     const void* d_qmin, const void* d_qmax, const void* d_mp_off, const void* d_mp_desc, float nnratio, int th_high,
+                                     int* d_kp_mp, void* d_mp_match, void* d_rounds, void* d_cnt, void* d_ovf_start, void* d_ovf_idx, void* d_ovf_pd,
+                                     int ovf_cap, void* d_ovf_total) {
+  hipStream_t s = c->stream;
+  CmsSearchLocalArgs a;
+  a.mp_off = (const int*)d_mp_off; a.mp_desc = (const uint4*)d_mp_desc; a.cand_off = (const int*)d_ovf_start; a.cand_idx = (const int*)d_ovf_idx;
+  a.t_desc = (const uint4*)c->d_desc; a.kp = (const CmsKeyPoint*)c->d_kps; a.kp_cap = c->g.kp_cap;
+  a.pair_dist = (uint16_t*)d_ovf_pd; a.kp_mp = d_kp_mp; a.mp_match = (int*)d_mp_match; a.rounds = (int*)d_rounds;
+  a.nnratio = nnratio; a.th_high = th_high; a.frame0 = frame0; a.total = (const int*)d_ovf_total; a.cap = ovf_cap;
+  if (!c->track_fused) {
+    if (nq == 0) HIPCHK(hipMemsetAsync(d_ovf_total, 0, sizeof(int), s));
+    const int rc = cms_features_in_area_batch_device(c, nq, d_qframe, d_qx, d_qy, d_qr, d_qmin, d_qmax, d_cnt, d_ovf_start, d_ovf_idx, ovf_cap, d_ovf_total);
+    if (rc) return rc;
+    hipLaunchKernelGGL(k_search_local, dim3(B), dim3(1024), 0, s, a);
+    HIPCHK(hipGetLastError());
+    return CMS_OK;
+  }
+  const int rc = cms_track_slots_reserve(c, nq);
+  if (rc) return rc;
+  int* ctr = c->d_track_ctr + c->track_par;
+  int* next_ctr = c->d_track_ctr + (c->track_par ^ 1);
+  c->track_par ^= 1;
+  if (nq > 0) {
+    CmsTrackWindowsArgs w;
+    w.kp = (const CmsKeyPoint*)c->d_kps; w.sorted_idx = c->d_area_sorted; w.cell_start = c->d_area_cell_start; w.t_desc = (const uint4*)c->d_desc;
+    w.qx = (const float*)d_qx; w.qy = (const float*)d_qy; w.qr = (const float*)d_qr; w.qmin = (const int*)d_qmin; w.qmax = (const int*)d_qmax;
+    w.q_frame = (const int*)d_qframe; w.mp_desc = (const uint4*)d_mp_desc;
+    w.kp_cap = c->g.kp_cap; w.nq = nq; w.F = c->g.F; w.inv = (float)(3 * CMS_AREA_G) / (float)c->g.W;
+    w.cnt = (int*)d_cnt; w.slot_idx = c->d_area_tmp; w.slot_pd = c->d_track_slot_pd;
+    w.ovf_start = (int*)d_ovf_start; w.ovf_idx = (int*)d_ovf_idx; w.ovf_pd = (uint16_t*)d_ovf_pd; w.ovf_cap = ovf_cap; w.ovf_ctr = ctr;
+    hipLaunchKernelGGL(k_track_windows, dim3((nq * CMS_AREA_QL + 255) / 256), dim3(256), 0, s, w);
+  }
+  CmsSearchSlotsArgs g;
+  g.s = a; g.s.total = ctr;
+  g.v.cnt = (const int*)d_cnt; g.v.slot_idx = c->d_area_tmp; g.v.slot_pd = c->d_track_slot_pd;
+  g.v.ovf_start = (const int*)d_ovf_start; g.v.ovf_idx = (const int*)d_ovf_idx; g.v.ovf_pd = (const uint16_t*)d_ovf_pd;
+  g.total_out = (int*)d_ovf_total; g.next_ctr = next_ctr;
+  hipLaunchKernelGGL(k_search_local_slots, dim3(B), dim3(1024), 0, s, g);
+  HIPCHK(hipGetLastError());
+  return CMS_OK;
+}
+
+extern "C" int cms_search_windows_device(cms_ctx* c, int B, int nq, const void* d_qframe, const void* d_qx, const void* d_qy, const void* d_qr,
+                                         const void* d_qmin, const void* d_qmax, const void* d_mp_off, const void* d_mp_desc, float nnratio, int th_high,
+                                         void* d_kp_mp, void* d_mp_match, void* d_rounds, void* d_cnt, void* d_ovf_start, void* d_ovf_idx, void* d_ovf_pd,
+                                         int ovf_cap, void* d_ovf_total) {
+  if (!c || B < 1 || B > c->area_frames || nq < 0 || ovf_cap < 0 || !d_mp_off || !d_kp_mp || !d_ovf_total ||
+      (nq > 0 && (!d_qframe || !d_qx || !d_qy || !d_qr || !d_qmin || !d_qmax || !d_mp_desc || !d_mp_match || !d_cnt || !d_ovf_start || !d_ovf_idx || !d_ovf_pd)))
+    return cms_fail(CMS_ERR_ARG, "cms_search_windows_device: bad argument (cms_area_grid first)");
+  if (c->g.kp_cap > CMS_TRACK_KPMAX) return cms_fail(CMS_ERR_UNSUPPORTED, "cms_search_windows_device: more than 4096 key points per frame");
+  HIPCHK(hipSetDevice(c->device));
+  return cms_search_windows_launch(c, B, 0, nq, d_qframe, d_qx, d_qy, d_qr, d_qmin, d_qmax, d_mp_off, d_mp_desc, nnratio, th_high, (int*)d_kp_mp, d_mp_match,
+                                   d_rounds, d_cnt, d_ovf_start, d_ovf_idx, d_ovf_pd, ovf_cap, d_ovf_total);
 }
 
 extern "C" int cms_search_local_points(cms_ctx* c, int b, const float* pose15, int nmp, const float* pos, const float* normal,
@@ -100,18 +172,10 @@
     rc = cms_is_in_frustum_device(c, nmp, nullptr, p + o_pose, p + o_pos, p + o_nrm, p + o_min, p + o_max, viewing_cos_limit, th, p + o_vis,
                                   p + o_px, p + o_py, p + o_lvl, p + o_vc, p + o_qr, p + o_qmin, p + o_qmax);
     if (rc) return rc;
-    rc = cms_features_in_area_batch_device(c, nmp, p + o_qf, p + o_px, p + o_py, p + o_qr, p + o_qmin, p + o_qmax, p + o_cnt, p + o_off, p + o_idx,
-                                           cap, p + o_tot);
-    if (rc) return rc;
-    CmsSearchLocalArgs a;
-    a.mp_off = (const int*)(p + o_mpoff); a.mp_desc = (const uint4*)(p + o_desc); a.cand_off = (const int*)(p + o_off); a.cand_idx = (const int*)(p + o_idx);
-    a.t_desc = (const uint4*)c->d_desc; a.kp = (const CmsKeyPoint*)c->d_kps; a.kp_cap = c->g.kp_cap;
-    a.pair_dist = (uint16_t*)(p + o_pd);
-    a.kp_mp = (int*)(p + o_kpmp) - (size_t)b * c->g.kp_cap;
-    a.mp_match = (int*)(p + o_match); a.rounds = (int*)(p + o_rounds);
-    a.nnratio = nnratio; a.th_high = th_high; a.frame0 = b; a.total = (const int*)(p + o_tot); a.cap = cap;
-    hipLaunchKernelGGL(k_search_local, dim3(1), dim3(1024), 0, s, a);
-    HIPCHK(hipGetLastError());
+    rc = cms_search_windows_launch(c, 1, b, nmp, p + o_qf, p + o_px, p + o_py, p + o_qr, p + o_qmin, p + o_qmax, p + o_mpoff, p + o_desc, nnratio, th_high,
+                                   (int*)(p + o_kpmp) - (size_t)b * c->g.kp_cap, p + o_match, p + o_rounds, p + o_cnt, p + o_off, p + o_idx, p + o_pd, cap,
+                                   p + o_tot);
+    if (rc) return rc;
     HIPCHK(hipMemcpyAsync(h + out_begin, p + out_begin, out_bytes, hipMemcpyDeviceToHost, s));
     HIPCHK(hipStreamSynchronize(s));
     const int tot = *reinterpret_cast<const int*>(h + o_tot);
@@ -211,17 +275,13 @@
     HIPCHK(hipMemcpyAsync(p, h, in_bytes, hipMemcpyHostToDevice, s));
     rc = cms_project_last_frame_device(c, nlast, nullptr, p + o_pose, p + o_valid, p + o_xw, p + o_oct, th, p + o_qx, p + o_qy, p + o_qr, p + o_qmin, p + o_qmax);
     if (rc) return rc;
-    rc = cms_features_in_area_batch_device(c, nlast, p + o_qf, p + o_qx, p + o_qy, p + o_qr, p + o_qmin, p + o_qmax, p + o_cnt, p + o_off, p + o_idx, cap, p + o_tot);
-    if (rc) return rc;
-    CmsSearchLocalArgs a;
-    a.mp_off = (const int*)(p + o_mpoff); a.mp_desc = (const uint4*)(p + o_desc); a.cand_off = (const int*)(p + o_off); a.cand_idx = (const int*)(p + o_idx);
-    a.t_desc = (const uint4*)c->d_desc; a.kp = (const CmsKeyPoint*)c->d_kps; a.kp_cap = c->g.kp_cap;
-    a.pair_dist = (uint16_t*)(p + o_pd); a.kp_mp = (int*)(p + o_kpmp) - (size_t)b * c->g.kp_cap; a.mp_match = (int*)(p + o_match); a.rounds = nullptr;
-    a.nnratio = -1.0f; a.th_high = th_high; a.frame0 = b; a.total = (const int*)(p + o_tot); a.cap = cap;
-    hipLaunchKernelGGL(k_search_local, dim3(1), dim3(1024), 0, s, a);
+    int* kp_rows = (int*)(p + o_kpmp) - (size_t)b * c->g.kp_cap;
+    rc = cms_search_windows_launch(c, 1, b, nlast, p + o_qf, p + o_qx, p + o_qy, p + o_qr, p + o_qmin, p + o_qmax, p + o_mpoff, p + o_desc, -1.0f, th_high,
+                                   kp_rows, p + o_match, nullptr, p + o_cnt, p + o_off, p + o_idx, p + o_pd, cap, p + o_tot);
+    if (rc) return rc;
     CmsRotFilterArgs r;
-    r.mp_off = (const int*)(p + o_mpoff); r.last_angle = (const float*)(p + o_ang); r.kp = (const CmsKeyPoint*)c->d_kps; r.kp_mp = a.kp_mp;
-    r.mp_match = (int*)(p + o_match); r.n_matches = (int*)(p + o_nm); r.check_orientation = check_orientation; r.total = a.total; r.cap = cap;
+    r.mp_off = (const int*)(p + o_mpoff); r.last_angle = (const float*)(p + o_ang); r.kp = (const CmsKeyPoint*)c->d_kps; r.kp_mp = kp_rows;
+    r.mp_match = (int*)(p + o_match); r.n_matches = (int*)(p + o_nm); r.check_orientation = check_orientation; r.total = (const int*)(p + o_tot); r.cap = cap;
     hipLaunchKernelGGL(k_rot_filter, dim3(1), dim3(1024), 0, s, r);
     HIPCHK(hipGetLastError());
     HIPCHK(hipMemcpyAsync(h + out_begin, p + out_begin, out_bytes, hipMemcpyDeviceToHost, s));
diff --git a/cubemapslam_amd/csrc/cms_area_kernels.hip b/cubemapslam_amd/csrc/cms_area_kernels.hip
--- a/cubemapslam_amd/csrc/cms_area_kernels.hip
+++ b/cubemapslam_amd/csrc/cms_area_kernels.hip
@@ -72,32 +72,37 @@
 #define CMS_AREA_TMP 8
 
 #define CMS_AREA_QL 8
-extern "C" __global__ void __launch_bounds__(256) k_area_query(CmsAreaArgs a, int pass) {
-  const int gl = threadIdx.x & (CMS_AREA_QL - 1);
-  const int q = (blockIdx.x * blockDim.x + threadIdx.x) / CMS_AREA_QL;
-  const int qq = q < a.nq ? q : 0;
-  const float x = a.qx[qq], y = a.qy[qq], r = a.qr[qq];
-  const bool live = q < a.nq && !(r < 0.0f);
-  const int minLevel = a.qmin[qq], maxLevel = a.qmax[qq];
-  const bool check = (minLevel > 0) || (maxLevel >= 0);
-  CmsAreaRectI rc[3];
-  const int base = (pass && live) ? a.off[qq] : 0;
-  bool copied = false;
-  if (pass && a.tmp && live) {
-    const int c = a.cnt[qq];
-    if (c <= CMS_AREA_TMP) {
-      if (gl < c && base + gl < a.cap) a.idx[base + gl] = a.tmp[(size_t)qq * CMS_AREA_TMP + gl];
-      copied = true;
-    }
-  }
-  const int nr = (live && !copied) ? cms_area_rects(x, y, r, a.F, a.inv, rc) : 0;
+
+struct CmsAreaWalk {
+  const CmsKeyPoint* kp; const uint16_t* sorted_idx; const int* cell_start;
+  float x, y, r; int minLevel, maxLevel; bool check;
+};
+__device__ __forceinline__ bool cms_area_hit(const CmsAreaWalk& w, const CmsKeyPoint& p) {
+  if (w.check) {
+    if (p.octave < w.minLevel) return false;
+    if (w.maxLevel >= 0 && p.octave > w.maxLevel) return false;
+  }
+  return fabsf(p.x - w.x) < w.r && fabsf(p.y - w.y) < w.r;
+}
+template <class Emit>
+__device__ __forceinline__ void cms_area_emit_column(const CmsAreaWalk& w, int pos, int limit, int nh, int h0, int h1, int h2, int h3, int s0, int s1,
+                                                     Emit&& emit) {
+  if (pos >= limit) return;
+  if (nh <= 4) {
+    emit(pos, h0);
+    if (nh > 1 && pos + 1 < limit) emit(pos + 1, h1);
+    if (nh > 2 && pos + 2 < limit) emit(pos + 2, h2);
+    if (nh > 3 && pos + 3 < limit) emit(pos + 3, h3);
+  } else {
+    for (int s = s0; s < s1 && pos < limit; ++s) {
+      const int j = w.sorted_idx[s];
+      if (cms_area_hit(w, w.kp[j])) { emit(pos, j); ++pos; }
+    }
+  }
+}
+template <class Sink>
+__device__ __forceinline__ int cms_area_walk(const CmsAreaWalk& w, const CmsAreaRectI* rc, int nr, int gl, Sink&& sink) {
   int n = 0;
-  int* tmpq = (!pass && a.tmp) ? a.tmp + (size_t)qq * CMS_AREA_TMP : nullptr;
-  const int fr = a.q_frame ? a.q_frame[qq] : 0;
-  const CmsKeyPoint* kp = a.kp + (size_t)fr * a.kp_cap;
-  const uint16_t* sorted_idx = a.sorted_idx + (size_t)fr * a.kp_cap;
-  const int* cell_start = a.cell_start + (size_t)fr * (CMS_AREA_CELLS + 1);
-  const int idx_base = a.idx_base + (a.q_frame ? fr * a.kp_cap : 0);
   for (int k = 0; k < 3; ++k) {
     const bool has = k < nr;
     const int x0 = has ? max(0, rc[k].x0) : 0, x1 = has ? min(CMS_AREA_G - 1, rc[k].x1) : -1;
@@ -112,18 +117,13 @@
       int s0 = 0, s1 = 0;
       if (col) {
         const int c0 = (face * CMS_AREA_G + ix) * CMS_AREA_G + y0;
-        s0 = cell_start[c0]; s1 = cell_start[c0 + (y1 - y0) + 1];
+        s0 = w.cell_start[c0]; s1 = w.cell_start[c0 + (y1 - y0) + 1];
       }
       int h0 = 0, h1 = 0, h2 = 0, h3 = 0;
       int nh = 0;
       for (int s = s0; s < s1; ++s) {
-        const int j = sorted_idx[s];
-        const CmsKeyPoint p = kp[j];
-        if (check) {
-          if (p.octave < minLevel) continue;
-          if (maxLevel >= 0 && p.octave > maxLevel) continue;
-        }
-        if (fabsf(p.x - x) < r && fabsf(p.y - y) < r) {
+        const int j = w.sorted_idx[s];
+        if (cms_area_hit(w, w.kp[j])) {
           if (nh == 0) h0 = j; else if (nh == 1) h1 = j; else if (nh == 2) h2 = j; else if (nh == 3) h3 = j;
           ++nh;
         }
@@ -132,43 +132,45 @@
 #pragma unroll
       for (int o = 1; o < CMS_AREA_QL; o <<= 1) { const int t = __shfl_up(incl, o, CMS_AREA_QL); if (gl >= o) incl += t; }
       const int tot = __shfl(incl, CMS_AREA_QL - 1, CMS_AREA_QL);
-      if (tmpq && nh > 0) {
-        int w = n + incl - nh;
-        if (w < CMS_AREA_TMP) {
-          if (nh <= 4) {
-            tmpq[w] = idx_base + h0;
-            if (nh > 1 && w + 1 < CMS_AREA_TMP) tmpq[w + 1] = idx_base + h1;
-            if (nh > 2 && w + 2 < CMS_AREA_TMP) tmpq[w + 2] = idx_base + h2;
-            if (nh > 3 && w + 3 < CMS_AREA_TMP) tmpq[w + 3] = idx_base + h3;
-          } else {
-            for (int s = s0; s < s1 && w < CMS_AREA_TMP; ++s) {
-              const int j = sorted_idx[s];
-              const CmsKeyPoint p = kp[j];
-              if (check && (p.octave < minLevel || (maxLevel >= 0 && p.octave > maxLevel))) continue;
-              if (fabsf(p.x - x) < r && fabsf(p.y - y) < r) { tmpq[w] = idx_base + j; ++w; }
-            }
-          }
-        }
-      }
-      if (pass && nh > 0) {
-        int w = base + n + incl - nh;
-        if (nh <= 4) {
-          if (w < a.cap) a.idx[w] = idx_base + h0;
-          if (nh > 1 && w + 1 < a.cap) a.idx[w + 1] = idx_base + h1;
-          if (nh > 2 && w + 2 < a.cap) a.idx[w + 2] = idx_base + h2;
-          if (nh > 3 && w + 3 < a.cap) a.idx[w + 3] = idx_base + h3;
-        } else {
-          for (int s = s0; s < s1; ++s) {
-            const int j = sorted_idx[s];
-            const CmsKeyPoint p = kp[j];
-            if (check && (p.octave < minLevel || (maxLevel >= 0 && p.octave > maxLevel))) continue;
-            if (fabsf(p.x - x) < r && fabsf(p.y - y) < r) { if (w < a.cap) a.idx[w] = idx_base + j; ++w; }
-          }
-        }
-      }
+      if (nh > 0) sink(n + incl - nh, nh, h0, h1, h2, h3, s0, s1);
       n += tot;
     }
   }
+  return n;
+}
+
+extern "C" __global__ void __launch_bounds__(256) k_area_query(CmsAreaArgs a, int pass) {
+  const int gl = threadIdx.x & (CMS_AREA_QL - 1);
+  const int q = (blockIdx.x * blockDim.x + threadIdx.x) / CMS_AREA_QL;
+  const int qq = q < a.nq ? q : 0;
+  CmsAreaWalk w;
+  w.x = a.qx[qq]; w.y = a.qy[qq]; w.r = a.qr[qq];
+  const bool live = q < a.nq && !(w.r < 0.0f);
+  w.minLevel = a.qmin[qq]; w.maxLevel = a.qmax[qq];
+  w.check = (w.minLevel > 0) || (w.maxLevel >= 0);
+  CmsAreaRectI rc[3];
+  const int base = (pass && live) ? a.off[qq] : 0;
+  bool copied = false;
+  if (pass && a.tmp && live) {
+    const int c = a.cnt[qq];
+    if (c <= CMS_AREA_TMP) {
+      if (gl < c && base + gl < a.cap) a.idx[base + gl] = a.tmp[(size_t)qq * CMS_AREA_TMP + gl];
+      copied = true;
+    }
+  }
+  const int nr = (live && !copied) ? cms_area_rects(w.x, w.y, w.r, a.F, a.inv, rc) : 0;
+  int* tmpq = (!pass && a.tmp) ? a.tmp + (size_t)qq * CMS_AREA_TMP : nullptr;
+  const int fr = a.q_frame ? a.q_frame[qq] : 0;
+  w.kp = a.kp + (size_t)fr * a.kp_cap;
+  w.sorted_idx = a.sorted_idx + (size_t)fr * a.kp_cap;
+  w.cell_start = a.cell_start + (size_t)fr * (CMS_AREA_CELLS + 1);
+  const int idx_base = a.idx_base + (a.q_frame ? fr * a.kp_cap : 0);
+  const int n = cms_area_walk(w, rc, nr, gl, [&](int pos, int nh, int h0, int h1, int h2, int h3, int s0, int s1) {
+    if (tmpq)
+      cms_area_emit_column(w, pos, CMS_AREA_TMP, nh, h0, h1, h2, h3, s0, s1, [&](int at, int j) { tmpq[at] = idx_base + j; });
+    if (pass)
+      cms_area_emit_column(w, base + pos, 0x7FFFFFFF, nh, h0, h1, h2, h3, s0, s1, [&](int at, int j) { if (at < a.cap) a.idx[at] = idx_base + j; });
+  });
   if (!pass && q < a.nq && gl == 0) a.cnt[q] = n;
 }
 
diff --git a/cubemapslam_amd/csrc/cms_area_table.h b/cubemapslam_amd/csrc/cms_area_table.h
--- a/cubemapslam_amd/csrc/cms_area_table.h
+++ b/cubemapslam_amd/csrc/cms_area_table.h
@@ -124,11 +124,9 @@
   v[AV_AU] = (int)floorf((xs + Ff) * inv); v[AV_CU] = (int)floorf((ys + Ff) * inv);
   v[AV_AN] = (int)floorf((-xs) * inv); v[AV_CN] = (int)floorf((-ys) * inv);
   const CmsAreaCase* cs;
-  CmsAreaCase inside;
   if (xinf && yinf) {
-    inside.n = 1;
-    inside.r[0].face = (int8_t)face; inside.r[0].x0 = vA; inside.r[0].x1 = vB; inside.r[0].y0 = vC; inside.r[0].y1 = vD;
-    cs = &inside;
+    out[0].face = face; out[0].x0 = v[AV_A]; out[0].x1 = v[AV_B]; out[0].y0 = v[AV_C]; out[0].y1 = v[AV_D];
+    return 1;
   } else if (xinf) {
     cs = &kAreaXin[face][yo ? 0 : 1];
   } else if (yinf) {
diff --git a/cubemapslam_amd/csrc/cms_track_kernels.hip b/cubemapslam_amd/csrc/cms_track_kernels.hip
--- a/cubemapslam_amd/csrc/cms_track_kernels.hip
+++ b/cubemapslam_amd/csrc/cms_track_kernels.hip
@@ -113,12 +113,90 @@
 }
 
 #define CMS_TRACK_KPMAX 4096
+
+struct CmsCsrView {
+  const int* off; const int* idx; const uint16_t* pd;
+  __device__ __forceinline__ int count(int i) const { return off[i + 1] - off[i]; }
+  __device__ __forceinline__ int list(int i, const int*& li, const uint16_t*& lp) const {
+    const int c0 = off[i];
+    li = idx + c0; lp = pd + c0;
+    return off[i + 1] - c0;
+  }
+};
+struct CmsSlotView {
+  const int* cnt; const int* slot_idx; const uint16_t* slot_pd; const int* ovf_start; const int* ovf_idx; const uint16_t* ovf_pd;
+  __device__ __forceinline__ int count(int i) const { return cnt[i]; }
+  __device__ __forceinline__ int list(int i, const int*& li, const uint16_t*& lp) const {
+    const int n = cnt[i];
+    if (n <= CMS_AREA_TMP) { li = slot_idx + (size_t)i * CMS_AREA_TMP; lp = slot_pd + (size_t)i * CMS_AREA_TMP; }
+    else { const int s = ovf_start[i]; li = ovf_idx + s; lp = ovf_pd + s; }
+    return n;
+  }
+};
+
+template <class View>
+__device__ __forceinline__ void track_greedy_rounds(const CmsSearchLocalArgs& a, const View& v, int* min_open) {
+  const int f = blockIdx.x, tid = threadIdx.x, nt = blockDim.x;
+  const int m0 = a.mp_off[f], m1 = a.mp_off[f + 1];
+  const int row0 = (f + a.frame0) * a.kp_cap;
+  for (int i = m0 + tid; i < m1; i += nt) a.mp_match[i] = v.count(i) == 0 ? -1 : -2;
+  __syncthreads();
+  int round = 0;
+  for (;;) {
+    for (int k = tid; k < a.kp_cap; k += nt) min_open[k] = 0x7FFFFFFF;
+    __syncthreads();
+    for (int i = m0 + tid; i < m1; i += nt) {
+      if (a.mp_match[i] != -2) continue;
+      const int* li; const uint16_t* lp;
+      const int n = v.list(i, li, lp);
+      for (int c = 0; c < n; ++c) {
+        const int row = li[c];
+        if (a.kp_mp[row] < 0) atomicMin(&min_open[row - row0], i);
+      }
+    }
+    __syncthreads();
+    int open = 0;
+    for (int i = m0 + tid; i < m1; i += nt) {
+      if (a.mp_match[i] != -2) continue;
+      const int* li; const uint16_t* lp;
+      const int n = v.list(i, li, lp);
+      bool ok = true;
+      for (int c = 0; c < n && ok; ++c) {
+        const int row = li[c];
+        ok = a.kp_mp[row] >= 0 || min_open[row - row0] == i;
+      }
+      if (ok) a.mp_match[i] = -3; else ++open;
+    }
+    __syncthreads();
+    for (int i = m0 + tid; i < m1; i += nt) {
+      if (a.mp_match[i] != -3) continue;
+      const int* li; const uint16_t* lp;
+      const int n = v.list(i, li, lp);
+      int bestDist = 256, bestLevel = -1, bestDist2 = 256, bestLevel2 = -1, bestRow = -1;
+      for (int c = 0; c < n; ++c) {
+        const int row = li[c];
+        if (a.kp_mp[row] >= 0) continue;
+        const int dist = lp[c];
+        if (dist < bestDist) { bestDist2 = bestDist; bestDist = dist; bestLevel2 = bestLevel; bestLevel = a.kp[row].octave; bestRow = row; }
+        else if (dist < bestDist2) { bestLevel2 = a.kp[row].octave; bestDist2 = dist; }
+      }
+      int m = -1;
+      const bool ratio_ok = a.nnratio < 0.0f || !(bestLevel == bestLevel2 && (float)bestDist > __fmul_rn(a.nnratio, (float)bestDist2));
+      if (bestDist <= a.th_high && ratio_ok) m = bestRow;
+      if (m >= 0) a.kp_mp[m] = i;
+      a.mp_match[i] = m;
+    }
+    ++round;
+    if (__syncthreads_count(open > 0) == 0) break;
+  }
+  if (a.rounds && tid == 0) a.rounds[f] = round;
+}
+
 extern "C" __global__ void __launch_bounds__(1024) k_search_local(CmsSearchLocalArgs a) {
   __shared__ int min_open[CMS_TRACK_KPMAX];
   const int f = blockIdx.x, tid = threadIdx.x, nt = blockDim.x;
   if (a.total && *a.total > a.cap) return;
   const int m0 = a.mp_off[f], m1 = a.mp_off[f + 1];
-  const int row0 = (f + a.frame0) * a.kp_cap;
   {
     const int sub = tid & 3;
     for (int i = m0 + (tid >> 2); i < m1; i += nt >> 2) {
@@ -131,51 +209,73 @@
       }
     }
   }
-  for (int i = m0 + tid; i < m1; i += nt) a.mp_match[i] = a.cand_off[i] == a.cand_off[i + 1] ? -1 : -2;
-  __syncthreads();
-  int round = 0;
-  for (;;) {
-    for (int k = tid; k < a.kp_cap; k += nt) min_open[k] = 0x7FFFFFFF;
-    __syncthreads();
-    for (int i = m0 + tid; i < m1; i += nt) {
-      if (a.mp_match[i] != -2) continue;
-      for (int c = a.cand_off[i]; c < a.cand_off[i + 1]; ++c) {
-        const int row = a.cand_idx[c];
-        if (a.kp_mp[row] < 0) atomicMin(&min_open[row - row0], i);
-      }
-    }
-    __syncthreads();
-    int open = 0;
-    for (int i = m0 + tid; i < m1; i += nt) {
-      if (a.mp_match[i] != -2) continue;
-      bool ok = true;
-      for (int c = a.cand_off[i]; c < a.cand_off[i + 1] && ok; ++c) {
-        const int row = a.cand_idx[c];
-        ok = a.kp_mp[row] >= 0 || min_open[row - row0] == i;
-      }
-      if (ok) a.mp_match[i] = -3; else ++open;
-    }
-    __syncthreads();
-    for (int i = m0 + tid; i < m1; i += nt) {
-      if (a.mp_match[i] != -3) continue;
-      int bestDist = 256, bestLevel = -1, bestDist2 = 256, bestLevel2 = -1, bestRow = -1;
-      for (int c = a.cand_off[i]; c < a.cand_off[i + 1]; ++c) {
-        const int row = a.cand_idx[c];
-        if (a.kp_mp[row] >= 0) continue;
-        const int dist = a.pair_dist[c];
-        if (dist < bestDist) { bestDist2 = bestDist; bestDist = dist; bestLevel2 = bestLevel; bestLevel = a.kp[row].octave; bestRow = row; }
-        else if (dist < bestDist2) { bestLevel2 = a.kp[row].octave; bestDist2 = dist; }
-      }
-      int m = -1;
-      const bool ratio_ok = a.nnratio < 0.0f || !(bestLevel == bestLevel2 && (float)bestDist > __fmul_rn(a.nnratio, (float)bestDist2));
-      if (bestDist <= a.th_high && ratio_ok) m = bestRow;
-      if (m >= 0) a.kp_mp[m] = i;
-      a.mp_match[i] = m;
-    }
-    ++round;
-    if (__syncthreads_count(open > 0) == 0) break;
-  }
-  if (a.rounds && tid == 0) a.rounds[f] = round;
+  __syncthreads();
+  CmsCsrView v;
+  v.off = a.cand_off; v.idx = a.cand_idx; v.pd = a.pair_dist;
+  track_greedy_rounds(a, v, min_open);
+}
+
+struct CmsTrackWindowsArgs {
+  const CmsKeyPoint* kp; const uint16_t* sorted_idx; const int* cell_start; const uint4* t_desc;
+  const float* qx; const float* qy; const float* qr; const int* qmin; const int* qmax; const int* q_frame;
+  const uint4* mp_desc;
+  int kp_cap, nq, F; float inv;
+  int* cnt; int* slot_idx; uint16_t* slot_pd;
+  int* ovf_start; int* ovf_idx; uint16_t* ovf_pd; int ovf_cap; int* ovf_ctr;
+};
+extern "C" __global__ void __launch_bounds__(256) k_track_windows(CmsTrackWindowsArgs a) {
+  const int gl = threadIdx.x & (CMS_AREA_QL - 1);
+  const int q = (blockIdx.x * blockDim.x + threadIdx.x) / CMS_AREA_QL;
+  const int qq = q < a.nq ? q : 0;
+  CmsAreaWalk w;
+  w.x = a.qx[qq]; w.y = a.qy[qq]; w.r = a.qr[qq];
+  const bool live = q < a.nq && !(w.r < 0.0f);
+  w.minLevel = a.qmin[qq]; w.maxLevel = a.qmax[qq];
+  w.check = (w.minLevel > 0) || (w.maxLevel >= 0);
+  CmsAreaRectI rc[3];
+  const int nr = live ? cms_area_rects(w.x, w.y, w.r, a.F, a.inv, rc) : 0;
+  const int fr = a.q_frame ? a.q_frame[qq] : 0;
+  w.kp = a.kp + (size_t)fr * a.kp_cap;
+  w.sorted_idx = a.sorted_idx + (size_t)fr * a.kp_cap;
+  w.cell_start = a.cell_start + (size_t)fr * (CMS_AREA_CELLS + 1);
+  const int idx_base = fr * a.kp_cap;
+  uint4 q0 = make_uint4(0, 0, 0, 0), q1 = q0;
+  if (live) { q0 = a.mp_desc[2 * (size_t)qq]; q1 = a.mp_desc[2 * (size_t)qq + 1]; }
+  int* si = a.slot_idx + (size_t)qq * CMS_AREA_TMP;
+  uint16_t* sp = a.slot_pd + (size_t)qq * CMS_AREA_TMP;
+  const int n = cms_area_walk(w, rc, nr, gl, [&](int pos, int nh, int h0, int h1, int h2, int h3, int s0, int s1) {
+    cms_area_emit_column(w, pos, CMS_AREA_TMP, nh, h0, h1, h2, h3, s0, s1, [&](int at, int j) {
+      const size_t row = (size_t)(idx_base + j);
+      si[at] = (int)row;
+      sp[at] = (uint16_t)track_hamming256(q0, q1, a.t_desc[2 * row], a.t_desc[2 * row + 1]);
+    });
+  });
+  if (q < a.nq && gl == 0) a.cnt[q] = n;
+  const bool over = n > CMS_AREA_TMP;
+  if (!__any(over)) return;
+  int start = 0;
+  if (over && gl == 0) { start = atomicAdd(a.ovf_ctr, n); a.ovf_start[q] = start; }
+  start = __shfl(start, 0, CMS_AREA_QL);
+  cms_area_walk(w, rc, over ? nr : 0, gl, [&](int pos, int nh, int h0, int h1, int h2, int h3, int s0, int s1) {
+    cms_area_emit_column(w, start + pos, a.ovf_cap, nh, h0, h1, h2, h3, s0, s1, [&](int at, int j) {
+      const size_t row = (size_t)(idx_base + j);
+      a.ovf_idx[at] = (int)row;
+      a.ovf_pd[at] = (uint16_t)track_hamming256(q0, q1, a.t_desc[2 * row], a.t_desc[2 * row + 1]);
+    });
+  });
+}
+
+struct CmsSearchSlotsArgs {
+  CmsSearchLocalArgs s;
+  CmsSlotView v;
+  int* total_out; int* next_ctr;
+};
+extern "C" __global__ void __launch_bounds__(1024) k_search_local_slots(CmsSearchSlotsArgs a) {
+  __shared__ int min_open[CMS_TRACK_KPMAX];
+  const int tot = *a.s.total;
+  if (blockIdx.x == 0 && threadIdx.x == 0) { if (a.total_out) *a.total_out = tot; *a.next_ctr = 0; }
+  if (tot > a.s.cap) return;
+  track_greedy_rounds(a.s, a.v, min_open);
 }
 
 
diff --git a/cubemapslam_amd/host/batch_driver.cpp b/cubemapslam_amd/host/batch_driver.cpp
--- a/cubemapslam_amd/host/batch_driver.cpp
+++ b/cubemapslam_amd/host/batch_driver.cpp
@@ -218,17 +218,13 @@
   chk(cms_stream_copy_device(c, S.d_kpmp, S.d_kpmp0, S.kpmp_bytes), "cms_stream_copy_device");
   chk(cms_project_last_frame_device(c, S.nq, S.d_mm_frame, S.d_mm_pose, S.d_mm_valid, S.d_mm_xw, S.d_mm_oct, 15.0f, S.d_mm_q[0], S.d_mm_q[1], S.d_mm_q[2],
                                     S.d_mm_q[3], S.d_mm_q[4]), "cms_project_last_frame_device");
-  chk(cms_features_in_area_batch_device(c, S.nq, S.d_mm_frame, S.d_mm_q[0], S.d_mm_q[1], S.d_mm_q[2], S.d_mm_q[3], S.d_mm_q[4], S.d_cnt, S.d_off, S.d_idx,
-                                        S.cand_cap, S.d_tot), "cms_features_in_area_batch_device");
-  chk(cms_search_local_points_device(c, B, S.d_mm_mpoff, S.d_mm_desc, S.d_off, S.d_idx, S.d_mm_pd, -1.0f, 100, S.d_kpmp, S.d_mm_match, nullptr),
-      "cms_search_local_points_device");
+  chk(cms_search_windows_device(c, B, S.nq, S.d_mm_frame, S.d_mm_q[0], S.d_mm_q[1], S.d_mm_q[2], S.d_mm_q[3], S.d_mm_q[4], S.d_mm_mpoff, S.d_mm_desc, -1.0f, 100,
+                                S.d_kpmp, S.d_mm_match, nullptr, S.d_cnt, S.d_off, S.d_idx, S.d_mm_pd, S.cand_cap, S.d_tot), "cms_search_windows_device");
   chk(cms_rotation_filter_device(c, B, S.d_mm_mpoff, S.d_mm_ang, S.d_kpmp, S.d_mm_match, S.d_mm_n, 1), "cms_rotation_filter_device");
   chk(cms_is_in_frustum_device(c, S.n_mp, S.d_lm_frame, S.d_lm_pose, S.d_lm_in[0], S.d_lm_in[1], S.d_lm_in[2], S.d_lm_in[3], 0.5f, 1.0f, S.d_lm_vis, S.d_lm_f[0],
                                S.d_lm_f[1], S.d_lm_i[0], S.d_lm_f[2], S.d_lm_f[3], S.d_lm_i[1], S.d_lm_i[2]), "cms_is_in_frustum_device");
-  chk(cms_features_in_area_batch_device(c, S.n_mp, S.d_lm_frame, S.d_lm_f[0], S.d_lm_f[1], S.d_lm_f[3], S.d_lm_i[1], S.d_lm_i[2], S.d_lm_i[3], S.d_lm_off,
-                                        S.d_lm_idx, S.lm_cap, S.d_lm_tot), "cms_features_in_area_batch_device");
-  chk(cms_search_local_points_device(c, B, S.d_lm_mpoff, S.d_lm_desc, S.d_lm_off, S.d_lm_idx, S.d_lm_pd, 0.8f, 100, S.d_kpmp, S.d_lm_i[4], nullptr),
-      "cms_search_local_points_device");
+  chk(cms_search_windows_device(c, B, S.n_mp, S.d_lm_frame, S.d_lm_f[0], S.d_lm_f[1], S.d_lm_f[3], S.d_lm_i[1], S.d_lm_i[2], S.d_lm_mpoff, S.d_lm_desc, 0.8f, 100,
+                                S.d_kpmp, S.d_lm_i[4], nullptr, S.d_lm_i[3], S.d_lm_off, S.d_lm_idx, S.d_lm_pd, S.lm_cap, S.d_lm_tot), "cms_search_windows_device");
 }
 void one_step(cbd* d, int i) {
   const cbd_plan& p = d->p;
diff --git a/include/cubemapslam_hip.h b/include/cubemapslam_hip.h
--- a/include/cubemapslam_hip.h
+++ b/include/cubemapslam_hip.h
@@ -174,6 +174,10 @@
 int cms_search_local_points_device(cms_ctx* ctx, int B, const void* d_mp_off, const void* d_mp_desc, const void* d_cand_off,
                                    const void* d_cand_idx, void* d_pair_dist, float nnratio, int th_high, void* d_kp_mp, void* d_mp_match,
                                    void* d_rounds);
+int cms_search_windows_device(cms_ctx* ctx, int B, int nq, const void* d_qframe, const void* d_qx, const void* d_qy, const void* d_qr,
+                              const void* d_min_level, const void* d_max_level, const void* d_mp_off, const void* d_mp_desc, float nnratio,
+                              int th_high, void* d_kp_mp, void* d_mp_match, void* d_rounds, void* d_cnt, void* d_ovf_start, void* d_ovf_idx,
+                              void* d_ovf_pd, int ovf_cap, void* d_ovf_total);
 
 typedef struct {
   int n; const cms_keypoint* kps; const uint8_t* desc; const float* rays; const int* mp;
```

Result: no change. 24250 (median of 2 runs) (+0.1%).
